# 31415Hacker/RayTracer-public

Measured on AMD Instinct MI355X. Metric: Msamples/sec @1920x1080 Stanford-Dragon-class, 4 spp, 8 bounces, higher is better.
Workload: dtype f32; 1 GPU; C2: dragon-class procedural closed mesh (871414 tris, seed 20260109; dragon.glb absent), native LBVH2->BVH4, 1920x1080, 4 spp, 8 bounces, camera (0,0,2.5) identity quat FOV 70, a new frame index (sample set) every step; triangles=871414, bvh4_nodes=1263056, width=1920, height=1080, spp=4, max_bounces=8, seed=1, frames_per_launch=32

## Files before the change

include/mi355pt.h:

```cpp
#ifndef MI355PT_H
#define MI355PT_H

#include <stdint.h>

#ifdef __cplusplus
extern "C" {
#endif

#if defined(__GNUC__)
#define PT_API __attribute__((visibility("default")))
#else
#define PT_API
#endif

typedef struct PtContext PtContext;

typedef enum PtStatus {
    PT_OK = 0,
    PT_ERR_INVALID_ARG = 1,
    PT_ERR_NO_DEVICE = 2,
    PT_ERR_HIP = 3,
    PT_ERR_NO_SCENE = 4,
    PT_ERR_BAD_BVH = 5,
    PT_ERR_IO = 6,
// ... 47 lines not shown
PT_API int  pt_set_stream(PtContext* ctx, void* hip_stream);
PT_API int  pt_synchronize(PtContext* ctx);
PT_API int  pt_get_stream(PtContext* ctx, void** hip_stream);


PT_API int pt_compute_bvh2_sizing(uint32_t num_tris, uint32_t* num_nodes2, uint64_t* bytes);
PT_API int pt_compute_bvh4_sizing(uint32_t num_nodes4, uint64_t* bytes);
PT_API int pt_morton_sort(const float* tris, uint32_t num_tris, uint32_t* morton_sorted, uint32_t* tri_index_sorted);
PT_API int pt_collapse_lbvh2_to_bvh4(const uint32_t* bvh2, uint32_t num_tris, uint32_t* out, uint64_t out_words, uint32_t* num_nodes4);
#define PT_ACCEL_REFERENCE     0
#define PT_ACCEL_AREA_COLLAPSE 1
#define PT_ACCEL_PLOC          2
PT_API int pt_collapse_bvh2_to_bvh4_accel(const uint32_t* bvh2, uint32_t num_tris, uint32_t accel, uint32_t* out, uint64_t out_words, uint32_t* num_nodes4);
PT_API int pt_build_bvh2_ploc(const float* tris, uint32_t num_tris, uint32_t* out, uint64_t out_words);
PT_API int pt_bvh2_to_bvh4_wide(const uint32_t* bvh2, uint64_t bvh2_words, uint32_t* out, uint64_t out_words);
PT_API int pt_file_write_u32(const char* path, const uint32_t* src, uint64_t words);
PT_API int pt_file_read_u32(const char* path, uint32_t* dst, uint64_t dst_words, uint64_t* words);

PT_API int pt_scene_procedural(uint32_t kind, uint32_t seed, uint32_t num_tris, float* tris_out);


PT_API int pt_set_triangles(PtContext* ctx, const float* tris, uint32_t num_tris);
PT_API int pt_build_bvh(PtContext* ctx);
PT_API int pt_build_bvh_accel(PtContext* ctx, uint32_t accel);
PT_API int pt_build_lbvh2(PtContext* ctx, const uint32_t* morton_sorted, const uint32_t* tri_index_sorted);
PT_API int pt_read_bvh2(PtContext* ctx, uint32_t* dst, uint64_t bytes);
PT_API int pt_set_bvh4(PtContext* ctx, const uint32_t* bvh4, uint64_t words);
PT_API int pt_set_bvh2(PtContext* ctx, const uint32_t* bvh2, uint64_t words);
PT_API int pt_read_bvh4(PtContext* ctx, uint32_t* dst, uint64_t bytes);
PT_API int pt_set_spheres(PtContext* ctx, const float* xyzr, uint32_t num_spheres);
PT_API int pt_scene_info(PtContext* ctx, uint32_t* num_tris, uint32_t* num_nodes2, uint32_t* num_nodes4);


PT_API int pt_render(PtContext* ctx, const PtRenderParams* params);
PT_API int pt_set_batch(PtContext* ctx, uint32_t frames_per_launch);
PT_API int pt_flush(PtContext* ctx);
PT_API int pt_last_render_ms(PtContext* ctx, float* ms);
PT_API int pt_timing_begin(PtContext* ctx, uint32_t capacity);
PT_API int pt_timing_collect(PtContext* ctx, float* ms, uint32_t capacity, uint32_t* count);
PT_API int pt_timing_collect_spans(PtContext* ctx, float* start_ms, float* dur_ms, uint32_t capacity, uint32_t* count);
PT_API int pt_get_stats(PtContext* ctx, PtStats* out);
PT_API int pt_read_radiance(PtContext* ctx, float* dst, uint64_t dst_floats);
PT_API int pt_read_rgba8(PtContext* ctx, uint8_t* dst, uint64_t dst_bytes);
PT_API int pt_read_tonemapped(PtContext* ctx, int from_rgba8, uint8_t* dst, uint64_t dst_bytes);

typedef struct PtAccumInfo {
    uint32_t width, height;
    uint32_t tile_rank, tile_count;
    uint32_t compact;
    uint32_t samples;
    uint64_t floats;
} PtAccumInfo;
PT_API int pt_accum_info(PtContext* ctx, PtAccumInfo* out);
PT_API int pt_read_accum(PtContext* ctx, float* dst, uint64_t dst_floats);
PT_API int pt_set_accum(PtContext* ctx, const PtAccumInfo* info, const float* src);

typedef struct PtRay { float org[3]; float t_max; float dir[3]; uint32_t reserved; } PtRay;
typedef struct PtHit { float t; uint32_t prim; float u, v; } PtHit;
enum {
    PT_TRACE_ANY_HIT = 1u,
    PT_TRACE_STATS = 2u,
    PT_TRACE_SIMPLE_KERNEL = 4u
};
PT_API int pt_trace_rays(PtContext* ctx, const void* rays_device, uint64_t n, uint32_t flags, void* hits_device);
PT_API int pt_trace_rays_host(PtContext* ctx, const PtRay* rays, uint64_t n, uint32_t flags, PtHit* hits);
PT_API int pt_camera_rays(PtContext* ctx, const PtRenderParams* params, void* rays_device);

typedef struct PtPoint   { float p[3]; float r_max; } PtPoint;
typedef struct PtClosest { float dist; uint32_t prim; float u, v; } PtClosest;
enum {
    PT_CLOSEST_STATS = 1u,
    PT_CLOSEST_SIMPLE_KERNEL = 2u,
    PT_CLOSEST_BRUTE_FORCE = 4u
};
PT_API int pt_closest_points(PtContext* ctx, const void* points_device, uint64_t n, uint32_t flags, void* out_device);
PT_API int pt_closest_points_host(PtContext* ctx, const PtPoint* points, uint64_t n, uint32_t flags, PtClosest* out);
PT_API int pt_closest_points_bvh4(const float* tris, uint32_t num_tris, const uint32_t* bvh4, uint64_t words,
                                  const PtPoint* points, uint64_t n, uint32_t flags, PtClosest* out, PtStats* stats);

typedef struct PtSurfel    { float p[3]; float r_max; float n[3]; uint32_t reserved; } PtSurfel;
typedef struct PtOcclusion { float visibility; uint32_t unoccluded; uint32_t samples; uint32_t reserved; } PtOcclusion;
typedef struct PtOcclusionParams { uint32_t samples; uint32_t seed; uint32_t index_base; float bias; uint32_t flags; } PtOcclusionParams;
enum {
    PT_OCCLUSION_STATS = 1u,
    PT_OCCLUSION_SIMPLE_KERNEL = 2u
};
PT_API int pt_occlusion(PtContext* ctx, const void* surfels_device, uint64_t n, const PtOcclusionParams* params, void* out_device);
PT_API int pt_occlusion_host(PtContext* ctx, const PtSurfel* surfels, uint64_t n, const PtOcclusionParams* params, PtOcclusion* out);
PT_API int pt_occlusion_rays(PtContext* ctx, const void* surfels_device, uint64_t n, const PtOcclusionParams* params, void* rays_device);
PT_API int pt_occlusion_rays_host(const PtSurfel* surfels, uint64_t n, const PtOcclusionParams* params, PtRay* rays);
PT_API int pt_hit_surfels(PtContext* ctx, const void* rays_device, const void* hits_device, uint64_t n, float r_max, void* surfels_device);
PT_API int pt_hit_surfels_host(PtContext* ctx, const PtRay* rays, const PtHit* hits, uint64_t n, float r_max, PtSurfel* out);

PT_API int pt_update_triangles(PtContext* ctx, const float* tris, uint32_t num_tris);
PT_API int pt_update_triangles_device(PtContext* ctx, const void* tris_device, uint32_t num_tris);
PT_API int pt_bvh_cost(PtContext* ctx, double* cost);
PT_API int pt_refit_bvh4(const float* tris, uint32_t num_tris, uint32_t* bvh4, uint64_t words);
PT_API int pt_refit_bvh2(const float* tris, uint32_t num_tris, uint32_t* bvh2, uint64_t words);
PT_API int pt_bvh4_cost(const uint32_t* bvh4, uint64_t words, double* cost);


PT_API int pt_tile_layout(uint32_t width, uint32_t height, uint32_t tile_rank, uint32_t tile_count,
                   uint32_t* num_tiles, uint64_t* compact_floats);
PT_API int pt_tile_ids(uint32_t width, uint32_t height, uint32_t tile_rank, uint32_t tile_count,
                uint32_t* ids, uint32_t capacity, uint32_t* num_tiles);
PT_API int pt_compact_radiance(PtContext* ctx, void** device_ptr, uint64_t* floats);
PT_API int pt_set_compact_buffer(PtContext* ctx, void* device_ptr, uint64_t floats);
PT_API int pt_set_output_buffer(PtContext* ctx, void* device_ptr, uint64_t floats);
PT_API int pt_buffer_busy(PtContext* ctx, const void* device_ptr, uint64_t bytes, int* busy);
PT_API int pt_deinterleave(PtContext* ctx, const void* gathered_device, uint64_t stride_floats,
                    uint32_t width, uint32_t height, uint32_t tile_count);
PT_API int pt_deinterleave_batch(PtContext* ctx, const void* gathered_device, uint64_t rank_stride_floats, uint64_t frame_stride_floats,
                          uint32_t num_frames, uint32_t width, uint32_t height, uint32_t tile_count,
                          void* frames_out_device, uint64_t out_stride_floats);

PT_API int pt_traced_tile_rect(PtContext* ctx, const PtRenderParams* params, uint32_t rect[4]);
PT_API int pt_packed_layout(uint32_t width, uint32_t height, uint32_t tile_count, const uint32_t rect[4], uint32_t* max_tiles, uint64_t* floats_per_frame);
PT_API int pt_packed_tile_ids(uint32_t width, uint32_t height, uint32_t tile_rank, uint32_t tile_count, const uint32_t rect[4],
                              uint32_t* ids, uint32_t capacity, uint32_t* num_tiles);
PT_API int pt_pack_shares(PtContext* ctx, const void* compact_device, uint64_t frame_stride_floats, uint32_t num_frames, uint32_t width, uint32_t height,
                          uint32_t tile_rank, uint32_t tile_count, const uint32_t rect[4], void* packed_device, uint64_t packed_frame_stride_floats);
PT_API int pt_unpack_batch(PtContext* ctx, const void* gathered_device, uint64_t rank_stride_floats, uint64_t frame_stride_floats, uint32_t num_frames,
                           uint32_t width, uint32_t height, uint32_t tile_count, const uint32_t rect[4], uint32_t spp,
                           void* frames_out_device, uint64_t out_stride_floats);

typedef struct PtGroup PtGroup;
enum {
    PT_GROUP_TRANSPORT_RCCL = 0,
    PT_GROUP_TRANSPORT_COPY = 1
};
PT_API int  pt_group_create(const int* device_ordinals, uint32_t num_devices, uint32_t transport, PtGroup** out);
PT_API void pt_group_destroy(PtGroup* group);
PT_API const char* pt_group_last_error(const PtGroup* group);
PT_API int  pt_group_size(const PtGroup* group, uint32_t* num_members);
PT_API int  pt_group_context(PtGroup* group, uint32_t rank, PtContext** ctx);
PT_API int  pt_group_set_triangles(PtGroup* group, const float* tris, uint32_t num_tris);
PT_API int  pt_group_update_triangles(PtGroup* group, const float* tris, uint32_t num_tris);
PT_API int  pt_group_build_bvh(PtGroup* group);
PT_API int  pt_group_build_bvh_accel(PtGroup* group, uint32_t accel);
PT_API int  pt_group_set_bvh2(PtGroup* group, const uint32_t* bvh2, uint64_t words);
PT_API int  pt_group_set_bvh4(PtGroup* group, const uint32_t* bvh4, uint64_t words);
PT_API int  pt_group_set_batch(PtGroup* group, uint32_t frames_per_launch);
PT_API int  pt_group_render(PtGroup* group, const PtRenderParams* params);
PT_API int  pt_group_flush(PtGroup* group);
PT_API int  pt_group_synchronize(PtGroup* group);
PT_API int  pt_group_read_radiance(PtGroup* group, float* dst, uint64_t dst_floats);
PT_API int  pt_group_read_rgba8(PtGroup* group, uint8_t* dst, uint64_t dst_bytes);
PT_API int  pt_group_read_tonemapped(PtGroup* group, int from_rgba8, uint8_t* dst, uint64_t dst_bytes);

PT_API int pt_debug_set_tune(PtContext* ctx, const char* name, uint32_t value);
PT_API int pt_debug_launch_plan(uint32_t num_cus, uint32_t frames, uint32_t tile_count, uint32_t launches_in_flight, uint32_t traced_batches, uint32_t batch_size, uint32_t out[12]);
PT_API int pt_debug_counters(PtContext* ctx, unsigned long long* dst24);
PT_API int pt_debug_wave_times(PtContext* ctx, unsigned long long* dst, uint32_t max_waves, uint32_t* n_waves);

#ifdef __cplusplus
}
#endif
#endif
```

raytracer-public_amd/__init__.py:

```python
import ctypes as C
import math
import os
import sys

import numpy as np

_HERE = os.path.dirname(os.path.abspath(__file__))
LIB_PATH = os.path.join(_HERE, "libmi355pt.so")

PT_MODE_REFERENCE_PACKET, PT_MODE_REFERENCE, PT_MODE_PATH = 0, 1, 2
PT_FLAG_STATS = 1
PT_FLAG_SIMPLE_KERNEL = 2
PT_FLAG_BRUTE_FORCE = 4
PT_FLAG_COMPACT = 8
SCENE_DRAGON_CLASS, SCENE_SPONZA_CLASS = 0, 1
PT_ACCEL_REFERENCE, PT_ACCEL_AREA_COLLAPSE, PT_ACCEL_PLOC = 0, 1, 2
PT_TRACE_ANY_HIT, PT_TRACE_STATS, PT_TRACE_SIMPLE_KERNEL = 1, 2, 4
PT_CLOSEST_STATS, PT_CLOSEST_SIMPLE_KERNEL, PT_CLOSEST_BRUTE_FORCE = 1, 2, 4
PT_OCCLUSION_STATS, PT_OCCLUSION_SIMPLE_KERNEL = 1, 2
PRIM_NONE = 0xFFFFFFFF


class PtError(RuntimeError):
    def __init__(self, code, message):
        super().__init__("libmi355pt error %d: %s" % (code, message))
        self.code = code


class PtRenderParams(C.Structure):
    _fields_ = [
        ("width", C.c_uint32), ("height", C.c_uint32),
        ("focal", C.c_float), ("aspect", C.c_float),
        ("cam_pos", C.c_float * 3), ("num_tris", C.c_uint32),
        ("cam_quat", C.c_float * 4),
        ("frame", C.c_uint32), ("mode", C.c_uint32),
        ("spp", C.c_uint32), ("max_bounces", C.c_uint32), ("seed", C.c_uint32),
        ("accumulate", C.c_uint32),
        ("tile_rank", C.c_uint32), ("tile_count", C.c_uint32),
        ("flags", C.c_uint32),
    ]


class PtStats(C.Structure):
    _fields_ = [(n, C.c_uint64) for n in (
        "rays_closest", "rays_shadow", "nodes_examined", "tris_tested", "stack_drops", "max_stack", "samples")]

    def as_dict(self):
        return {n: int(getattr(self, n)) for n, _ in self._fields_}


class PtRay(C.Structure):
    _fields_ = [("org", C.c_float * 3), ("t_max", C.c_float), ("dir", C.c_float * 3), ("reserved", C.c_uint32)]


class PtHit(C.Structure):
    _fields_ = [("t", C.c_float), ("prim", C.c_uint32), ("u", C.c_float), ("v", C.c_float)]


class PtPoint(C.Structure):
    _fields_ = [("p", C.c_float * 3), ("r_max", C.c_float)]


class PtClosest(C.Structure):
    _fields_ = [("dist", C.c_float), ("prim", C.c_uint32), ("u", C.c_float), ("v", C.c_float)]


class PtSurfel(C.Structure):
    _fields_ = [("p", C.c_float * 3), ("r_max", C.c_float), ("n", C.c_float * 3), ("reserved", C.c_uint32)]


class PtOcclusion(C.Structure):
    _fields_ = [("visibility", C.c_float), ("unoccluded", C.c_uint32), ("samples", C.c_uint32), ("reserved", C.c_uint32)]


class PtOcclusionParams(C.Structure):
    _fields_ = [("samples", C.c_uint32), ("seed", C.c_uint32), ("index_base", C.c_uint32), ("bias", C.c_float), ("flags", C.c_uint32)]


class PtAccumInfo(C.Structure):
    _fields_ = [("width", C.c_uint32), ("height", C.c_uint32), ("tile_rank", C.c_uint32), ("tile_count", C.c_uint32),
                ("compact", C.c_uint32), ("samples", C.c_uint32), ("floats", C.c_uint64)]


EXPORTS = [
    "pt_create", "pt_destroy", "pt_last_error", "pt_version", "pt_set_stream", "pt_get_stream", "pt_synchronize",
    "pt_compute_bvh2_sizing", "pt_compute_bvh4_sizing", "pt_morton_sort", "pt_collapse_lbvh2_to_bvh4",
    "pt_collapse_bvh2_to_bvh4_accel", "pt_build_bvh2_ploc", "pt_bvh2_to_bvh4_wide", "pt_file_write_u32", "pt_file_read_u32", "pt_scene_procedural",
    "pt_set_triangles", "pt_build_bvh", "pt_build_bvh_accel", "pt_build_lbvh2", "pt_read_bvh2", "pt_set_bvh4", "pt_set_bvh2",
    "pt_read_bvh4", "pt_set_spheres", "pt_scene_info", "pt_render", "pt_last_render_ms", "pt_set_batch", "pt_flush", "pt_timing_begin", "pt_timing_collect", "pt_timing_collect_spans", "pt_set_compact_buffer", "pt_set_output_buffer", "pt_get_stats", "pt_read_radiance",
    "pt_read_rgba8", "pt_read_tonemapped", "pt_tile_layout", "pt_tile_ids", "pt_compact_radiance", "pt_deinterleave", "pt_deinterleave_batch", "pt_buffer_busy",
    "pt_accum_info", "pt_read_accum", "pt_set_accum",
    "pt_trace_rays", "pt_trace_rays_host", "pt_camera_rays",
    "pt_closest_points", "pt_closest_points_host", "pt_closest_points_bvh4",
    "pt_occlusion", "pt_occlusion_host", "pt_occlusion_rays", "pt_occlusion_rays_host", "pt_hit_surfels", "pt_hit_surfels_host",
    "pt_update_triangles", "pt_update_triangles_device", "pt_bvh_cost", "pt_refit_bvh4", "pt_refit_bvh2", "pt_bvh4_cost", "pt_group_update_triangles",
    "pt_traced_tile_rect", "pt_packed_layout", "pt_packed_tile_ids", "pt_pack_shares", "pt_unpack_batch",
    "pt_group_create", "pt_group_destroy", "pt_group_last_error", "pt_group_size", "pt_group_context", "pt_group_set_triangles", "pt_group_build_bvh",
    "pt_group_build_bvh_accel",
    "pt_group_set_bvh2", "pt_group_set_bvh4", "pt_group_set_batch", "pt_group_render", "pt_group_flush", "pt_group_synchronize", "pt_group_read_radiance",
    "pt_group_read_rgba8", "pt_group_read_tonemapped",
    "pt_debug_set_tune", "pt_debug_counters", "pt_debug_wave_times", "pt_debug_launch_plan",
]


def _load():
    os.environ.setdefault("GPU_MAX_HW_QUEUES", "12")
    if not os.path.exists(LIB_PATH):
        raise ImportError(
            "libmi355pt.so is not built (%s). Run `python -c 'import __graft_entry__ as g; g.build()'` "
            "or `make -C raytracer-public_amd/csrc`. There is no CPU fallback." % LIB_PATH)
    lib = C.CDLL(LIB_PATH)
    lib.pt_last_error.restype = C.c_char_p
    lib.pt_last_error.argtypes = [C.c_void_p]
    lib.pt_version.restype = C.c_char_p
    lib.pt_destroy.restype = None
    lib.pt_destroy.argtypes = [C.c_void_p]
    return lib


_TORCH_FIRST = "torch" in sys.modules
lib = _load()


def _p(a, t):
    return a.ctypes.data_as(C.POINTER(t))


def _aligned_zeros(shape, dtype, align=16):
    dtype = np.dtype(dtype)
    n = int(np.prod(shape)) * dtype.itemsize
    raw = np.zeros(n + align, np.uint8)
    off = (-raw.ctypes.data) % align
    return raw[off: off + n].view(dtype).reshape(shape)


def _is_torch(x):
    return type(x).__module__.startswith("torch")


def _torch_route():
    if not _TORCH_FIRST:
        raise RuntimeError("the torch route of the ray queries needs `import torch` before this package is imported: both must use "
                           "the same HIP runtime (torch ships its own)")


def pack_rays(origins, directions, t_max=None):
    o = np.asarray(origins, np.float32).reshape(-1, 3)
    d = np.asarray(directions, np.float32).reshape(-1, 3)
    if o.shape != d.shape:
        raise ValueError("origins and directions differ in shape: %s vs %s" % (o.shape, d.shape))
    out = _aligned_zeros((o.shape[0], 8), np.float32)
    out[:, 0:3] = o
    out[:, 3] = np.inf if t_max is None else np.broadcast_to(np.asarray(t_max, np.float32), (o.shape[0],))
    out[:, 4:7] = d
    return out


def pack_points(points, r_max=None):
    p = np.asarray(points, np.float32).reshape(-1, 3)
    out = _aligned_zeros((p.shape[0], 4), np.float32)
    out[:, 0:3] = p
    out[:, 3] = np.inf if r_max is None else np.broadcast_to(np.asarray(r_max, np.float32), (p.shape[0],))
    return out


def _point_records(points, r_max):
    a = np.asarray(points, np.float32)
    if a.ndim == 2 and a.shape[1] == 4:
        if a.ctypes.data % 16 or not a.flags.c_contiguous or r_max is not None:
            r2 = _aligned_zeros(a.shape, np.float32); r2[...] = a; a = r2
            if r_max is not None:
                a[:, 3] = r_max
        return a
    return pack_points(a, r_max)


def pack_surfels(points, normals, r_max=None):
    return pack_rays(points, normals, r_max)


def _records8(a, what):
    a = np.asarray(a, np.float32)
    if a.ndim != 2 or a.shape[1] != 8:
        raise ValueError("%s: expected (n, 8) float32 records, got shape %s" % (what, a.shape))
    if a.ctypes.data % 16 or not a.flags.c_contiguous:
        r2 = _aligned_zeros(a.shape, np.float32); r2[...] = a; a = r2
    return a


def _occlusion_params(samples, seed, bias, index_base, stats=False, simple=False):
    p = PtOcclusionParams()
    p.samples, p.seed, p.index_base, p.bias = int(samples), int(seed) & 0xFFFFFFFF, int(index_base) & 0xFFFFFFFF, float(bias)
    p.flags = (PT_OCCLUSION_STATS if stats else 0) | (PT_OCCLUSION_SIMPLE_KERNEL if simple else 0)
    return p


def occlusion_rays_host(surfels, samples, seed=0, bias=1e-4, index_base=0):
    sf = _records8(surfels, "occlusion_rays_host")
    n = sf.shape[0]
    p = _occlusion_params(samples, seed, bias, index_base)
    rays = _aligned_zeros((n * max(int(samples), 0) if 0 < int(samples) <= 65536 else 0, 8), np.float32)
    _check(lib.pt_occlusion_rays_host(sf.ctypes.data_as(C.POINTER(PtSurfel)), C.c_uint64(n), C.byref(p), rays.ctypes.data_as(C.POINTER(PtRay))))
    return rays


def _closest_flags(stats, simple, brute_force):
    return (PT_CLOSEST_STATS if stats else 0) | (PT_CLOSEST_SIMPLE_KERNEL if simple else 0) | (PT_CLOSEST_BRUTE_FORCE if brute_force else 0)


def _check(rc, ctx=None):
    if rc != 0:
        msg = lib.pt_last_error(ctx)
        raise PtError(rc, msg.decode() if msg else "")


def focal_aspect(width, height):
    fov = (70.0 * math.pi) / 180
    return float(np.float32(1.0 / math.tan(0.5 * fov))), float(np.float32(width / height))



def compute_bvh2_sizing(num_tris):
    nn, by = C.c_uint32(), C.c_uint64()
    _check(lib.pt_compute_bvh2_sizing(C.c_uint32(num_tris), C.byref(nn), C.byref(by)))
    return {"numNodes2": nn.value, "bytes": by.value}


def compute_bvh4_sizing(num_nodes4):
    by = C.c_uint64()
    _check(lib.pt_compute_bvh4_sizing(C.c_uint32(num_nodes4), C.byref(by)))
    return {"bytes": by.value}


def morton_sort(tris):
    tris = np.ascontiguousarray(tris, np.float32).reshape(-1)
    n = tris.size // 9
    m = np.zeros(n, np.uint32); t = np.zeros(n, np.uint32)
    _check(lib.pt_morton_sort(_p(tris, C.c_float), C.c_uint32(n), _p(m, C.c_uint32), _p(t, C.c_uint32)))
    return m, t


def collapse_lbvh2_to_bvh4(bvh2, num_tris):
    bvh2 = np.ascontiguousarray(bvh2, np.uint32)
    cap = 1 + 8 * max(2 * num_tris - 1, 0)
    out = np.zeros(cap, np.uint32)
    n4 = C.c_uint32()
    _check(lib.pt_collapse_lbvh2_to_bvh4(_p(bvh2, C.c_uint32), C.c_uint32(num_tris), _p(out, C.c_uint32), C.c_uint64(cap), C.byref(n4)))
    return out[: 1 + 8 * n4.value].copy(), n4.value


def collapse_bvh2_to_bvh4_accel(bvh2, num_tris, accel):
    bvh2 = np.ascontiguousarray(bvh2, np.uint32)
    cap = 1 + 8 * max(2 * num_tris - 1, 0)
    out = np.zeros(cap, np.uint32)
# ... 93 lines not shown
    r = (C.c_uint32 * 4)(*rect); n = C.c_uint32()
    _check(lib.pt_packed_tile_ids(C.c_uint32(width), C.c_uint32(height), C.c_uint32(rank), C.c_uint32(count), r, None, C.c_uint32(0), C.byref(n)))
    ids = np.zeros(max(n.value, 1), np.uint32)
    _check(lib.pt_packed_tile_ids(C.c_uint32(width), C.c_uint32(height), C.c_uint32(rank), C.c_uint32(count), r, _p(ids, C.c_uint32), C.c_uint32(ids.size), C.byref(n)))
    return ids[: n.value]


def tile_ids(width, height, rank, count):
    n = C.c_uint32()
    _check(lib.pt_tile_ids(C.c_uint32(width), C.c_uint32(height), C.c_uint32(rank), C.c_uint32(count), None, C.c_uint32(0), C.byref(n)))
    ids = np.zeros(max(n.value, 1), np.uint32)
    _check(lib.pt_tile_ids(C.c_uint32(width), C.c_uint32(height), C.c_uint32(rank), C.c_uint32(count), ids.ctypes.data_as(C.POINTER(C.c_uint32)), C.c_uint32(ids.size), C.byref(n)))
    return ids[: n.value]



class Context:

    def __init__(self, device=-1):
        h = C.c_void_p()
        _check(lib.pt_create(C.c_int(device), C.byref(h)))
        self.h = h

    def close(self):
        if getattr(self, "h", None):
            lib.pt_destroy(self.h)
            self.h = None

    def __del__(self):
        try:
            self.close()
        except Exception:
            pass

    def _ck(self, rc):
        _check(rc, self.h)

    def set_stream(self, stream_handle):
        self._ck(lib.pt_set_stream(self.h, C.c_void_p(stream_handle)))

    def get_stream(self):
        p = C.c_void_p()
        self._ck(lib.pt_get_stream(self.h, C.byref(p)))
        return p.value

    def synchronize(self):
        self._ck(lib.pt_synchronize(self.h))

    def set_triangles(self, tris):
        tris = np.ascontiguousarray(tris, np.float32).reshape(-1)
        self._ck(lib.pt_set_triangles(self.h, _p(tris, C.c_float), C.c_uint32(tris.size // 9)))
        self.num_tris = tris.size // 9

    def update_triangles(self, tris):
        if _is_torch(tris):
            _torch_route()
            import torch
            if tris.device.type != "cuda":
                raise ValueError("update_triangles: torch tensors must be on the context's GPU (got %s)" % tris.device)
            t = tris.reshape(-1)
            if t.dtype != torch.float32 or not t.is_contiguous() or t.data_ptr() % 16:
                t = t.to(torch.float32).contiguous().clone()
            if t.numel() % 9:
                raise ValueError("update_triangles: 9 floats per triangle")
            self._on_context_stream(t.device, lambda: self.update_triangles_device(t.data_ptr(), t.numel() // 9))
            return
        tris = np.ascontiguousarray(tris, np.float32).reshape(-1)
        self._ck(lib.pt_update_triangles(self.h, _p(tris, C.c_float), C.c_uint32(tris.size // 9)))

    def update_triangles_device(self, tris_ptr, num_tris):
        self._ck(lib.pt_update_triangles_device(self.h, C.c_void_p(tris_ptr), C.c_uint32(num_tris)))

    def bvh_cost(self):
        cost = C.c_double()
        self._ck(lib.pt_bvh_cost(self.h, C.byref(cost)))
        return cost.value

    def set_spheres(self, xyzr):
        xyzr = np.ascontiguousarray(xyzr, np.float32).reshape(-1)
        self._ck(lib.pt_set_spheres(self.h, _p(xyzr, C.c_float), C.c_uint32(xyzr.size // 4)))

    def build_bvh(self, accel=PT_ACCEL_REFERENCE):
        if accel == PT_ACCEL_REFERENCE:
            self._ck(lib.pt_build_bvh(self.h))
        else:
            self._ck(lib.pt_build_bvh_accel(self.h, C.c_uint32(accel)))

    def build_lbvh2(self, morton, tri_idx):
        morton = np.ascontiguousarray(morton, np.uint32); tri_idx = np.ascontiguousarray(tri_idx, np.uint32)
        self._ck(lib.pt_build_lbvh2(self.h, _p(morton, C.c_uint32), _p(tri_idx, C.c_uint32)))

    def read_bvh2(self):
        out = np.zeros(compute_bvh2_sizing(self.num_tris)["bytes"] // 4, np.uint32)
        self._ck(lib.pt_read_bvh2(self.h, _p(out, C.c_uint32), C.c_uint64(out.size * 4)))
        return out

    def set_bvh4(self, bvh4):
        bvh4 = np.ascontiguousarray(bvh4, np.uint32)
        self._ck(lib.pt_set_bvh4(self.h, _p(bvh4, C.c_uint32), C.c_uint64(bvh4.size)))

    def set_bvh2(self, bvh2):
        bvh2 = np.ascontiguousarray(bvh2, np.uint32)
        self._ck(lib.pt_set_bvh2(self.h, _p(bvh2, C.c_uint32), C.c_uint64(bvh2.size)))

    def scene_info(self):
        a, b, c = C.c_uint32(), C.c_uint32(), C.c_uint32()
        self._ck(lib.pt_scene_info(self.h, C.byref(a), C.byref(b), C.byref(c)))
        return {"numTris": a.value, "numNodes2": b.value, "numNodes4": c.value}

    def read_bvh4(self):
        out = np.zeros(1 + 8 * self.scene_info()["numNodes4"], np.uint32)
        self._ck(lib.pt_read_bvh4(self.h, _p(out, C.c_uint32), C.c_uint64(out.size * 4)))
        return out

    def make_params(self, width, height, cam_pos=(0, 0, 2.5), cam_quat=(0, 0, 0, 1), mode=PT_MODE_REFERENCE, spp=1,
                    max_bounces=0, seed=1, frame=0, accumulate=False, tile_rank=0, tile_count=1, stats=False, num_tris=None, simple_kernel=False, brute_force=False):
        p = PtRenderParams()
        p.width, p.height = width, height
        p.focal, p.aspect = focal_aspect(width, height)
        p.cam_pos[:] = [float(np.float32(v)) for v in cam_pos]
        p.cam_quat[:] = [float(np.float32(v)) for v in cam_quat]
        p.num_tris = self.num_tris if num_tris is None else num_tris
        p.frame, p.mode, p.spp, p.max_bounces, p.seed = frame, mode, spp, max_bounces, seed
        p.accumulate = 1 if accumulate else 0
        p.tile_rank, p.tile_count = tile_rank, tile_count
        p.flags = (PT_FLAG_STATS if stats else 0) | (PT_FLAG_SIMPLE_KERNEL if simple_kernel else 0) | (PT_FLAG_BRUTE_FORCE if brute_force else 0)
        return p

    def render(self, params):
        self._ck(lib.pt_render(self.h, C.byref(params)))
        self._last = (params.width, params.height)

    def last_render_ms(self):
        ms = C.c_float()
        self._ck(lib.pt_last_render_ms(self.h, C.byref(ms)))
        return ms.value

    def set_batch(self, frames_per_launch):
        self._ck(lib.pt_set_batch(self.h, C.c_uint32(frames_per_launch)))

    def flush(self):
        self._ck(lib.pt_flush(self.h))

    def timing_begin(self, capacity):
        self._ck(lib.pt_timing_begin(self.h, C.c_uint32(capacity)))

    def timing_collect(self, capacity):
        ms = np.zeros(capacity, np.float32); n = C.c_uint32()
        self._ck(lib.pt_timing_collect(self.h, _p(ms, C.c_float), C.c_uint32(capacity), C.byref(n)))
        return ms[: n.value].copy()

    def debug_set_tune(self, name, value=None):
        self._ck(lib.pt_debug_set_tune(self.h, name.encode(), C.c_uint32(0xFFFFFFFF if value is None else value)))

    def timing_collect_spans(self, capacity):
        st = np.zeros(capacity, np.float32); ms = np.zeros(capacity, np.float32); n = C.c_uint32()
        self._ck(lib.pt_timing_collect_spans(self.h, _p(st, C.c_float), _p(ms, C.c_float), C.c_uint32(capacity), C.byref(n)))
        return st[: n.value].copy(), ms[: n.value].copy()

    def set_compact_buffer(self, device_ptr, floats):
        self._ck(lib.pt_set_compact_buffer(self.h, C.c_void_p(device_ptr), C.c_uint64(floats)))

    def set_output_buffer(self, device_ptr, floats):
        self._ck(lib.pt_set_output_buffer(self.h, C.c_void_p(device_ptr), C.c_uint64(floats)))

    def stats(self):
        st = PtStats()
        self._ck(lib.pt_get_stats(self.h, C.byref(st)))
        return st.as_dict()

    def read_radiance(self, width=None, height=None):
        w, h = (width, height) if width else self._last
        out = np.zeros((h, w, 4), np.float32)
        self._ck(lib.pt_read_radiance(self.h, _p(out, C.c_float), C.c_uint64(out.size)))
        return out

    def read_rgba8(self):
        w, h = self._last
        out = np.zeros((h, w, 4), np.uint8)
        self._ck(lib.pt_read_rgba8(self.h, _p(out, C.c_uint8), C.c_uint64(out.size)))
        return out

    def read_tonemapped(self, from_rgba8=True):
        w, h = self._last
        out = np.zeros((h, w, 4), np.uint8)
        self._ck(lib.pt_read_tonemapped(self.h, C.c_int(int(from_rgba8)), _p(out, C.c_uint8), C.c_uint64(out.size)))
        return out

    def compact_radiance(self):
        ptr, fl = C.c_void_p(), C.c_uint64()
        self._ck(lib.pt_compact_radiance(self.h, C.byref(ptr), C.byref(fl)))
        return ptr.value, fl.value

    def deinterleave(self, gathered_device_ptr, stride_floats, width, height, tile_count):
        self._ck(lib.pt_deinterleave(self.h, C.c_void_p(gathered_device_ptr), C.c_uint64(stride_floats),
                                     C.c_uint32(width), C.c_uint32(height), C.c_uint32(tile_count)))
        self._last = (width, height)

    def deinterleave_batch(self, gathered_device_ptr, rank_stride_floats, frame_stride_floats, num_frames, width, height, tile_count, frames_out_ptr=0, out_stride_floats=0):
        self._ck(lib.pt_deinterleave_batch(self.h, C.c_void_p(gathered_device_ptr), C.c_uint64(rank_stride_floats), C.c_uint64(frame_stride_floats), C.c_uint32(num_frames),
                                           C.c_uint32(width), C.c_uint32(height), C.c_uint32(tile_count), C.c_void_p(frames_out_ptr or None), C.c_uint64(out_stride_floats)))
        self._last = (width, height)

    def traced_tile_rect(self, params):
        r = (C.c_uint32 * 4)()
        self._ck(lib.pt_traced_tile_rect(self.h, C.byref(params), r))
        return tuple(int(v) for v in r)

    def pack_shares(self, compact_ptr, frame_stride_floats, num_frames, width, height, tile_rank, tile_count, rect, packed_ptr, packed_frame_stride_floats):
        self._ck(lib.pt_pack_shares(self.h, C.c_void_p(compact_ptr), C.c_uint64(frame_stride_floats), C.c_uint32(num_frames), C.c_uint32(width), C.c_uint32(height),
                                    C.c_uint32(tile_rank), C.c_uint32(tile_count), (C.c_uint32 * 4)(*rect), C.c_void_p(packed_ptr), C.c_uint64(packed_frame_stride_floats)))

    def unpack_batch(self, gathered_ptr, rank_stride_floats, frame_stride_floats, num_frames, width, height, tile_count, rect, spp, frames_out_ptr=0, out_stride_floats=0):
        self._ck(lib.pt_unpack_batch(self.h, C.c_void_p(gathered_ptr), C.c_uint64(rank_stride_floats), C.c_uint64(frame_stride_floats), C.c_uint32(num_frames),
                                     C.c_uint32(width), C.c_uint32(height), C.c_uint32(tile_count), (C.c_uint32 * 4)(*rect), C.c_uint32(spp),
                                     C.c_void_p(frames_out_ptr or None), C.c_uint64(out_stride_floats)))
        self._last = (width, height)

    def accum_info(self):
        info = PtAccumInfo()
        self._ck(lib.pt_accum_info(self.h, C.byref(info)))
        return info

    def read_accum(self):
        info = self.accum_info()
        out = np.zeros(int(info.floats), np.float32)
        self._ck(lib.pt_read_accum(self.h, _p(out, C.c_float), C.c_uint64(out.size)))
        return info, out

    def set_accum(self, info, data):
        data = np.ascontiguousarray(data, np.float32).reshape(-1)
        assert data.size == info.floats
        self._ck(lib.pt_set_accum(self.h, C.byref(info), _p(data, C.c_float)))

    def trace_rays(self, origins, directions=None, t_max=None, any_hit=False, stats=False, simple=False):
        flags = (PT_TRACE_ANY_HIT if any_hit else 0) | (PT_TRACE_STATS if stats else 0) | (PT_TRACE_SIMPLE_KERNEL if simple else 0)
        if _is_torch(origins):
            return self._trace_rays_torch(origins, directions, t_max, flags)
        if directions is None:
            rays = np.asarray(origins, np.float32).reshape(-1, 8)
            if rays.ctypes.data % 16 or not rays.flags.c_contiguous or t_max is not None:
                r2 = _aligned_zeros(rays.shape, np.float32); r2[...] = rays; rays = r2
                if t_max is not None:
                    rays[:, 3] = t_max
        else:
            rays = pack_rays(origins, directions, t_max)
        n = rays.shape[0]
        hits = _aligned_zeros((n, 4), np.uint32)
        self._ck(lib.pt_trace_rays_host(self.h, rays.ctypes.data_as(C.POINTER(PtRay)), C.c_uint64(n), C.c_uint32(flags),
                                        hits.ctypes.data_as(C.POINTER(PtHit))))
        f = hits.view(np.float32)
        return f[:, 0].copy(), hits[:, 1].copy(), f[:, 2].copy(), f[:, 3].copy()

    def trace_rays_device(self, rays_ptr, n, hits_ptr, flags=0):
        self._ck(lib.pt_trace_rays(self.h, C.c_void_p(rays_ptr), C.c_uint64(n), C.c_uint32(flags), C.c_void_p(hits_ptr)))

    def camera_rays_device(self, params, rays_ptr):
        self._ck(lib.pt_camera_rays(self.h, C.byref(params), C.c_void_p(rays_ptr)))

    def _on_context_stream(self, device, launch):
        import torch
        cur = torch.cuda.current_stream(device)
        mine = self.get_stream()
        if cur.cuda_stream == mine:
            launch()
            return
        ext = torch.cuda.ExternalStream(mine, device=device)
        before = torch.cuda.Event(); before.record(cur); ext.wait_event(before)
        launch()
        after = torch.cuda.Event(); after.record(ext); cur.wait_event(after)

    def _trace_rays_torch(self, origins, directions, t_max, flags):
        _torch_route()
        import torch
        dev = origins.device
        if dev.type != "cuda":
            raise ValueError("trace_rays: torch tensors must be on the context's GPU (got %s)" % dev)
        if directions is None:
            rays = origins.reshape(-1, 8)
            if rays.dtype != torch.float32 or not rays.is_contiguous() or rays.data_ptr() % 16:
                rays = rays.to(torch.float32).contiguous().clone()
            if t_max is not None:
                rays = rays.clone(); rays[:, 3] = t_max
        else:
            o = origins.reshape(-1, 3).to(torch.float32); d = directions.reshape(-1, 3).to(device=dev, dtype=torch.float32)
            n = o.shape[0]
            tm = torch.full((n, 1), float("inf"), dtype=torch.float32, device=dev) if t_max is None else \
                torch.as_tensor(t_max, dtype=torch.float32, device=dev).reshape(-1, 1).expand(n, 1)
            rays = torch.cat([o, tm, d, torch.zeros((n, 1), dtype=torch.float32, device=dev)], dim=1).contiguous()
        n = rays.shape[0]
        hits = torch.empty((n, 4), dtype=torch.int32, device=dev)
        self._on_context_stream(dev, lambda: self.trace_rays_device(rays.data_ptr(), n, hits.data_ptr(), flags))
        hf = hits.view(torch.float32)
        return hf[:, 0], hits.view(torch.uint32)[:, 1], hf[:, 2], hf[:, 3]

    def camera_rays(self, params, device=None):
        _torch_route()
        import torch
        dev = torch.device("cuda", torch.cuda.current_device() if device is None else device)
        rays = torch.empty((params.height * params.width, 8), dtype=torch.float32, device=dev)
        self._on_context_stream(dev, lambda: self.camera_rays_device(params, rays.data_ptr()))
        return rays

    def closest_points(self, points, r_max=None, stats=False, simple=False, brute_force=False):
        flags = _closest_flags(stats, simple, brute_force)
        if _is_torch(points):
# ... 295 lines not shown
```

raytracer-public_amd/csrc/pt_api.cpp:

```cpp
#include "mi355pt.h"
#include "pt_host.h"
#include "pt_kernels.h"

#include <hip/hip_runtime.h>

#include <algorithm>
#include <cstdio>
#include <cstdlib>
#include <cstring>
#include <string>
#include <vector>

namespace {

thread_local std::string g_global_error;

template <typename T>
struct DevBuf {
    T* ptr = nullptr; size_t cap = 0;
    hipError_t ensure(size_t n) {
        if (n <= cap && ptr) return hipSuccess;
        if (ptr) { (void)hipFree(ptr); ptr = nullptr; cap = 0; }
        if (n == 0) n = 1;
        hipError_t e = hipMalloc((void**)&ptr, n * sizeof(T));
        if (e == hipSuccess) cap = n;
        return e;
    }
    void release() { if (ptr) (void)hipFree(ptr); ptr = nullptr; cap = 0; }
};

}

struct PtTune {
    static constexpr uint32_t kAuto = 0xFFFFFFFFu;
    uint32_t grid_div = kAuto, rows = kAuto, chunk = kAuto, xcd = kAuto, shade = kAuto, fill = kAuto,
             slots = kAuto, cull = kAuto, stats_batch = kAuto, quad = kAuto, fork = kAuto, bounded = kAuto, timeline = kAuto;
    uint32_t* find(const char* name) {
        static const struct { const char* n; uint32_t PtTune::* m; } tab[] = {
            {"GRIDDIV", &PtTune::grid_div}, {"ROWS", &PtTune::rows}, {"CHUNK", &PtTune::chunk}, {"XCD", &PtTune::xcd}, {"SHADE", &PtTune::shade},
            {"FILL", &PtTune::fill}, {"SLOTS", &PtTune::slots}, {"CULL", &PtTune::cull}, {"STATSBATCH", &PtTune::stats_batch}, {"QUAD", &PtTune::quad}, {"FORK", &PtTune::fork}, {"BOUNDED", &PtTune::bounded}, {"TIMELINE", &PtTune::timeline}};
        for (const auto& t : tab) if (std::strcmp(name, t.n) == 0) return &(this->*(t.m));
        return nullptr;
    }
    void from_environment() {
        static const char* names[] = {"GRIDDIV", "ROWS", "CHUNK", "XCD", "SHADE", "FILL", "SLOTS", "CULL", "STATSBATCH", "QUAD", "FORK", "BOUNDED", "TIMELINE"};
        for (const char* n : names) {
            const std::string key = std::string("PT_TUNE_") + n;
            const char* v = std::getenv(key.c_str());
            if (v && *v) *find(n) = uint32_t(std::strtoul(v, nullptr, 10));
        }
    }
    static uint32_t pick(uint32_t knob, uint32_t dflt) { return knob == kAuto ? dflt : knob; }
};

struct PtContext {
    int device = 0;
    PtTune tune;
    hipStream_t own_stream = nullptr;
    hipStream_t stream = nullptr;
    hipEvent_t ev_start = nullptr, ev_stop = nullptr;
    bool timed = false;
    std::string err;

    uint32_t num_tris = 0, num_nodes2 = 0, num_nodes4 = 0;
    bool edges_small = false;
    DevBuf<uint32_t> d_edge_max;
    bool have_tris = false, have_bvh = false, have_bvh2 = false;
    bool bvh2_refit_pending = false;
    pt::WideBvh wide_meta;

    DevBuf<float> d_tris9;
    DevBuf<uint4> d_scene; uint64_t node_off = 0, node_cap = 0; uint32_t scene_tris = 0;
    float4* trirec() const { return (float4*)d_scene.ptr; }
    uint4* wide() const { return d_scene.ptr + node_off / 16; }
    DevBuf<uint32_t> d_bvh2, d_bvh4;
    DevBuf<uint32_t> d_morton, d_triidx, d_parent, d_flags;
    DevBuf<unsigned long long> d_bounds; DevBuf<uint32_t> d_counters, d_code_tmp, d_index_tmp, d_node2, d_subtree, d_ids, d_bnd;
    DevBuf<uint4> d_child_pos; DevBuf<unsigned char> d_build_temp; uint32_t* h_word = nullptr;
    DevBuf<uint32_t> d_ploc;
    DevBuf<float4> d_spheres; uint32_t num_spheres = 0;
    bool tree_built = false, refit_ready = false, refit2_ready = false;
    uint32_t num_wide = 0;
    DevBuf<uint2> d_refit_up, d_refit_self; DevBuf<uint4> d_refit_ref; DevBuf<uint32_t> d_refit_arrive, d_refit_parent2, d_refit_arrive2;
    DevBuf<double> d_cost;
    bool bvh2_stale = false;
    uint32_t* h_refit = nullptr; hipEvent_t ev_refit = nullptr; bool meta_pending = false, meta_has_root = false;
    DevBuf<unsigned long long> d_rq_queue, d_rq_spill; DevBuf<uint4> d_rq_rays, d_rq_hits;
    DevBuf<uint4> d_oc_surfels;

    DevBuf<float4> d_out, d_accum, d_compact, d_compact_accum;
    DevBuf<uint32_t> d_tiles, d_u32tmp;
    struct FrameSlot {
        hipStream_t side = nullptr; hipEvent_t resolved = nullptr, done = nullptr; bool used = false;
        uint64_t resolved_seq = 0;
        DevBuf<uint32_t> queue; DevBuf<float4> samples; DevBuf<uint2> spill; DevBuf<uint4> rays;
        DevBuf<uint32_t> trace_slots; uint32_t* h_trace = nullptr; size_t h_trace_cap = 0; hipEvent_t trace_copied = nullptr;
        uint32_t cull_key[8] = {0, 0, 0, 0, 0, 0, 0, 0}; uint32_t num_trace_tiles = 0; bool cull_valid = false;
        DevBuf<ptk::FrameParams> frame_params; DevBuf<float4*> frame_outs;
        const void* primed_ptr = nullptr; size_t primed_samples = 0;
    };
    static constexpr int kMaxSlots = 16;
    FrameSlot slots[kMaxSlots]; int num_slots = 0; uint32_t next_slot = 0;
    uint32_t batch_size = 1; uint32_t pending = 0; ptk::RenderArgs pendingA; bool pending_ring = false; uint32_t pending_rank = 0, pending_count = 1;
    std::vector<ptk::FrameParams> pending_frames; std::vector<float4*> pending_outs;
    DevBuf<unsigned long long> d_wave_times; uint32_t wave_times_n = 0;
    int num_cus = 0;
    DevBuf<unsigned long long> d_stats;
    std::vector<uint32_t> tiles_host; uint32_t tiles_w = 0, tiles_h = 0, tiles_rank = 0, tiles_count = 0;
    uint32_t out_w = 0, out_h = 0;
    uint32_t accum_w = 0, accum_h = 0, accum_count = 0, accum_rank = 0;
    uint64_t compact_floats = 0;
    uint32_t share_w = 0, share_h = 0, share_count = 0, share_max_tiles = 0;
    float4* ext_compact = nullptr; uint64_t ext_compact_floats = 0;
    float4* ext_out = nullptr; uint64_t ext_out_floats = 0;
    const float4* last_full = nullptr;
    bool last_stats = false;
    uint64_t stats_culled = 0;
    std::vector<hipEvent_t> ring;
    uint32_t ring_used = 0;
    struct InFlight { const char* lo; const char* hi; uint64_t seq; };
    std::vector<InFlight> inflight;
    uint64_t launch_seq = 0, delivered_seq = 0;
    hipEvent_t misc_fence = nullptr; uint64_t misc_fence_seq = 0;
};

namespace {

int fail(PtContext* ctx, int code, const std::string& msg) {
    if (ctx) ctx->err = msg; else g_global_error = msg;
    return code;
}
int fail_hip(PtContext* ctx, hipError_t e, const char* what) {
    return fail(ctx, PT_ERR_HIP, std::string(what) + ": " + hipGetErrorString(e));
}
#define PT_HIP(ctx, call) do { hipError_t e__ = (call); if (e__ != hipSuccess) return fail_hip((ctx), e__, #call); } while (0)

int bind(PtContext* ctx) {
    if (!ctx) return fail(nullptr, PT_ERR_INVALID_ARG, "null context");
    PT_HIP(ctx, hipSetDevice(ctx->device));
    return PT_OK;
}

int sync_refit_meta(PtContext* ctx) {
    if (!ctx->meta_pending) return PT_OK;
    PT_HIP(ctx, hipEventSynchronize(ctx->ev_refit));
    ctx->meta_pending = false;
    const uint32_t* h = ctx->h_refit;
    ctx->edges_small = h[3] < 0x49800000u;
    if (ctx->meta_has_root && ctx->have_bvh) {
        pt::WideBvh& w = ctx->wide_meta;
        w.root_box[0] = h[0]; w.root_box[1] = h[1]; w.root_box[2] = h[2];
        w.root_degenerate = pt::half_to_float(h[0] & 0xffffu) > pt::half_to_float(h[1] >> 16) || pt::half_to_float(h[0] >> 16) > pt::half_to_float(h[2] & 0xffffu) ||
                            pt::half_to_float(h[1] & 0xffffu) > pt::half_to_float(h[2] >> 16);
    }
    return PT_OK;
}

uint32_t accum_share_key(uint32_t rank, uint32_t count, bool compact) { return (rank & 0xfffu) | ((count & 0xfffu) << 12) | (compact ? 0x80000000u : 0u); }

void prune_inflight(PtContext* ctx) {
    if (ctx->inflight.empty()) return;
    uint64_t delivered = ctx->delivered_seq;
    auto done = [&](hipEvent_t ev) {
        const hipError_t q = hipEventQuery(ev);
        if (q == hipErrorNotReady) { (void)hipGetLastError(); return false; }
        return true;
    };
    for (auto& sl : ctx->slots) if (sl.side && sl.used && sl.resolved_seq > delivered && done(sl.resolved)) delivered = sl.resolved_seq;
    if (ctx->misc_fence && ctx->misc_fence_seq > delivered && done(ctx->misc_fence)) delivered = ctx->misc_fence_seq;
    if (delivered != ctx->delivered_seq) {
        ctx->delivered_seq = delivered;
        ctx->inflight.erase(std::remove_if(ctx->inflight.begin(), ctx->inflight.end(), [&](const PtContext::InFlight& f) { return f.seq <= delivered; }), ctx->inflight.end());
    }
}
void everything_delivered(PtContext* ctx) {
    ctx->delivered_seq = ctx->launch_seq; ctx->inflight.clear();
}
uint64_t track_targets(PtContext* ctx, float4* const* targets, uint32_t n, size_t bytes) {
    if (ctx->inflight.size() >= 64) prune_inflight(ctx);
    const uint64_t seq = ++ctx->launch_seq;
    for (uint32_t i = 0; i < n; ++i) {
        if (!targets[i]) continue;
        bool dup = false;
        for (uint32_t g = 0; g < i && !dup; ++g) dup = targets[g] == targets[i];
        if (!dup) ctx->inflight.push_back({(const char*)targets[i], (const char*)targets[i] + bytes, seq});
    }
    return seq;
}

uint64_t tri_region_bytes(uint32_t num_tris) { return (uint64_t(num_tris) + 1u) * 64u; }

int ensure_scene(PtContext* ctx, uint32_t num_tris, uint64_t nodes) {
    const uint64_t tri_bytes = tri_region_bytes(num_tris);
    const uint64_t need = tri_bytes + (nodes + 1u) * 64u;
    if (need >= 0xFFFFFFFFull) return fail(ctx, PT_ERR_INVALID_ARG, "scene too large: triangle records and BVH nodes are addressed by 32-bit byte offsets (4 GiB)");
    if (ctx->d_scene.ptr && ctx->node_off == tri_bytes && ctx->node_cap >= nodes) {
        if (ctx->scene_tris != num_tris)
            PT_HIP(ctx, hipMemset((char*)ctx->d_scene.ptr + uint64_t(num_tris) * 64u, 0, tri_bytes - uint64_t(num_tris) * 64u));
        ctx->scene_tris = num_tris; return PT_OK;
    }
    const uint64_t cap_nodes = nodes + nodes / 8u + 16u;
    uint4* fresh = nullptr;
    PT_HIP(ctx, hipMalloc((void**)&fresh, tri_bytes + (cap_nodes + 1u) * 64u));
    if (ctx->d_scene.ptr && ctx->scene_tris == num_tris && num_tris)
        PT_HIP(ctx, hipMemcpy(fresh, ctx->d_scene.ptr, uint64_t(num_tris) * 64u, hipMemcpyDeviceToDevice));
    if (ctx->d_scene.ptr) (void)hipFree(ctx->d_scene.ptr);
    PT_HIP(ctx, hipMemset((char*)fresh + uint64_t(num_tris) * 64u, 0, tri_bytes - uint64_t(num_tris) * 64u));
    ctx->d_scene.ptr = fresh; ctx->d_scene.cap = size_t((tri_bytes + (cap_nodes + 1u) * 64u) / 16u);
    ctx->node_off = tri_bytes; ctx->node_cap = cap_nodes; ctx->scene_tris = num_tris;
    return PT_OK;
}

int upload_wide(PtContext* ctx, const uint32_t* bvh4, uint64_t words) {
    pt::WideBvh w; std::string err;
    if (int rc = sync_refit_meta(ctx)) return rc;
    const uint32_t tris_now = ctx->have_tris ? ctx->num_tris : 0u;
    if (!pt::build_wide_bvh(bvh4, words, tris_now, uint32_t(tri_region_bytes(tris_now) / 16u), w, err)) return fail(ctx, PT_ERR_BAD_BVH, err);
    PT_HIP(ctx, ctx->d_bvh4.ensure(words));
    PT_HIP(ctx, hipMemcpyAsync(ctx->d_bvh4.ptr, bvh4, words * 4, hipMemcpyHostToDevice, ctx->stream));
    if (int rc = ensure_scene(ctx, tris_now, w.nodes.size())) return rc;
    if (!w.nodes.empty())
        PT_HIP(ctx, hipMemcpyAsync(ctx->wide(), w.nodes.data(), w.nodes.size() * sizeof(pt::WideNode), hipMemcpyHostToDevice, ctx->stream));
    PT_HIP(ctx, hipStreamSynchronize(ctx->stream));
    ctx->num_nodes4 = w.num_nodes4;
    ctx->num_wide = uint32_t(w.nodes.size()); ctx->tree_built = false; ctx->refit_ready = false;
    w.nodes.clear(); w.nodes.shrink_to_fit();
    ctx->wide_meta = w;
    ctx->have_bvh = true;
    return PT_OK;
}

struct TileRect { uint32_t tx0, ty0, tx1, ty1; };
bool root_box_rect(const pt::WideBvh& w, const ptk::FrameParams& f, uint32_t width, uint32_t height, TileRect& out) {
    const double qx = f.quat[0], qy = f.quat[1], qz = f.quat[2], qw = f.quat[3];
    const double qn = qx * qx + qy * qy + qz * qz + qw * qw;
    if (!(qn > 1.0 - 1e-5 && qn < 1.0 + 1e-5) || !(f.focal > 1e-3f) || !(f.aspect > 1e-3f)) return false;
    const double mn[3] = {pt::half_to_float(w.root_box[0] & 0xffffu), pt::half_to_float(w.root_box[0] >> 16), pt::half_to_float(w.root_box[1] & 0xffffu)};
    const double mx[3] = {pt::half_to_float(w.root_box[1] >> 16), pt::half_to_float(w.root_box[2] & 0xffffu), pt::half_to_float(w.root_box[2] >> 16)};
    double x0 = 1e300, x1 = -1e300, y0 = 1e300, y1 = -1e300;
    for (int c = 0; c < 8; ++c) {
        const double p[3] = {((c & 1) ? mx[0] : mn[0]) - f.cam[0], ((c & 2) ? mx[1] : mn[1]) - f.cam[1], ((c & 4) ? mx[2] : mn[2]) - f.cam[2]};
        if (!(p[0] == p[0] && p[1] == p[1] && p[2] == p[2])) return false;
        const double ux = -qx, uy = -qy, uz = -qz;
        const double cx = uy * p[2] - uz * p[1], cy = uz * p[0] - ux * p[2], cz = ux * p[1] - uy * p[0];
        const double dx = uy * cz - uz * cy, dy = uz * cx - ux * cz, dz = ux * cy - uy * cx;
        const double vx = p[0] + 2.0 * (qw * cx + dx), vy = p[1] + 2.0 * (qw * cy + dy), vz = p[2] + 2.0 * (qw * cz + dz);
        if (!(vz < -1e-4)) return false;
        const double sx = vx / -vz * f.focal / f.aspect, sy = vy / -vz * f.focal;
        const double fx = (sx + 1.0) * 0.5 * width, fy = (sy + 1.0) * 0.5 * height;
        x0 = fx < x0 ? fx : x0; x1 = fx > x1 ? fx : x1; y0 = fy < y0 ? fy : y0; y1 = fy > y1 ? fy : y1;
    }
    const double margin = 2.0;
    const uint32_t tiles_x = (width + pt::kTile - 1) / pt::kTile, tiles_y = (height + pt::kTile - 1) / pt::kTile;
    auto lo = [&](double v, uint32_t n) { v = (v - margin) / pt::kTile; return v <= 0.0 ? 0u : (v >= n ? n : uint32_t(v)); };
    auto hi = [&](double v, uint32_t n) { v = (v + margin) / pt::kTile + 1.0; return v <= 0.0 ? 0u : (v >= n ? n : uint32_t(v)); };
    out.tx0 = lo(x0, tiles_x); out.tx1 = hi(x1, tiles_x); out.ty0 = lo(y0, tiles_y); out.ty1 = hi(y1, tiles_y);
    return true;
}

bool arith_is_bounded(const PtContext* ctx, const std::vector<ptk::FrameParams>& frames, uint32_t nf) {
    if (!ctx->edges_small) return false;
    for (uint32_t i = 0; i < nf; ++i) {
        const float* q = frames[i].quat;
        const double n2 = double(q[0]) * q[0] + double(q[1]) * q[1] + double(q[2]) * q[2] + double(q[3]) * q[3];
        if (!(n2 < 262144.0)) return false;
        if (!(frames[i].focal > 1e-6f && frames[i].focal < 1e6f && frames[i].aspect < 1e6f && frames[i].aspect > -1e6f)) return false;
    }
    return true;
}


struct PlanInput {
    uint32_t num_cus;
    uint32_t frames;
    uint32_t tile_count;
    bool     sharded;
    bool     stats;
    uint32_t launches_in_flight;
    uint32_t traced_batches;
    uint32_t batch_size;
};
struct LaunchPlan {
    uint32_t grid;
    uint32_t perm_rows, perm_cols, total_items, chunk_items, xcd_span;
    uint32_t shade_threshold, fill_threshold, quad_live, fork_shadow;
    int      slots, setup_slots;
    const char* error;
};

int slots_for(const PtTune& tune, uint32_t frames, uint32_t tile_count, bool sharded) {
    const uint32_t w8 = frames * 8u / (tile_count ? tile_count : 1u);
    const int n = int(PtTune::pick(tune.slots, w8 >= 256u ? 3u : (w8 >= 64u ? 4u : (w8 >= 16u ? PT_FRAME_SLOTS : (w8 >= 8u ? (sharded ? 4u : 6u) : (sharded ? 8u : PT_FRAME_SLOTS))))));
    return n < 1 ? 1 : (n > PtContext::kMaxSlots ? PtContext::kMaxSlots : n);
}

LaunchPlan plan_launch(const PtTune& tune, const PlanInput& in) {
    LaunchPlan P; std::memset(&P, 0, sizeof(P));
    const uint32_t nf = in.frames, count = in.tile_count ? in.tile_count : 1u;
    const int cus = in.num_cus > 0 ? int(in.num_cus) : 256;
    P.grid = ptk::megakernel_grid(cus);
    {
        uint32_t div = PtTune::pick(tune.grid_div, count >= 8u ? 4u : (count >= 2u ? 2u : std::min(4u, 1u + in.launches_in_flight)));
        if (nf > 1u) div = div > nf ? div / nf : 1u;
        if (div > 1u) P.grid = (P.grid + div - 1u) / div;
    }
    const uint32_t grid_lanes = P.grid * ptk::megakernel_block();
    const uint32_t work8 = nf * 8u / count;
    P.perm_rows = PtTune::pick(tune.rows, work8 >= 24u ? nf : (work8 >= 8u ? 128u * nf : 64u * nf));
    if (P.perm_rows < 1u) P.perm_rows = 1u;
    if (P.perm_rows > 4096u) P.perm_rows = 4096u;
    P.perm_cols = (in.traced_batches + P.perm_rows - 1u) / P.perm_rows;
    if (uint64_t(P.perm_cols) * P.perm_rows * 64ull > 0xFFFFFFFFull) { P.error = "pt_render: batch too large (more than 2^32 items per launch)"; return P; }
    P.total_items = P.perm_cols * P.perm_rows * 64u;
    P.chunk_items = ((PtTune::pick(tune.chunk, 128u) + 63u) / 64u) * 64u;
    if (P.chunk_items < 64u) P.chunk_items = 64u;
    if (uint64_t(P.total_items) + uint64_t(grid_lanes / 64u + 1u) * P.chunk_items > 0xFFFFFFFFull) {
        P.error = "pt_render: launch too large for the 32-bit work-queue cursor (more than 2^32 - grid * chunk items; lower spp, the resolution or the batch)"; return P;
    }
    {
        const uint32_t per = (P.total_items + 7u) / 8u;
        P.xcd_span = PtTune::pick(tune.xcd, work8 >= 64u ? 1u : 0u) ? ((per + P.chunk_items - 1u) / P.chunk_items) * P.chunk_items : 0u;
    }
    P.shade_threshold = PtTune::pick(tune.shade, PT_SHADE_THRESHOLD); P.fill_threshold = PtTune::pick(tune.fill, PT_FILL_THRESHOLD);
    P.quad_live = std::min(16u, PtTune::pick(tune.quad, PT_QUAD_LIVE));
    P.fork_shadow = PtTune::pick(tune.fork, PT_FORK_SHADOW);
    P.slots = in.stats ? 1 : slots_for(tune, nf, count, in.sharded);
    P.setup_slots = in.stats ? 1 : std::max(P.slots, slots_for(tune, std::max(nf, in.batch_size), count, in.sharded));
    return P;
}

bool traced_tiles(const PtContext* ctx, const ptk::RenderArgs& A, uint32_t nf, bool sharded, TileRect& rect, std::vector<uint32_t>& traced) {
    traced.clear(); rect = {0, 0, 0, 0};
    if (!(ctx->have_bvh && ctx->wide_meta.root_ref != pt::kInvalid && !ctx->wide_meta.root_degenerate && A.num_tris != 0u && ctx->tune.cull != 0u)) return false;
    for (uint32_t i = 0; i < nf; ++i) {
        TileRect r;
        if (!root_box_rect(ctx->wide_meta, ctx->pending_frames[i], A.width, A.height, r)) return false;
        if (i == 0) rect = r;
        else { rect.tx0 = std::min(rect.tx0, r.tx0); rect.ty0 = std::min(rect.ty0, r.ty0); rect.tx1 = std::max(rect.tx1, r.tx1); rect.ty1 = std::max(rect.ty1, r.ty1); }
    }
    const uint32_t tiles_y = (A.height + pt::kTile - 1) / pt::kTile;
    if (rect.tx0 == 0u && rect.ty0 == 0u && rect.tx1 >= A.tiles_x && rect.ty1 >= tiles_y) return false;
    auto inside = [&](uint32_t tile) { const uint32_t tx = tile % A.tiles_x, ty = tile / A.tiles_x; return tx >= rect.tx0 && tx < rect.tx1 && ty >= rect.ty0 && ty < rect.ty1; };
    if (sharded) { for (uint32_t sl = 0; sl < A.num_tiles; ++sl) if (inside(ctx->tiles_host[sl])) traced.push_back(sl); }
    else { for (uint32_t ty = rect.ty0; ty < rect.ty1; ++ty) for (uint32_t tx = rect.tx0; tx < rect.tx1; ++tx) traced.push_back(ty * A.tiles_x + tx); }
    return true;
}

int prepare_slots(PtContext* ctx, const LaunchPlan& P, const ptk::RenderArgs& A, uint32_t nf, bool stats) {
    const size_t n_samples = size_t(A.num_sample_batches) * 64u;
    const size_t cap_samples = std::max(n_samples, size_t(A.batches_per_frame) * 64u * size_t(ctx->batch_size));
    if (cap_samples > 0xFFFFFFFFull) return fail(ctx, PT_ERR_INVALID_ARG, "pt_render: batch too large (more than 2^32 samples per launch)");
    const int cus = ctx->num_cus > 0 ? ctx->num_cus : 256;
    const uint32_t full_lanes = ptk::megakernel_grid(cus) * ptk::megakernel_block();
    for (int si = 0; si < (stats ? 1 : P.setup_slots); ++si) {
        PtContext::FrameSlot& s = ctx->slots[si];
        if (!s.side) {
            PT_HIP(ctx, hipStreamCreateWithFlags(&s.side, hipStreamNonBlocking));
            PT_HIP(ctx, hipEventCreateWithFlags(&s.resolved, hipEventDisableTiming));
            PT_HIP(ctx, hipEventCreateWithFlags(&s.done, hipEventDisableTiming));
        }
        PT_HIP(ctx, s.queue.ensure(16));
        PT_HIP(ctx, s.samples.ensure(cap_samples));
        PT_HIP(ctx, s.spill.ensure(size_t(full_lanes) * size_t(64 - PT_SHORT_STACK)));
        PT_HIP(ctx, s.rays.ensure(size_t(full_lanes) * 3u));
        PT_HIP(ctx, s.frame_params.ensure(std::max<size_t>(ctx->batch_size, nf))); PT_HIP(ctx, s.frame_outs.ensure(std::max<size_t>(ctx->batch_size, nf)));
        if (s.primed_ptr != (const void*)s.samples.ptr || s.primed_samples < cap_samples) {
            if (s.used) PT_HIP(ctx, hipStreamWaitEvent(s.side, s.resolved, 0));
            PT_HIP(ctx, ptk::launch_prime(s.queue.ptr, s.side));
            s.primed_ptr = s.samples.ptr; s.primed_samples = cap_samples;
        }
    }
    return PT_OK;
}

int stage_traced_tiles(PtContext* ctx, PtContext::FrameSlot& sl, const uint32_t key[8], const std::vector<uint32_t>& traced) {
    if (sl.cull_valid && std::memcmp(key, sl.cull_key, 8 * sizeof(uint32_t)) == 0) return PT_OK;
    if (!sl.trace_copied) PT_HIP(ctx, hipEventCreateWithFlags(&sl.trace_copied, hipEventDisableTiming));
    else PT_HIP(ctx, hipEventSynchronize(sl.trace_copied));
    if (sl.h_trace_cap < traced.size()) {
        if (sl.h_trace) (void)hipHostFree(sl.h_trace);
        sl.h_trace = nullptr; sl.h_trace_cap = 0;
        PT_HIP(ctx, hipHostMalloc((void**)&sl.h_trace, std::max<size_t>(traced.size(), 1024) * sizeof(uint32_t), hipHostMallocDefault));
        sl.h_trace_cap = std::max<size_t>(traced.size(), 1024);
    }
    PT_HIP(ctx, sl.trace_slots.ensure(std::max<size_t>(traced.size(), 1)));
    if (!traced.empty()) std::memcpy(sl.h_trace, traced.data(), traced.size() * sizeof(uint32_t));
    sl.cull_valid = false;
    return PT_OK;
}

int flush_pending_stats(PtContext* ctx, bool stats, bool sharded, uint32_t count) {
    if (!ctx->pending) return PT_OK;
    ptk::RenderArgs A = ctx->pendingA;
    const uint32_t nf = ctx->pending;
    ctx->pending = 0;
    const bool ring = ctx->ring_used + 2 <= ctx->ring.size();
    hipEvent_t e0 = ring ? ctx->ring[ctx->ring_used] : ctx->ev_start, e1 = ring ? ctx->ring[ctx->ring_used + 1] : ctx->ev_stop;
    A.num_frames = nf;
    if (uint64_t(A.num_tiles) * A.spp * nf * 64ull > 0xFFFFFFFFull)
        return fail(ctx, PT_ERR_INVALID_ARG, "pt_render: more than 2^32 pixel-samples in one launch (lower spp, the resolution or the batch)");
    A.batches_per_frame = A.num_tiles * A.spp;
    A.num_sample_batches = A.batches_per_frame * nf;

    std::vector<uint32_t> traced;
    TileRect rect;
    const bool cull = traced_tiles(ctx, A, nf, sharded, rect, traced);
    A.num_trace_tiles = cull ? uint32_t(traced.size()) : A.num_tiles;
    ctx->stats_culled = 0;
    if (stats && cull) {
        uint64_t px_all = 0, px_traced = 0;
        auto tile_px = [&](uint32_t tile) { const uint32_t tx = tile % A.tiles_x, ty = tile / A.tiles_x; return uint64_t(std::min(8u, A.width - tx * 8u)) * std::min(8u, A.height - ty * 8u); };
        for (uint32_t sl = 0; sl < A.num_tiles; ++sl) px_all += tile_px(sharded ? ctx->tiles_host[sl] : sl);
        for (uint32_t sl : traced) px_traced += tile_px(sharded ? ctx->tiles_host[sl] : sl);
        ctx->stats_culled = (px_all - px_traced) * A.spp * nf;
    }
    A.trace_bpf = A.num_trace_tiles * A.spp;
    A.num_batches = A.trace_bpf * nf;
    auto magic = [](uint32_t d) { return d > 1u ? uint32_t(0x100000000ull / d) : 0xFFFFFFFFu; };
    A.trace_bpf_magic = magic(A.trace_bpf ? A.trace_bpf : 1u); A.spp_magic = magic(A.spp); A.tiles_x_magic = magic(A.tiles_x);
    if (A.num_batches == 0u) { A.trace_bpf = 1u; A.trace_bpf_magic = magic(1u); }
    PlanInput in; std::memset(&in, 0, sizeof(in));
    in.num_cus = uint32_t(ctx->num_cus > 0 ? ctx->num_cus : 256); in.frames = nf; in.tile_count = count; in.sharded = sharded; in.stats = stats;
    in.traced_batches = A.num_batches; in.batch_size = ctx->batch_size;
    if (count < 2u && nf == 1u && !stats) {
        for (const auto& o : ctx->slots) if (o.side && o.used && hipEventQuery(o.done) == hipErrorNotReady) ++in.launches_in_flight;
        (void)hipGetLastError();
    }
    const LaunchPlan P = plan_launch(ctx->tune, in);
    if (P.error) return fail(ctx, PT_ERR_INVALID_ARG, P.error);
    A.perm_rows = P.perm_rows; A.perm_rows_magic = magic(P.perm_rows); A.perm_cols = P.perm_cols; A.total_items = P.total_items;
    A.chunk_items = P.chunk_items; A.xcd_span = P.xcd_span;
    A.shade_threshold = P.shade_threshold; A.fill_threshold = P.fill_threshold; A.quad_live = P.quad_live; A.fork_shadow = P.fork_shadow;
    A.rcp_short = (PtTune::pick(ctx->tune.bounded, 1u) != 0u && arith_is_bounded(ctx, ctx->pending_frames, nf)) ? 1u : 0u;

    ctx->num_slots = P.slots;
    if (int rc = prepare_slots(ctx, P, A, nf, stats)) return rc;
    PtContext::FrameSlot& sl = ctx->slots[stats ? 0 : (ctx->next_slot++ % uint32_t(P.slots))];
    A.prime = stats ? 1u : 0u;
    A.samples = sl.samples.ptr; A.queue = sl.queue.ptr; A.spill = sl.spill.ptr; A.raybuf = sl.rays.ptr;
    A.trace_slots = nullptr;
    const uint32_t cull_key[8] = {rect.tx0, rect.ty0, rect.tx1, rect.ty1, A.width, A.height, ctx->pending_rank | (ctx->pending_count << 16), A.num_trace_tiles};
    if (cull) { if (int rc = stage_traced_tiles(ctx, sl, cull_key, traced)) return rc; }
    const bool timeline = !stats && PtTune::pick(ctx->tune.timeline, 0u) != 0u;
    if (stats || timeline) {
        const uint32_t stat_waves = P.grid * ptk::megakernel_block() / 64u;
        PT_HIP(ctx, ctx->d_wave_times.ensure(size_t(stat_waves) * ptk::kWaveTimeWords));
        A.wave_times = ctx->d_wave_times.ptr; ctx->wave_times_n = stat_waves;
    }

    if (!ring) PT_HIP(ctx, hipEventRecord(e0, ctx->stream));
    if (sl.used) PT_HIP(ctx, hipStreamWaitEvent(sl.side, sl.resolved, 0));
    if (cull) {
        if (!sl.cull_valid) {
            if (!traced.empty()) PT_HIP(ctx, hipMemcpyAsync(sl.trace_slots.ptr, sl.h_trace, traced.size() * sizeof(uint32_t), hipMemcpyHostToDevice, sl.side));
            PT_HIP(ctx, hipEventRecord(sl.trace_copied, sl.side));
            std::memcpy(sl.cull_key, cull_key, sizeof cull_key); sl.cull_valid = true; sl.num_trace_tiles = A.num_trace_tiles;
        }
        A.trace_slots = sl.trace_slots.ptr;
        A.trace_rect[0] = rect.tx0; A.trace_rect[1] = rect.tx1; A.trace_rect[2] = rect.ty0; A.trace_rect[3] = rect.ty1;
    }
    if (stats) {
        PT_HIP(ctx, hipMemsetAsync(ctx->d_stats.ptr, 0, 24 * sizeof(unsigned long long), sl.side));
        PT_HIP(ctx, hipMemsetAsync(ctx->d_wave_times.ptr, 0, size_t(ctx->wave_times_n) * ptk::kWaveTimeWords * 8u, sl.side));
    }
    if (timeline) PT_HIP(ctx, hipMemsetAsync(ctx->d_wave_times.ptr, 0, size_t(ctx->wave_times_n) * ptk::kWaveTimeWords * 8u, sl.side));
    {
        std::vector<ptk::FrameParams>& F = ctx->pending_frames;
        for (uint32_t i = 0; i < nf; ++i) {
            bool superseded = false;
            if ((F[i].accum_mode & 0xffu) == 0u)
                for (uint32_t g = i + 1u; g < nf && !superseded; ++g) superseded = ctx->pending_outs[g] == ctx->pending_outs[i];
            F[i].accum_mode = (F[i].accum_mode & 0xffu) | (superseded ? 0x100u : 0u);
        }
        PT_HIP(ctx, ptk::launch_frame_params(F.data(), ctx->pending_outs.data(), nf, sl.frame_params.ptr, sl.frame_outs.ptr, sl.side));
        A.frames = sl.frame_params.ptr; A.outs = sl.frame_outs.ptr;
    }
    PT_HIP(ctx, ptk::launch_trace(A, stats, P.grid, sl.side, ring ? e0 : nullptr, ring ? e1 : nullptr));
    PT_HIP(ctx, hipEventRecord(sl.done, sl.side));
    PT_HIP(ctx, hipStreamWaitEvent(ctx->stream, sl.done, 0));
    PT_HIP(ctx, ptk::launch_resolve(A, ctx->stream));
    PT_HIP(ctx, hipEventRecord(sl.resolved, ctx->stream)); sl.used = true;
    sl.resolved_seq = track_targets(ctx, ctx->pending_outs.data(), nf, (A.compact ? size_t(A.num_tiles) * 64u : size_t(A.width) * A.height) * sizeof(float4));
    if (!ring) PT_HIP(ctx, hipEventRecord(e1, ctx->stream));
    if (ring) ctx->ring_used += 2;
    ctx->timed = !ring;
    return PT_OK;
}

int flush_pending(PtContext* ctx) {
    if (!ctx->pending) return PT_OK;
    const uint32_t count = ctx->tiles_count ? ctx->tiles_count : 1u;
    const bool sharded = ctx->pendingA.compact != 0u;
    return flush_pending_stats(ctx, ctx->pendingA.stats != nullptr, sharded, sharded ? count : 1u);
}

}

extern "C" {

#define PT_STR2(x) #x
#define PT_STR(x) PT_STR2(x)
const char* pt_version(void) { return "mi355pt 0.1 (gfx950; workgroup " PT_STR(PT_MEGA_BLOCK) ", quad " PT_STR(PT_QUAD) ")"; }

const char* pt_last_error(const PtContext* ctx) { return ctx ? ctx->err.c_str() : g_global_error.c_str(); }

int pt_create(int device_ordinal, PtContext** out) {
    if (!out) return fail(nullptr, PT_ERR_INVALID_ARG, "pt_create: null out pointer");
    *out = nullptr;
    int count = 0;
    hipError_t e = hipGetDeviceCount(&count);
    if (e != hipSuccess || count <= 0)
        return fail(nullptr, PT_ERR_NO_DEVICE, std::string("pt_create: no HIP device available (") + (e != hipSuccess ? hipGetErrorString(e) : "device count 0") + "); libmi355pt has no CPU path");
    int dev = device_ordinal;
    if (dev < 0) { if (hipGetDevice(&dev) != hipSuccess) dev = 0; }
    if (dev >= count) return fail(nullptr, PT_ERR_INVALID_ARG, "pt_create: device ordinal out of range");
    e = hipSetDevice(dev);
    if (e != hipSuccess) return fail_hip(nullptr, e, "hipSetDevice");
    PtContext* ctx = new PtContext();
    ctx->device = dev;
    ctx->tune.from_environment();
    {
        int lo = 0, hi = 0;
        (void)hipDeviceGetStreamPriorityRange(&lo, &hi);
        e = hipStreamCreateWithPriority(&ctx->own_stream, hipStreamNonBlocking, hi);
    }
    if (e == hipSuccess) e = hipEventCreate(&ctx->ev_start);
    if (e == hipSuccess) e = hipEventCreate(&ctx->ev_stop);
    if (e == hipSuccess) e = ctx->d_stats.ensure(24);
    if (e == hipSuccess) { hipDeviceProp_t prop; e = hipGetDeviceProperties(&prop, dev); if (e == hipSuccess) ctx->num_cus = prop.multiProcessorCount; }
    if (e != hipSuccess) { int rc = fail_hip(nullptr, e, "pt_create"); pt_destroy(ctx); return rc; }
    ctx->stream = ctx->own_stream;
    *out = ctx;
    return PT_OK;
}

void pt_destroy(PtContext* ctx) {
    if (!ctx) return;
    (void)hipSetDevice(ctx->device);
    (void)flush_pending(ctx);
    if (ctx->stream) (void)hipStreamSynchronize(ctx->stream);
    ctx->d_tris9.release(); ctx->d_scene.release(); ctx->d_bvh2.release(); ctx->d_bvh4.release();
    ctx->d_spheres.release(); ctx->d_rq_queue.release(); ctx->d_rq_spill.release(); ctx->d_rq_rays.release(); ctx->d_rq_hits.release(); ctx->d_oc_surfels.release();
    ctx->d_morton.release(); ctx->d_triidx.release(); ctx->d_parent.release(); ctx->d_flags.release();
    ctx->d_out.release(); ctx->d_accum.release(); ctx->d_compact.release(); ctx->d_compact_accum.release();
    ctx->d_tiles.release(); ctx->d_u32tmp.release(); ctx->d_stats.release();
    ctx->d_wave_times.release();
    ctx->d_bounds.release(); ctx->d_counters.release(); ctx->d_code_tmp.release(); ctx->d_index_tmp.release(); ctx->d_node2.release();
    ctx->d_subtree.release(); ctx->d_ids.release(); ctx->d_bnd.release(); ctx->d_child_pos.release(); ctx->d_build_temp.release();
    if (ctx->h_word) (void)hipHostFree(ctx->h_word);
    ctx->d_refit_up.release(); ctx->d_refit_self.release(); ctx->d_refit_ref.release(); ctx->d_refit_arrive.release();
    ctx->d_refit_parent2.release(); ctx->d_refit_arrive2.release(); ctx->d_cost.release();
    if (ctx->h_refit) (void)hipHostFree(ctx->h_refit);
    if (ctx->ev_refit) (void)hipEventDestroy(ctx->ev_refit);
    for (auto& sl : ctx->slots) {
        sl.queue.release(); sl.samples.release(); sl.spill.release(); sl.rays.release(); sl.trace_slots.release();
        if (sl.h_trace) (void)hipHostFree(sl.h_trace);
        if (sl.trace_copied) (void)hipEventDestroy(sl.trace_copied); sl.frame_params.release(); sl.frame_outs.release();
        if (sl.resolved) (void)hipEventDestroy(sl.resolved);
        if (sl.done) (void)hipEventDestroy(sl.done);
        if (sl.side) { (void)hipStreamSynchronize(sl.side); (void)hipStreamDestroy(sl.side); }
    }
    for (hipEvent_t e : ctx->ring) (void)hipEventDestroy(e);
    if (ctx->misc_fence) (void)hipEventDestroy(ctx->misc_fence);
    if (ctx->ev_start) (void)hipEventDestroy(ctx->ev_start);
    if (ctx->ev_stop) (void)hipEventDestroy(ctx->ev_stop);
    if (ctx->own_stream) (void)hipStreamDestroy(ctx->own_stream);
    delete ctx;
}

int pt_set_stream(PtContext* ctx, void* hip_stream) {
    if (int rc = bind(ctx)) return rc;
    if (int rc = flush_pending(ctx)) return rc;
    PT_HIP(ctx, hipStreamSynchronize(ctx->stream));
    everything_delivered(ctx);
    ctx->stream = hip_stream ? (hipStream_t)hip_stream : ctx->own_stream;
    ctx->timed = false;
    return PT_OK;
}

int pt_get_stream(PtContext* ctx, void** hip_stream) {
    if (!ctx || !hip_stream) return fail(ctx, PT_ERR_INVALID_ARG, "pt_get_stream: null argument");
    *hip_stream = (void*)ctx->stream;
    return PT_OK;
}

int pt_synchronize(PtContext* ctx) {
    if (int rc = bind(ctx)) return rc;
    if (int rc = flush_pending(ctx)) return rc;
    PT_HIP(ctx, hipStreamSynchronize(ctx->stream));
    everything_delivered(ctx);
    return PT_OK;
}


int pt_compute_bvh2_sizing(uint32_t num_tris, uint32_t* num_nodes2, uint64_t* bytes) {
    const uint32_t nn = num_tris ? 2 * num_tris - 1 : 0;
    if (num_nodes2) *num_nodes2 = nn;
    if (bytes) *bytes = num_tris ? 4ull * (1ull + 6ull * nn) : 4ull;
    return PT_OK;
}
int pt_compute_bvh4_sizing(uint32_t num_nodes4, uint64_t* bytes) {
    if (bytes) *bytes = num_nodes4 ? 4ull * (1ull + 8ull * num_nodes4) : 4ull;
    return PT_OK;
}
int pt_morton_sort(const float* tris, uint32_t num_tris, uint32_t* morton_sorted, uint32_t* tri_index_sorted) {
    if (num_tris && (!tris || !morton_sorted || !tri_index_sorted)) return fail(nullptr, PT_ERR_INVALID_ARG, "pt_morton_sort: null pointer");
    pt::morton_codes_sorted(tris, num_tris, morton_sorted, tri_index_sorted);
    return PT_OK;
}
int pt_collapse_lbvh2_to_bvh4(const uint32_t* bvh2, uint32_t num_tris, uint32_t* out, uint64_t out_words, uint32_t* num_nodes4) {
    if (!out || (num_tris && !bvh2)) return fail(nullptr, PT_ERR_INVALID_ARG, "pt_collapse_lbvh2_to_bvh4: null pointer");
    std::vector<uint32_t> v; std::string err;
    if (!pt::collapse_to_bvh4(bvh2, num_tris, v, err)) return fail(nullptr, PT_ERR_BAD_BVH, err);
    if (v.size() > out_words) return fail(nullptr, PT_ERR_INVALID_ARG, "pt_collapse_lbvh2_to_bvh4: output buffer too small");
    std::memcpy(out, v.data(), v.size() * 4);
    if (num_nodes4) *num_nodes4 = v[0];
    return PT_OK;
}
int pt_collapse_bvh2_to_bvh4_accel(const uint32_t* bvh2, uint32_t num_tris, uint32_t accel, uint32_t* out, uint64_t out_words, uint32_t* num_nodes4) {
    if (accel > PT_ACCEL_PLOC) return fail(nullptr, PT_ERR_INVALID_ARG, "pt_collapse_bvh2_to_bvh4_accel: accel must be 0, 1 or 2");
    if (!out || (num_tris && !bvh2)) return fail(nullptr, PT_ERR_INVALID_ARG, "pt_collapse_bvh2_to_bvh4_accel: null pointer");
    std::vector<uint32_t> v; std::string err;
    if (!pt::collapse_to_bvh4(bvh2, num_tris, accel != PT_ACCEL_REFERENCE, v, err)) return fail(nullptr, PT_ERR_BAD_BVH, err);
    if (v.size() > out_words) return fail(nullptr, PT_ERR_INVALID_ARG, "pt_collapse_bvh2_to_bvh4_accel: output buffer too small");
    std::memcpy(out, v.data(), v.size() * 4);
    if (num_nodes4) *num_nodes4 = v[0];
    return PT_OK;
}
int pt_build_bvh2_ploc(const float* tris, uint32_t num_tris, uint32_t* out, uint64_t out_words) {
    if (!out || (num_tris && !tris)) return fail(nullptr, PT_ERR_INVALID_ARG, "pt_build_bvh2_ploc: null pointer");
    if (num_tris >= 0x7fffffffu) return fail(nullptr, PT_ERR_INVALID_ARG, "pt_build_bvh2_ploc: too many triangles for the 31-bit leaf index");
    std::vector<uint32_t> v; std::string err;
    if (!pt::build_bvh2_ploc(tris, num_tris, v, err)) return fail(nullptr, PT_ERR_BAD_BVH, err);
    if (v.size() > out_words) return fail(nullptr, PT_ERR_INVALID_ARG, "pt_build_bvh2_ploc: output buffer too small");
    std::memcpy(out, v.data(), v.size() * 4);
    return PT_OK;
}
int pt_bvh2_to_bvh4_wide(const uint32_t* bvh2, uint64_t bvh2_words, uint32_t* out, uint64_t out_words) {
    if (!bvh2 || !out) return fail(nullptr, PT_ERR_INVALID_ARG, "pt_bvh2_to_bvh4_wide: null pointer");
    std::vector<uint32_t> v; std::string err;
    if (!pt::promote_to_bvh4_wide(bvh2, bvh2_words, v, err)) return fail(nullptr, PT_ERR_BAD_BVH, err);
    if (v.size() > out_words) return fail(nullptr, PT_ERR_INVALID_ARG, "pt_bvh2_to_bvh4_wide: output buffer too small");
    std::memcpy(out, v.data(), v.size() * 4);
    return PT_OK;
}
int pt_file_write_u32(const char* path, const uint32_t* src, uint64_t words) {
    if (!path || (!src && words)) return fail(nullptr, PT_ERR_INVALID_ARG, "pt_file_write_u32: null pointer");
    FILE* f = std::fopen(path, "wb");
    if (!f) return fail(nullptr, PT_ERR_IO, std::string("cannot open for writing: ") + path);
    const size_t n = std::fwrite(src, 4, words, f);
    const int rc = std::fclose(f);
    if (n != words || rc != 0) return fail(nullptr, PT_ERR_IO, std::string("short write: ") + path);
    return PT_OK;
}
int pt_file_read_u32(const char* path, uint32_t* dst, uint64_t dst_words, uint64_t* words) {
    if (!path) return fail(nullptr, PT_ERR_INVALID_ARG, "pt_file_read_u32: null path");
    FILE* f = std::fopen(path, "rb");
    if (!f) return fail(nullptr, PT_ERR_IO, std::string("cannot open: ") + path);
    std::fseek(f, 0, SEEK_END);
    const long size = std::ftell(f);
    std::fseek(f, 0, SEEK_SET);
    if (size <= 0 || (size & 3)) { std::fclose(f); return fail(nullptr, PT_ERR_IO, std::string("not a u32 dump (size): ") + path); }
    const uint64_t n = uint64_t(size) / 4;
    if (words) *words = n;
    if (!dst) { std::fclose(f); return PT_OK; }
    if (dst_words < n) { std::fclose(f); return fail(nullptr, PT_ERR_INVALID_ARG, "pt_file_read_u32: destination too small"); }
    const size_t got = std::fread(dst, 4, n, f);
    std::fclose(f);
    if (got != n) return fail(nullptr, PT_ERR_IO, std::string("short read: ") + path);
    return PT_OK;
}
int pt_scene_procedural(uint32_t kind, uint32_t seed, uint32_t num_tris, float* tris_out) {
    std::string err;
    if (!pt::procedural_scene(kind, seed, num_tris, tris_out, err)) return fail(nullptr, PT_ERR_INVALID_ARG, err);
    return PT_OK;
}


int pt_set_triangles(PtContext* ctx, const float* tris, uint32_t num_tris) {
    if (int rc = bind(ctx)) return rc;
    if (int rc = flush_pending(ctx)) return rc;
    if (num_tris && !tris) return fail(ctx, PT_ERR_INVALID_ARG, "pt_set_triangles: null triangles");
    if (num_tris >= 0x7fffffffu) return fail(ctx, PT_ERR_INVALID_ARG, "pt_set_triangles: too many triangles for the 31-bit leaf index");
    if (int rc = sync_refit_meta(ctx)) return rc;
    PT_HIP(ctx, ctx->d_tris9.ensure(size_t(num_tris) * 9));
    ctx->scene_tris = ~0u;
    if (int rc = ensure_scene(ctx, num_tris, uint64_t(num_tris) + 16u)) return rc;
    uint32_t edge_bits = 0u;
    if (num_tris) {
        PT_HIP(ctx, ctx->d_edge_max.ensure(1));
        PT_HIP(ctx, hipMemsetAsync(ctx->d_edge_max.ptr, 0, sizeof(uint32_t), ctx->stream));
        PT_HIP(ctx, hipMemcpyAsync(ctx->d_tris9.ptr, tris, size_t(num_tris) * 36, hipMemcpyHostToDevice, ctx->stream));
        PT_HIP(ctx, ptk::launch_tri_records(ctx->d_tris9.ptr, num_tris, ctx->trirec(), ctx->d_edge_max.ptr, ctx->stream));
        PT_HIP(ctx, hipMemcpyAsync(&edge_bits, ctx->d_edge_max.ptr, sizeof(uint32_t), hipMemcpyDeviceToHost, ctx->stream));
    }
    PT_HIP(ctx, hipStreamSynchronize(ctx->stream));
    ctx->edges_small = edge_bits < 0x49800000u;
    ctx->num_tris = num_tris;
    ctx->have_tris = true;
    ctx->have_bvh = false; ctx->have_bvh2 = false; ctx->bvh2_refit_pending = false;
    ctx->refit_ready = false; ctx->refit2_ready = false; ctx->bvh2_stale = false;
    ctx->accum_count = 0;
    return PT_OK;
}

int pt_build_lbvh2(PtContext* ctx, const uint32_t* morton_sorted, const uint32_t* tri_index_sorted) {
    if (int rc = bind(ctx)) return rc;
    if (int rc = flush_pending(ctx)) return rc;
    if (!ctx->have_tris) return fail(ctx, PT_ERR_NO_SCENE, "pt_build_lbvh2: no triangles uploaded");
    const uint32_t n = ctx->num_tris;
    uint32_t nn2 = 0; uint64_t bytes = 0;
    pt_compute_bvh2_sizing(n, &nn2, &bytes);
    PT_HIP(ctx, ctx->d_bvh2.ensure(bytes / 4));
    ctx->num_nodes2 = nn2; ctx->refit2_ready = false; ctx->bvh2_stale = false;
    PT_HIP(ctx, hipMemcpyAsync(ctx->d_bvh2.ptr, &nn2, 4, hipMemcpyHostToDevice, ctx->stream));
    if (n == 0) { PT_HIP(ctx, hipStreamSynchronize(ctx->stream)); ctx->have_bvh2 = true; return PT_OK; }
    if (!morton_sorted || !tri_index_sorted) return fail(ctx, PT_ERR_INVALID_ARG, "pt_build_lbvh2: null sorted arrays");
    for (uint32_t i = 0; i < n; ++i)
        if (tri_index_sorted[i] >= n) return fail(ctx, PT_ERR_INVALID_ARG, "pt_build_lbvh2: triangle index out of range");
    for (uint32_t i = 1; i < n; ++i)
        if (morton_sorted[i] < morton_sorted[i - 1]) return fail(ctx, PT_ERR_INVALID_ARG, "pt_build_lbvh2: Morton codes are not sorted");
    PT_HIP(ctx, ctx->d_morton.ensure(n)); PT_HIP(ctx, ctx->d_triidx.ensure(n));
    PT_HIP(ctx, ctx->d_parent.ensure(nn2)); PT_HIP(ctx, ctx->d_flags.ensure(n > 1 ? n - 1 : 1));
    PT_HIP(ctx, hipMemcpyAsync(ctx->d_morton.ptr, morton_sorted, size_t(n) * 4, hipMemcpyHostToDevice, ctx->stream));
    PT_HIP(ctx, hipMemcpyAsync(ctx->d_triidx.ptr, tri_index_sorted, size_t(n) * 4, hipMemcpyHostToDevice, ctx->stream));
    PT_HIP(ctx, ptk::launch_lbvh2(ctx->d_bvh2.ptr, ctx->d_tris9.ptr, ctx->d_morton.ptr, ctx->d_triidx.ptr, ctx->d_parent.ptr, ctx->d_flags.ptr, n, true, ctx->stream));
    ctx->bvh2_refit_pending = false;
    PT_HIP(ctx, hipStreamSynchronize(ctx->stream));
    ctx->have_bvh2 = true;
    return PT_OK;
}

namespace {
ptk::RefitBuffers refit_buffers(PtContext* ctx) {
    ptk::RefitBuffers R;
    R.up = ctx->d_refit_up.ptr; R.self = ctx->d_refit_self.ptr; R.child_ref = ctx->d_refit_ref.ptr; R.arrive = ctx->d_refit_arrive.ptr;
    return R;
}

int ensure_refit_plan(PtContext* ctx) {
    if (ctx->refit_ready) return PT_OK;
    const uint32_t m = ctx->num_nodes4;
    PT_HIP(ctx, ctx->d_refit_up.ensure(m)); PT_HIP(ctx, ctx->d_refit_self.ensure(m));
    PT_HIP(ctx, ctx->d_refit_ref.ensure(ctx->num_wide)); PT_HIP(ctx, ctx->d_refit_arrive.ensure(m));
    if (m) PT_HIP(ctx, hipMemsetAsync(ctx->d_refit_arrive.ptr, 0, size_t(m) * 4, ctx->stream));
    const uint32_t node_base16 = uint32_t(ctx->node_off / 16u);
    if (ctx->tree_built) {
        PT_HIP(ctx, ptk::launch_refit_prepare4(ctx->d_bvh4.ptr, m, ctx->d_ids.ptr, ctx->num_tris, node_base16, refit_buffers(ctx), ctx->stream));
    } else if (m) {
        std::vector<uint32_t> words(1 + size_t(m) * 8), up, self, ref; std::string err;
        PT_HIP(ctx, hipMemcpyAsync(words.data(), ctx->d_bvh4.ptr, words.size() * 4, hipMemcpyDeviceToHost, ctx->stream));
        PT_HIP(ctx, hipStreamSynchronize(ctx->stream));
        if (!pt::refit_plan4(words.data(), words.size(), ctx->num_tris, node_base16, up, self, ref, err)) return fail(ctx, PT_ERR_BAD_BVH, err);
        if (ref.size() / 4 != ctx->num_wide) return fail(ctx, PT_ERR_BAD_BVH, "refit plan: wide node count differs from the arena's");
        PT_HIP(ctx, hipMemcpyAsync(ctx->d_refit_up.ptr, up.data(), up.size() * 4, hipMemcpyHostToDevice, ctx->stream));
        PT_HIP(ctx, hipMemcpyAsync(ctx->d_refit_self.ptr, self.data(), self.size() * 4, hipMemcpyHostToDevice, ctx->stream));
        if (!ref.empty()) PT_HIP(ctx, hipMemcpyAsync(ctx->d_refit_ref.ptr, ref.data(), ref.size() * 4, hipMemcpyHostToDevice, ctx->stream));
        PT_HIP(ctx, hipStreamSynchronize(ctx->stream));
    }
    ctx->refit_ready = true;
    return PT_OK;
}

int refit_bvh2_on_stream(PtContext* ctx) {
    const uint32_t nn2 = ctx->num_nodes2;
    if (!ctx->refit2_ready) {
        PT_HIP(ctx, ctx->d_refit_parent2.ensure(nn2)); PT_HIP(ctx, ctx->d_refit_arrive2.ensure(nn2));
        if (nn2) PT_HIP(ctx, hipMemsetAsync(ctx->d_refit_arrive2.ptr, 0, size_t(nn2) * 4, ctx->stream));
        PT_HIP(ctx, ptk::launch_refit_prepare2(ctx->d_bvh2.ptr, nn2, ctx->d_refit_parent2.ptr, ctx->stream));
        ctx->refit2_ready = true;
    }
    PT_HIP(ctx, ptk::launch_refit2(ctx->d_tris9.ptr, ctx->num_tris, ctx->d_bvh2.ptr, nn2, ctx->d_refit_parent2.ptr, ctx->d_refit_arrive2.ptr, ctx->stream));
    ctx->bvh2_stale = false; ctx->bvh2_refit_pending = false;
    return PT_OK;
}

int update_triangles(PtContext* ctx, const char* fn, const void* tris, uint32_t num_tris, bool from_device) {
    if (int rc = bind(ctx)) return rc;
    if (!tris) return fail(ctx, PT_ERR_INVALID_ARG, std::string(fn) + ": null triangles");
    if (from_device && (reinterpret_cast<uintptr_t>(tris) & 15u)) return fail(ctx, PT_ERR_INVALID_ARG, std::string(fn) + ": the device array must be 16-byte aligned");
    if (!ctx->have_tris) return fail(ctx, PT_ERR_NO_SCENE, std::string(fn) + ": no triangles uploaded (pt_set_triangles first)");
    if (num_tris != ctx->num_tris) return fail(ctx, PT_ERR_INVALID_ARG, std::string(fn) + ": an update keeps the triangle count (pt_set_triangles changes it)");
    if (int rc = flush_pending(ctx)) return rc;
    if (num_tris == 0u) return PT_OK;
    const bool tree = ctx->have_bvh && ctx->num_nodes4 != 0u;
    if (tree) { if (int rc = ensure_refit_plan(ctx)) return rc; }
    if (!ctx->h_refit) PT_HIP(ctx, hipHostMalloc((void**)&ctx->h_refit, 16, hipHostMallocDefault));
    if (!ctx->ev_refit) PT_HIP(ctx, hipEventCreateWithFlags(&ctx->ev_refit, hipEventDisableTiming));
    PT_HIP(ctx, ctx->d_edge_max.ensure(1));
    PT_HIP(ctx, hipMemsetAsync(ctx->d_edge_max.ptr, 0, sizeof(uint32_t), ctx->stream));
    PT_HIP(ctx, hipMemcpyAsync(ctx->d_tris9.ptr, tris, size_t(num_tris) * 36, from_device ? hipMemcpyDeviceToDevice : hipMemcpyHostToDevice, ctx->stream));
    PT_HIP(ctx, ptk::launch_tri_records(ctx->d_tris9.ptr, num_tris, ctx->trirec(), ctx->d_edge_max.ptr, ctx->stream));
    if (tree) {
        PT_HIP(ctx, ptk::launch_refit4(ctx->d_tris9.ptr, num_tris, ctx->d_bvh4.ptr, ctx->num_nodes4, refit_buffers(ctx), ctx->wide(), ctx->stream));
        PT_HIP(ctx, hipMemcpyAsync(ctx->h_refit, ctx->d_bvh4.ptr + 1, 12, hipMemcpyDeviceToHost, ctx->stream));
    }
    PT_HIP(ctx, hipMemcpyAsync(ctx->h_refit + 3, ctx->d_edge_max.ptr, 4, hipMemcpyDeviceToHost, ctx->stream));
    PT_HIP(ctx, hipEventRecord(ctx->ev_refit, ctx->stream));
    ctx->meta_pending = true; ctx->meta_has_root = tree;
    if (ctx->have_bvh2) ctx->bvh2_stale = true;
    ctx->accum_count = 0;
    if (!from_device) {
        PT_HIP(ctx, hipStreamSynchronize(ctx->stream));
        return sync_refit_meta(ctx);
    }
    return PT_OK;
}
}

int pt_update_triangles(PtContext* ctx, const float* tris, uint32_t num_tris) { return update_triangles(ctx, "pt_update_triangles", tris, num_tris, false); }
int pt_update_triangles_device(PtContext* ctx, const void* tris_device, uint32_t num_tris) { return update_triangles(ctx, "pt_update_triangles_device", tris_device, num_tris, true); }

int pt_bvh_cost(PtContext* ctx, double* cost) {
    if (int rc = bind(ctx)) return rc;
    if (!cost) return fail(ctx, PT_ERR_INVALID_ARG, "pt_bvh_cost: null destination");
    if (!ctx->have_bvh) return fail(ctx, PT_ERR_NO_SCENE, "pt_bvh_cost: no BVH on the device");
    *cost = 0.0;
    if (ctx->num_nodes4 == 0u) return PT_OK;
    if (int rc = ensure_refit_plan(ctx)) return rc;
    PT_HIP(ctx, ctx->d_cost.ensure(1));
    PT_HIP(ctx, ptk::launch_bvh_cost(ctx->d_bvh4.ptr, ctx->num_nodes4, ctx->d_refit_self.ptr, ctx->d_cost.ptr, ctx->stream));
    PT_HIP(ctx, hipMemcpyAsync(cost, ctx->d_cost.ptr, sizeof(double), hipMemcpyDeviceToHost, ctx->stream));
    PT_HIP(ctx, hipStreamSynchronize(ctx->stream));
    return PT_OK;
}

int pt_refit_bvh4(const float* tris, uint32_t num_tris, uint32_t* bvh4, uint64_t words) {
    if (!bvh4 || (!tris && num_tris)) return fail(nullptr, PT_ERR_INVALID_ARG, "pt_refit_bvh4: null pointer");
    std::string err;
    if (!pt::refit_bvh4(tris, num_tris, bvh4, words, err)) return fail(nullptr, PT_ERR_BAD_BVH, err);
    return PT_OK;
}
int pt_refit_bvh2(const float* tris, uint32_t num_tris, uint32_t* bvh2, uint64_t words) {
    if (!bvh2 || (!tris && num_tris)) return fail(nullptr, PT_ERR_INVALID_ARG, "pt_refit_bvh2: null pointer");
    std::string err;
    if (!pt::refit_bvh2(tris, num_tris, bvh2, words, err)) return fail(nullptr, PT_ERR_BAD_BVH, err);
    return PT_OK;
}
int pt_bvh4_cost(const uint32_t* bvh4, uint64_t words, double* cost) {
    if (!bvh4 || !cost) return fail(nullptr, PT_ERR_INVALID_ARG, "pt_bvh4_cost: null pointer");
    std::string err;
    if (!pt::bvh4_cost(bvh4, words, *cost, err)) return fail(nullptr, PT_ERR_BAD_BVH, err);
    return PT_OK;
}

int pt_read_bvh2(PtContext* ctx, uint32_t* dst, uint64_t bytes) {
    if (int rc = bind(ctx)) return rc;
    if (!ctx->have_bvh2) return fail(ctx, PT_ERR_NO_SCENE, "pt_read_bvh2: no BVH2 on the device");
    if (!dst) return fail(ctx, PT_ERR_INVALID_ARG, "pt_read_bvh2: null destination");
    uint64_t have = 0; pt_compute_bvh2_sizing(ctx->num_tris, nullptr, &have);
    const uint64_t n = bytes < have ? bytes : have;
    if (ctx->bvh2_stale) {
        if (int rc = refit_bvh2_on_stream(ctx)) return rc;
    } else if (ctx->bvh2_refit_pending) {
        PT_HIP(ctx, ptk::launch_lbvh2_refit(ctx->d_bvh2.ptr, ctx->d_parent.ptr, ctx->d_flags.ptr, ctx->num_tris, ctx->stream));
        ctx->bvh2_refit_pending = false;
    }
    PT_HIP(ctx, hipMemcpyAsync(dst, ctx->d_bvh2.ptr, n, hipMemcpyDeviceToHost, ctx->stream));
    PT_HIP(ctx, hipStreamSynchronize(ctx->stream));
    return PT_OK;
}

int pt_set_bvh4(PtContext* ctx, const uint32_t* bvh4, uint64_t words) {
    if (int rc = bind(ctx)) return rc;
    if (int rc = flush_pending(ctx)) return rc;
    if (!bvh4 || words < 1) return fail(ctx, PT_ERR_INVALID_ARG, "pt_set_bvh4: empty buffer");
    ctx->accum_count = 0;
    return upload_wide(ctx, bvh4, words);
}

int pt_set_bvh2(PtContext* ctx, const uint32_t* bvh2, uint64_t words) {
    if (int rc = bind(ctx)) return rc;
    if (int rc = flush_pending(ctx)) return rc;
    if (!ctx->have_tris) return fail(ctx, PT_ERR_NO_SCENE, "pt_set_bvh2: upload triangles first");
    uint32_t nn2 = 0; uint64_t bytes = 0; pt_compute_bvh2_sizing(ctx->num_tris, &nn2, &bytes);
    if (!bvh2 || words * 4 < bytes || bvh2[0] != nn2) return fail(ctx, PT_ERR_BAD_BVH, "pt_set_bvh2: buffer does not match 2N-1 nodes of the uploaded triangles");
    PT_HIP(ctx, ctx->d_bvh2.ensure(bytes / 4));
    PT_HIP(ctx, hipMemcpyAsync(ctx->d_bvh2.ptr, bvh2, bytes, hipMemcpyHostToDevice, ctx->stream));
    PT_HIP(ctx, hipStreamSynchronize(ctx->stream));
    ctx->num_nodes2 = nn2; ctx->have_bvh2 = true; ctx->bvh2_refit_pending = false;
    ctx->refit2_ready = false; ctx->bvh2_stale = false;
    std::vector<uint32_t> b4; std::string err;
    if (!pt::collapse_to_bvh4(bvh2, ctx->num_tris, b4, err)) return fail(ctx, PT_ERR_BAD_BVH, err);
    ctx->accum_count = 0;
    return upload_wide(ctx, b4.data(), b4.size());
}

int pt_build_bvh(PtContext* ctx) { return pt_build_bvh_accel(ctx, PT_ACCEL_REFERENCE); }

int pt_build_bvh_accel(PtContext* ctx, uint32_t accel) {
    if (int rc = bind(ctx)) return rc;
    if (accel > PT_ACCEL_PLOC) return fail(ctx, PT_ERR_INVALID_ARG, "pt_build_bvh_accel: accel must be 0 (reference), 1 (area collapse) or 2 (PLOC)");
    if (int rc = flush_pending(ctx)) return rc;
    if (!ctx->have_tris) return fail(ctx, PT_ERR_NO_SCENE, "pt_build_bvh: no triangles uploaded");
    if (int rc = sync_refit_meta(ctx)) return rc;
    const uint32_t n = ctx->num_tris;
    if (n == 0) {
        const uint32_t zero = 0;
        if (int rc = pt_build_lbvh2(ctx, nullptr, nullptr)) return rc;
        return upload_wide(ctx, &zero, 1);
    }
    uint32_t nn2 = 0; uint64_t bytes2 = 0;
    pt_compute_bvh2_sizing(n, &nn2, &bytes2);
    PT_HIP(ctx, ctx->d_bvh2.ensure(bytes2 / 4));
    PT_HIP(ctx, ctx->d_morton.ensure(n)); PT_HIP(ctx, ctx->d_triidx.ensure(n));
    PT_HIP(ctx, ctx->d_parent.ensure(nn2)); PT_HIP(ctx, ctx->d_flags.ensure(n > 1 ? n - 1 : 1));
    PT_HIP(ctx, ctx->d_bounds.ensure(6)); PT_HIP(ctx, ctx->d_counters.ensure(ptk::kBuildCounters));
    PT_HIP(ctx, ctx->d_code_tmp.ensure(n)); PT_HIP(ctx, ctx->d_index_tmp.ensure(n));
    PT_HIP(ctx, ctx->d_node2.ensure(nn2)); PT_HIP(ctx, ctx->d_child_pos.ensure(nn2)); PT_HIP(ctx, ctx->d_subtree.ensure(nn2));
    PT_HIP(ctx, ctx->d_ids.ensure(nn2)); PT_HIP(ctx, ctx->d_bnd.ensure(size_t(nn2) * 3));
    size_t temp_bytes = ptk::build_temp_bytes(n);
    if (accel == PT_ACCEL_PLOC) {
        temp_bytes = std::max(temp_bytes, ptk::ploc_temp_bytes(n));
        PT_HIP(ctx, ctx->d_ploc.ensure(ptk::ploc_words(n)));
    }
    PT_HIP(ctx, ctx->d_build_temp.ensure(temp_bytes));
    if (!ctx->h_word) PT_HIP(ctx, hipHostMalloc((void**)&ctx->h_word, 64, hipHostMallocDefault));
    PT_HIP(ctx, ctx->d_bvh4.ensure(1 + size_t(nn2) * 8));
    ptk::BuildBuffers B;
    B.bounds = ctx->d_bounds.ptr; B.counters = ctx->d_counters.ptr; B.code_tmp = ctx->d_code_tmp.ptr; B.index_tmp = ctx->d_index_tmp.ptr;
    B.morton = ctx->d_morton.ptr; B.tri_index = ctx->d_triidx.ptr; B.temp = ctx->d_build_temp.ptr; B.temp_bytes = temp_bytes;
    B.node2 = ctx->d_node2.ptr; B.child_pos = ctx->d_child_pos.ptr; B.subtree = ctx->d_subtree.ptr; B.ids = ctx->d_ids.ptr; B.bnd = ctx->d_bnd.ptr;
    B.host_word = ctx->h_word;
    ctx->have_bvh = false; ctx->have_bvh2 = false;
    ctx->refit_ready = false; ctx->refit2_ready = false; ctx->bvh2_stale = false;
    PT_HIP(ctx, hipMemcpyAsync(ctx->d_bvh2.ptr, &nn2, 4, hipMemcpyHostToDevice, ctx->stream));
    PT_HIP(ctx, ptk::launch_morton_sort(B, ctx->d_tris9.ptr, n, ctx->stream));
    if (accel == PT_ACCEL_PLOC) {
        uint32_t iterations = 0;
        hipError_t e = ptk::build_ploc_on_device(B, ctx->d_ploc.ptr, ctx->d_tris9.ptr, n, ctx->d_bvh2.ptr, ctx->d_parent.ptr, ctx->d_flags.ptr, &iterations, ctx->stream);
        if (e == hipErrorInvalidValue) return fail(ctx, PT_ERR_BAD_BVH, "pt_build_bvh_accel: a PLOC iteration merged no pair");
        PT_HIP(ctx, e);
        ctx->bvh2_refit_pending = false;
    } else {
        PT_HIP(ctx, ptk::launch_lbvh2(ctx->d_bvh2.ptr, ctx->d_tris9.ptr, ctx->d_morton.ptr, ctx->d_triidx.ptr, ctx->d_parent.ptr, ctx->d_flags.ptr, n,
                                      accel == PT_ACCEL_AREA_COLLAPSE, ctx->stream));
        ctx->bvh2_refit_pending = accel == PT_ACCEL_REFERENCE;
    }
    ctx->num_nodes2 = nn2;
    uint32_t m = 0;
    {
        hipError_t e = ptk::collapse_on_device(B, ctx->d_bvh2.ptr, n, ctx->d_bvh4.ptr, &m, accel != PT_ACCEL_REFERENCE, ctx->stream);
        if (e == hipErrorInvalidValue) return fail(ctx, PT_ERR_BAD_BVH, "pt_build_bvh: the LBVH2 is not a tree of 2N-1 nodes");
        PT_HIP(ctx, e);
    }
    ctx->have_bvh2 = true;
    PT_HIP(ctx, ptk::launch_internal_scan(B, ctx->d_bvh4.ptr, m, ctx->stream));
    uint32_t tail[2] = {0, 0}, root[8];
    PT_HIP(ctx, hipMemcpyAsync(&tail[0], ctx->d_ids.ptr + (m - 1), 4, hipMemcpyDeviceToHost, ctx->stream));
    PT_HIP(ctx, hipMemcpyAsync(&tail[1], ctx->d_subtree.ptr + (m - 1), 4, hipMemcpyDeviceToHost, ctx->stream));
    PT_HIP(ctx, hipMemcpyAsync(root, ctx->d_bvh4.ptr + 1, 32, hipMemcpyDeviceToHost, ctx->stream));
    PT_HIP(ctx, hipStreamSynchronize(ctx->stream));
    const uint32_t internal = tail[0] + tail[1];
    if (int rc = ensure_scene(ctx, n, internal)) return rc;
    PT_HIP(ctx, ptk::launch_wide_nodes(B, ctx->d_bvh4.ptr, m, ctx->wide(), n, uint32_t(ctx->node_off / 16u), ctx->stream));
    PT_HIP(ctx, hipStreamSynchronize(ctx->stream));
    pt::WideBvh meta;
    meta.num_nodes4 = m;
    meta.root_box[0] = root[0]; meta.root_box[1] = root[1]; meta.root_box[2] = root[2];
    meta.root_degenerate = pt::half_to_float(root[0] & 0xffffu) > pt::half_to_float(root[1] >> 16) || pt::half_to_float(root[0] >> 16) > pt::half_to_float(root[2] & 0xffffu) ||
                           pt::half_to_float(root[1] & 0xffffu) > pt::half_to_float(root[2] >> 16);
    meta.root_ref = (root[7] & pt::kLeafFlag) ? pt::packed_leaf_ref(root[7] & 0x7fffffffu, n) : uint32_t(ctx->node_off / 16u);
    ctx->wide_meta = meta;
    ctx->num_nodes4 = m;
    ctx->num_wide = internal; ctx->tree_built = true;
    ctx->have_bvh = true;
    ctx->accum_count = 0;
    return PT_OK;
}

int pt_read_bvh4(PtContext* ctx, uint32_t* dst, uint64_t bytes) {
    if (int rc = bind(ctx)) return rc;
    if (!ctx->have_bvh) return fail(ctx, PT_ERR_NO_SCENE, "pt_read_bvh4: no BVH on the device");
    if (!dst) return fail(ctx, PT_ERR_INVALID_ARG, "pt_read_bvh4: null destination");
    const uint64_t have = 4ull * (1ull + 8ull * ctx->num_nodes4);
    const uint64_t n = bytes < have ? bytes : have;
    PT_HIP(ctx, hipMemcpyAsync(dst, ctx->d_bvh4.ptr, n, hipMemcpyDeviceToHost, ctx->stream));
    PT_HIP(ctx, hipStreamSynchronize(ctx->stream));
    return PT_OK;
}

int pt_set_spheres(PtContext* ctx, const float* xyzr, uint32_t num_spheres) {
    if (int rc = bind(ctx)) return rc;
    if (int rc = flush_pending(ctx)) return rc;
    if (num_spheres && !xyzr) return fail(ctx, PT_ERR_INVALID_ARG, "pt_set_spheres: null spheres");
    PT_HIP(ctx, ctx->d_spheres.ensure(num_spheres));
    if (num_spheres) PT_HIP(ctx, hipMemcpy(ctx->d_spheres.ptr, xyzr, size_t(num_spheres) * 16, hipMemcpyHostToDevice));
    ctx->num_spheres = num_spheres; ctx->accum_count = 0;
    return PT_OK;
}

int pt_scene_info(PtContext* ctx, uint32_t* num_tris, uint32_t* num_nodes2, uint32_t* num_nodes4) {
    if (!ctx) return fail(nullptr, PT_ERR_INVALID_ARG, "null context");
    if (num_tris) *num_tris = ctx->num_tris;
    if (num_nodes2) *num_nodes2 = ctx->have_bvh2 ? ctx->num_nodes2 : 0;
    if (num_nodes4) *num_nodes4 = ctx->have_bvh ? ctx->num_nodes4 : 0;
    return PT_OK;
}


int pt_tile_layout(uint32_t width, uint32_t height, uint32_t tile_rank, uint32_t tile_count, uint32_t* num_tiles, uint64_t* compact_floats) {
    if (tile_count == 0) tile_count = 1;
    if (tile_rank >= tile_count) return fail(nullptr, PT_ERR_INVALID_ARG, "pt_tile_layout: rank >= count");
    const uint32_t n = pt::tile_count_of(width, height, tile_rank, tile_count);
    if (num_tiles) *num_tiles = n;
    if (compact_floats) *compact_floats = uint64_t(n) * 64ull * 4ull;
    return PT_OK;
}

int pt_tile_ids(uint32_t width, uint32_t height, uint32_t tile_rank, uint32_t tile_count, uint32_t* ids, uint32_t capacity, uint32_t* num_tiles) {
    if (tile_count == 0) tile_count = 1;
    if (tile_rank >= tile_count) return fail(nullptr, PT_ERR_INVALID_ARG, "pt_tile_ids: rank >= count");
    std::vector<uint32_t> t; pt::tile_list(width, height, tile_rank, tile_count, t);
    if (num_tiles) *num_tiles = uint32_t(t.size());
    if (ids) {
        if (capacity < t.size()) return fail(nullptr, PT_ERR_INVALID_ARG, "pt_tile_ids: destination too small");
        if (!t.empty()) std::memcpy(ids, t.data(), t.size() * sizeof(uint32_t));
    }
    return PT_OK;
}

int pt_render(PtContext* ctx, const PtRenderParams* p) {
    if (int rc = bind(ctx)) return rc;
    if (!p) return fail(ctx, PT_ERR_INVALID_ARG, "pt_render: null params");
    if (int rc = sync_refit_meta(ctx)) return rc;
    const bool brute = (p->flags & PT_FLAG_BRUTE_FORCE) != 0;
    if (!ctx->have_tris || (!ctx->have_bvh && !brute)) return fail(ctx, PT_ERR_NO_SCENE, "pt_render: scene not set (triangles + BVH)");
    if (brute && p->mode == PT_MODE_REFERENCE_PACKET) return fail(ctx, PT_ERR_INVALID_ARG, "pt_render: brute-force scenes render in modes 1 and 2");
    if (p->width == 0 || p->height == 0 || p->width > 32768 || p->height > 32768) return fail(ctx, PT_ERR_INVALID_ARG, "pt_render: bad resolution");
    if (p->num_tris > ctx->num_tris) return fail(ctx, PT_ERR_INVALID_ARG, "pt_render: num_tris exceeds the uploaded triangle count");
    if (p->mode > PT_MODE_PATH) return fail(ctx, PT_ERR_INVALID_ARG, "pt_render: unknown mode");
    if (p->mode == PT_MODE_PATH && p->spp == 0) return fail(ctx, PT_ERR_INVALID_ARG, "pt_render: spp must be >= 1");
    const uint32_t count = p->tile_count ? p->tile_count : 1;
    if (p->tile_rank >= count) return fail(ctx, PT_ERR_INVALID_ARG, "pt_render: tile_rank >= tile_count");
    if (count > 0xfffu) return fail(ctx, PT_ERR_INVALID_ARG, "pt_render: tile_count > 4095 (the share a running accumulation covers is remembered as 12 + 12 bits; pt_set_accum has the same limit)");
    const bool sharded = count > 1 || (p->flags & PT_FLAG_COMPACT) != 0;
    const bool stats = (p->flags & PT_FLAG_STATS) != 0;

    if (ctx->pending) {
        const ptk::RenderArgs& Q = ctx->pendingA;
        const bool ref = p->mode == PT_MODE_REFERENCE;
        const bool stats_joins = stats && PtTune::pick(ctx->tune.stats_batch, 0u) != 0u && Q.stats != nullptr;
        const bool mega = (p->mode == PT_MODE_PATH || ref) && !(p->flags & PT_FLAG_SIMPLE_KERNEL) && !brute && (!stats || stats_joins);
        const bool same = mega && Q.width == p->width && Q.height == p->height && Q.ref_mode == (ref ? 1u : 0u) && (ref || (Q.spp == p->spp && Q.max_bounces == p->max_bounces)) &&
                          Q.num_tris == p->num_tris && ctx->pending_rank == p->tile_rank && ctx->pending_count == count && (Q.accum != nullptr) == (!ref && p->accumulate != 0);
        if (!same) { if (int rc = flush_pending(ctx)) return rc; }
    }

    ptk::RenderArgs A; std::memset(&A, 0, sizeof(A));
    A.nodes = ctx->wide(); A.tris = ctx->trirec(); A.scene = ctx->d_scene.ptr; A.node_off = uint32_t(ctx->node_off); A.bvh4_ref = ctx->d_bvh4.ptr; A.tris9 = ctx->d_tris9.ptr;
    A.width = p->width; A.height = p->height; A.focal = p->focal; A.aspect = p->aspect;
    std::memcpy(A.cam, p->cam_pos, 12); std::memcpy(A.quat, p->cam_quat, 16);
    A.num_tris = p->num_tris; A.frame = p->frame;
    A.tri_gate = p->num_tris < ctx->num_tris ? (0x80000000u | (4u * p->num_tris)) : 0xFFFFFFFFu;
    A.root_ref = ctx->wide_meta.root_ref; std::memcpy(A.root_box, ctx->wide_meta.root_box, 12);
    A.root_degenerate = ctx->wide_meta.root_degenerate ? 1u : 0u;
    A.spheres = ctx->d_spheres.ptr; A.num_spheres = brute ? ctx->num_spheres : 0u; A.brute = brute ? 1u : 0u;
    A.spp = p->spp; A.max_bounces = p->max_bounces; A.seed = p->seed; A.accumulate = 0; A.compact = sharded ? 1u : 0u;
    A.tiles_x = (p->width + pt::kTile - 1) / pt::kTile;
    const uint32_t tiles_y = (p->height + pt::kTile - 1) / pt::kTile;

    const size_t npx = size_t(p->width) * p->height;
    if (sharded) {
        if (ctx->tiles_w != p->width || ctx->tiles_h != p->height || ctx->tiles_rank != p->tile_rank || ctx->tiles_count != count) {
            pt::tile_list(p->width, p->height, p->tile_rank, count, ctx->tiles_host);
            PT_HIP(ctx, ctx->d_tiles.ensure(ctx->tiles_host.size()));
            if (!ctx->tiles_host.empty())
                PT_HIP(ctx, hipMemcpyAsync(ctx->d_tiles.ptr, ctx->tiles_host.data(), ctx->tiles_host.size() * 4, hipMemcpyHostToDevice, ctx->stream));
            PT_HIP(ctx, hipStreamSynchronize(ctx->stream));
            ctx->tiles_w = p->width; ctx->tiles_h = p->height; ctx->tiles_rank = p->tile_rank; ctx->tiles_count = count;
        }
        A.tiles = ctx->d_tiles.ptr; A.num_tiles = uint32_t(ctx->tiles_host.size());
        ctx->compact_floats = uint64_t(A.num_tiles) * 64ull * 4ull;
        if (ctx->ext_compact) {
            if (ctx->ext_compact_floats < ctx->compact_floats) return fail(ctx, PT_ERR_INVALID_ARG, "pt_render: caller-owned compact buffer too small");
            A.out = ctx->ext_compact;
        } else {
            PT_HIP(ctx, ctx->d_compact.ensure(size_t(A.num_tiles) * 64));
            A.out = ctx->d_compact.ptr;
        }
    } else {
        A.tiles = nullptr; A.num_tiles = A.tiles_x * tiles_y;
        if (ctx->ext_out) {
            if (ctx->ext_out_floats < uint64_t(npx) * 4ull) return fail(ctx, PT_ERR_INVALID_ARG, "pt_render: caller-owned output buffer too small");
            A.out = ctx->ext_out;
        } else {
            PT_HIP(ctx, ctx->d_out.ensure(npx));
            A.out = ctx->d_out.ptr;
        }
        ctx->last_full = A.out;
        ctx->out_w = p->width; ctx->out_h = p->height;
    }
    if (p->mode == PT_MODE_PATH && p->accumulate) {
        DevBuf<float4>& acc = sharded ? ctx->d_compact_accum : ctx->d_accum;
        const size_t need = sharded ? size_t(A.num_tiles) * 64 : npx;
        const uint32_t share_key = accum_share_key(p->tile_rank, count, sharded);
        const bool cont = ctx->accum_count > 0 && ctx->accum_w == p->width && ctx->accum_h == p->height && ctx->accum_rank == share_key && acc.cap >= need;
        PT_HIP(ctx, acc.ensure(need));
        A.accum = acc.ptr; A.accumulate = cont ? 1u : 0u;
        ctx->accum_w = p->width; ctx->accum_h = p->height; ctx->accum_rank = share_key;
        ctx->accum_count = cont ? ctx->accum_count + p->spp : p->spp;
    } else {
        ctx->accum_count = 0;
    }
    const bool mega_ref = p->mode == PT_MODE_REFERENCE && !(p->flags & PT_FLAG_SIMPLE_KERNEL) && !brute;
    const bool mega_path = (p->mode == PT_MODE_PATH && !(p->flags & PT_FLAG_SIMPLE_KERNEL) && !brute) || mega_ref;
    if (mega_ref) { A.ref_mode = 1u; A.spp = 1u; A.max_bounces = 0u; }
    if (stats) {
        if (!mega_path) {
            if (int rc = flush_pending(ctx)) return rc;
            ctx->stats_culled = 0;
            PT_HIP(ctx, hipMemsetAsync(ctx->d_stats.ptr, 0, 24 * sizeof(unsigned long long), ctx->stream));
        }
        A.stats = ctx->d_stats.ptr;
    }
    ctx->last_stats = stats;
    const bool ring = ctx->ring_used + 2 <= ctx->ring.size();
    hipEvent_t e0 = ring ? ctx->ring[ctx->ring_used] : ctx->ev_start, e1 = ring ? ctx->ring[ctx->ring_used + 1] : ctx->ev_stop;
    const int kmode = p->mode == PT_MODE_REFERENCE_PACKET ? PT_KMODE_PACKET : (p->mode == PT_MODE_REFERENCE ? PT_KMODE_REFERENCE : PT_KMODE_PATH);
    if (mega_path) {
        if (uint64_t(A.num_tiles) * A.spp * 64ull * ctx->batch_size > 0xFFFFFFFFull)
// ... 257 lines not shown
    if (int rc = flush_pending(ctx)) return rc;
    PT_HIP(ctx, ptk::launch_occlusion_rays(surfels_device, rays_device, uint32_t(n), params->samples, params->seed, params->index_base, params->bias, ctx->stream));
    return PT_OK;
}

int pt_occlusion_rays_host(const PtSurfel* surfels, uint64_t n, const PtOcclusionParams* params, PtRay* rays) {
    if (int rc = check_occlusion_params(nullptr, "pt_occlusion_rays_host", n, params)) return rc;
    if (n && (!surfels || !rays)) return fail(nullptr, PT_ERR_INVALID_ARG, "pt_occlusion_rays_host: null pointer");
    pt::occlusion_rays(reinterpret_cast<const float*>(surfels), n, params->samples, params->seed, params->index_base, params->bias, reinterpret_cast<float*>(rays));
    return PT_OK;
}

int pt_hit_surfels(PtContext* ctx, const void* rays_device, const void* hits_device, uint64_t n, float r_max, void* surfels_device) {
    if (int rc = bind(ctx)) return rc;
    if (n > 0xFFFFFFFFull) return fail(ctx, PT_ERR_INVALID_ARG, "pt_hit_surfels: more than 2^32 - 1 rays");
    if (!aligned16(rays_device) || !aligned16(hits_device) || !aligned16(surfels_device))
        return fail(ctx, PT_ERR_INVALID_ARG, "pt_hit_surfels: rays, hits and surfels must be non-null and 16-byte aligned");
    if (!ctx->have_tris) return fail(ctx, PT_ERR_NO_SCENE, "pt_hit_surfels: no triangles set");
    if (int rc = flush_pending(ctx)) return rc;
    if (n == 0) return PT_OK;
    ptk::RenderArgs A; std::memset(&A, 0, sizeof(A));
    A.tris = ctx->trirec(); A.num_tris = ctx->num_tris;
    PT_HIP(ctx, ptk::launch_hit_surfels(A, rays_device, hits_device, uint32_t(n), r_max, surfels_device, ctx->stream));
    return PT_OK;
}

int pt_hit_surfels_host(PtContext* ctx, const PtRay* rays, const PtHit* hits, uint64_t n, float r_max, PtSurfel* out) {
    if (int rc = bind(ctx)) return rc;
    if (n > 0xFFFFFFFFull) return fail(ctx, PT_ERR_INVALID_ARG, "pt_hit_surfels_host: more than 2^32 - 1 rays");
    if (!aligned16(rays) || !aligned16(hits) || !aligned16(out))
        return fail(ctx, PT_ERR_INVALID_ARG, "pt_hit_surfels_host: rays, hits and surfels must be non-null and 16-byte aligned");
    if (!ctx->have_tris) return fail(ctx, PT_ERR_NO_SCENE, "pt_hit_surfels_host: no triangles set");
    if (int rc = flush_pending(ctx)) return rc;
    if (n == 0) return PT_OK;
    PT_HIP(ctx, ctx->d_rq_rays.ensure(size_t(n) * 2)); PT_HIP(ctx, ctx->d_rq_hits.ensure(size_t(n))); PT_HIP(ctx, ctx->d_oc_surfels.ensure(size_t(n) * 2));
    PT_HIP(ctx, hipMemcpyAsync(ctx->d_rq_rays.ptr, rays, size_t(n) * sizeof(PtRay), hipMemcpyHostToDevice, ctx->stream));
    PT_HIP(ctx, hipMemcpyAsync(ctx->d_rq_hits.ptr, hits, size_t(n) * sizeof(PtHit), hipMemcpyHostToDevice, ctx->stream));
    ptk::RenderArgs A; std::memset(&A, 0, sizeof(A));
    A.tris = ctx->trirec(); A.num_tris = ctx->num_tris;
    PT_HIP(ctx, ptk::launch_hit_surfels(A, ctx->d_rq_rays.ptr, ctx->d_rq_hits.ptr, uint32_t(n), r_max, ctx->d_oc_surfels.ptr, ctx->stream));
    PT_HIP(ctx, hipMemcpyAsync(out, ctx->d_oc_surfels.ptr, size_t(n) * sizeof(PtSurfel), hipMemcpyDeviceToHost, ctx->stream));
    PT_HIP(ctx, hipStreamSynchronize(ctx->stream));
    return PT_OK;
}

int pt_set_batch(PtContext* ctx, uint32_t frames_per_launch) {
    if (int rc = bind(ctx)) return rc;
    if (int rc = flush_pending(ctx)) return rc;
    if (frames_per_launch < 1u || frames_per_launch > PT_MAX_BATCH) return fail(ctx, PT_ERR_INVALID_ARG, "pt_set_batch: 1..256 frames per launch");
    ctx->batch_size = frames_per_launch;
    return PT_OK;
}

int pt_flush(PtContext* ctx) {
    if (int rc = bind(ctx)) return rc;
    return flush_pending(ctx);
}

int pt_timing_begin(PtContext* ctx, uint32_t capacity) {
    if (int rc = bind(ctx)) return rc;
    while (ctx->ring.size() < size_t(capacity) * 2) {
        hipEvent_t e = nullptr;
        PT_HIP(ctx, hipEventCreate(&e));
        ctx->ring.push_back(e);
    }
    while (ctx->ring.size() > size_t(capacity) * 2) { (void)hipEventDestroy(ctx->ring.back()); ctx->ring.pop_back(); }
    ctx->ring_used = 0;
    return PT_OK;
}

int pt_timing_collect_spans(PtContext* ctx, float* start_ms, float* dur_ms, uint32_t capacity, uint32_t* count) {
    if (int rc = bind(ctx)) return rc;
    if (int rc = flush_pending(ctx)) return rc;
    PT_HIP(ctx, hipStreamSynchronize(ctx->stream));
    const uint32_t n = ctx->ring_used / 2;
    uint32_t got = 0;
    for (uint32_t i = 0; i < n && i < capacity; ++i, ++got) {
        if (dur_ms) PT_HIP(ctx, hipEventElapsedTime(&dur_ms[i], ctx->ring[2 * i], ctx->ring[2 * i + 1]));
        if (start_ms) { start_ms[i] = 0.0f; if (i) PT_HIP(ctx, hipEventElapsedTime(&start_ms[i], ctx->ring[0], ctx->ring[2 * i])); }
    }
    if (count) *count = got;
    for (hipEvent_t e : ctx->ring) (void)hipEventDestroy(e);
    ctx->ring.clear(); ctx->ring_used = 0;
    return PT_OK;
}

int pt_timing_collect(PtContext* ctx, float* ms, uint32_t capacity, uint32_t* count) {
    return pt_timing_collect_spans(ctx, nullptr, ms, capacity, count);
}

int pt_last_render_ms(PtContext* ctx, float* ms) {
    if (int rc = bind(ctx)) return rc;
    if (int rc = flush_pending(ctx)) return rc;
    if (!ms) return fail(ctx, PT_ERR_INVALID_ARG, "pt_last_render_ms: null output");
    if (!ctx->timed) return fail(ctx, PT_ERR_NO_SCENE, "pt_last_render_ms: nothing rendered yet");
    PT_HIP(ctx, hipEventSynchronize(ctx->ev_stop));
    PT_HIP(ctx, hipEventElapsedTime(ms, ctx->ev_start, ctx->ev_stop));
    return PT_OK;
}

int pt_get_stats(PtContext* ctx, PtStats* out) {
    if (int rc = bind(ctx)) return rc;
    if (int rc = flush_pending(ctx)) return rc;
    if (!out) return fail(ctx, PT_ERR_INVALID_ARG, "pt_get_stats: null output");
    if (!ctx->last_stats) return fail(ctx, PT_ERR_NO_SCENE, "pt_get_stats: last render did not run with PT_FLAG_STATS");
    unsigned long long h[8];
    PT_HIP(ctx, hipMemcpyAsync(h, ctx->d_stats.ptr, sizeof(h), hipMemcpyDeviceToHost, ctx->stream));
    PT_HIP(ctx, hipStreamSynchronize(ctx->stream));
    out->rays_closest = h[0]; out->rays_shadow = h[1]; out->nodes_examined = h[2]; out->tris_tested = h[3];
    out->stack_drops = h[4]; out->max_stack = h[5]; out->samples = h[6];
    if (ctx->stats_culled) {
        out->rays_closest += ctx->stats_culled; out->nodes_examined += ctx->stats_culled; out->samples += ctx->stats_culled;
        if (out->max_stack < 1u) out->max_stack = 1u;
    }
    return PT_OK;
}

int pt_debug_set_tune(PtContext* ctx, const char* name, uint32_t value) {
    if (int rc = bind(ctx)) return rc;
    if (int rc = flush_pending(ctx)) return rc;
    uint32_t* knob = name ? ctx->tune.find(name) : nullptr;
    if (!knob) return fail(ctx, PT_ERR_INVALID_ARG, "pt_debug_set_tune: unknown knob");
    *knob = value;
    return PT_OK;
}

int pt_debug_launch_plan(uint32_t num_cus, uint32_t frames, uint32_t tile_count, uint32_t launches_in_flight, uint32_t traced_batches, uint32_t batch_size, uint32_t out[12]) {
    if (!out || frames == 0u) return fail(nullptr, PT_ERR_INVALID_ARG, "pt_debug_launch_plan: bad arguments");
    PlanInput in; std::memset(&in, 0, sizeof(in));
    in.num_cus = num_cus; in.frames = frames; in.tile_count = tile_count ? tile_count : 1u; in.sharded = in.tile_count > 1u; in.stats = false;
    in.launches_in_flight = launches_in_flight; in.traced_batches = traced_batches; in.batch_size = batch_size ? batch_size : 1u;
    const LaunchPlan P = plan_launch(PtTune(), in);
    if (P.error) return fail(nullptr, PT_ERR_INVALID_ARG, P.error);
    const uint32_t v[12] = {P.grid, P.perm_rows, P.perm_cols, P.total_items, P.chunk_items, P.xcd_span, P.shade_threshold, P.fill_threshold, P.quad_live, P.fork_shadow,
                            uint32_t(P.slots), uint32_t(P.setup_slots)};
    std::memcpy(out, v, sizeof v);
    return PT_OK;
}

int pt_debug_counters(PtContext* ctx, unsigned long long* dst24) {
    if (int rc = bind(ctx)) return rc;
    PT_HIP(ctx, hipMemcpy(dst24, ctx->d_stats.ptr, 24 * sizeof(unsigned long long), hipMemcpyDeviceToHost));
    return PT_OK;
}

int pt_debug_wave_times(PtContext* ctx, unsigned long long* dst, uint32_t max_waves, uint32_t* n_waves) {
    if (int rc = bind(ctx)) return rc;
    const uint32_t n = ctx->wave_times_n < max_waves ? ctx->wave_times_n : max_waves;
    if (n) PT_HIP(ctx, hipMemcpy(dst, ctx->d_wave_times.ptr, size_t(n) * ptk::kWaveTimeWords * 8u, hipMemcpyDeviceToHost));
    if (n_waves) *n_waves = n;
    return PT_OK;
}

int pt_read_radiance(PtContext* ctx, float* dst, uint64_t dst_floats) {
    if (int rc = bind(ctx)) return rc;
    if (int rc = flush_pending(ctx)) return rc;
    if (!dst) return fail(ctx, PT_ERR_INVALID_ARG, "pt_read_radiance: null destination");
    const uint64_t need = uint64_t(ctx->out_w) * ctx->out_h * 4;
    if (need == 0) return fail(ctx, PT_ERR_NO_SCENE, "pt_read_radiance: no full-frame result (render with tile_count <= 1 or call pt_deinterleave)");
    if (dst_floats < need) return fail(ctx, PT_ERR_INVALID_ARG, "pt_read_radiance: destination too small");
    PT_HIP(ctx, hipMemcpyAsync(dst, ctx->last_full, need * 4, hipMemcpyDeviceToHost, ctx->stream));
    PT_HIP(ctx, hipStreamSynchronize(ctx->stream));
    return PT_OK;
}

int pt_read_rgba8(PtContext* ctx, uint8_t* dst, uint64_t dst_bytes) {
    if (int rc = bind(ctx)) return rc;
    if (int rc = flush_pending(ctx)) return rc;
    const uint64_t npx = uint64_t(ctx->out_w) * ctx->out_h;
    if (npx == 0) return fail(ctx, PT_ERR_NO_SCENE, "pt_read_rgba8: no full-frame result");
    if (!dst || dst_bytes < npx * 4) return fail(ctx, PT_ERR_INVALID_ARG, "pt_read_rgba8: destination too small");
    PT_HIP(ctx, ctx->d_u32tmp.ensure(npx));
    PT_HIP(ctx, ptk::launch_rgba8(ctx->last_full, ctx->d_u32tmp.ptr, uint32_t(npx), ctx->stream));
    PT_HIP(ctx, hipMemcpyAsync(dst, ctx->d_u32tmp.ptr, npx * 4, hipMemcpyDeviceToHost, ctx->stream));
    PT_HIP(ctx, hipStreamSynchronize(ctx->stream));
    return PT_OK;
}

int pt_read_tonemapped(PtContext* ctx, int from_rgba8, uint8_t* dst, uint64_t dst_bytes) {
    if (int rc = bind(ctx)) return rc;
    if (int rc = flush_pending(ctx)) return rc;
    const uint64_t npx = uint64_t(ctx->out_w) * ctx->out_h;
    if (npx == 0) return fail(ctx, PT_ERR_NO_SCENE, "pt_read_tonemapped: no full-frame result");
    if (!dst || dst_bytes < npx * 4) return fail(ctx, PT_ERR_INVALID_ARG, "pt_read_tonemapped: destination too small");
    PT_HIP(ctx, ctx->d_u32tmp.ensure(npx));
    PT_HIP(ctx, ptk::launch_tonemap(ctx->last_full, ctx->d_u32tmp.ptr, ctx->out_w, ctx->out_h, from_rgba8, ctx->stream));
    PT_HIP(ctx, hipMemcpyAsync(dst, ctx->d_u32tmp.ptr, npx * 4, hipMemcpyDeviceToHost, ctx->stream));
    PT_HIP(ctx, hipStreamSynchronize(ctx->stream));
    return PT_OK;
}

int pt_accum_info(PtContext* ctx, PtAccumInfo* out) {
    if (int rc = bind(ctx)) return rc;
    if (int rc = flush_pending(ctx)) return rc;
    if (!out) return fail(ctx, PT_ERR_INVALID_ARG, "pt_accum_info: null output");
    std::memset(out, 0, sizeof(*out));
    if (ctx->accum_count == 0) return PT_OK;
    out->width = ctx->accum_w; out->height = ctx->accum_h;
    out->tile_rank = ctx->accum_rank & 0xfffu; out->tile_count = (ctx->accum_rank >> 12) & 0xfffu; out->compact = ctx->accum_rank >> 31;
    out->samples = ctx->accum_count;
    out->floats = out->compact ? uint64_t(pt::tile_count_of(out->width, out->height, out->tile_rank, out->tile_count)) * 256ull : uint64_t(out->width) * out->height * 4ull;
    return PT_OK;
}

int pt_read_accum(PtContext* ctx, float* dst, uint64_t dst_floats) {
    PtAccumInfo info;
    if (int rc = pt_accum_info(ctx, &info)) return rc;
    if (info.samples == 0) return fail(ctx, PT_ERR_NO_SCENE, "pt_read_accum: no running accumulation (render with accumulate = 1 first)");
    if (info.floats == 0) return PT_OK;
    if (!dst || dst_floats < info.floats) return fail(ctx, PT_ERR_INVALID_ARG, "pt_read_accum: destination too small (pt_accum_info gives the size)");
    const DevBuf<float4>& acc = info.compact ? ctx->d_compact_accum : ctx->d_accum;
    PT_HIP(ctx, hipMemcpyAsync(dst, acc.ptr, info.floats * sizeof(float), hipMemcpyDeviceToHost, ctx->stream));
    PT_HIP(ctx, hipStreamSynchronize(ctx->stream));
    if (info.compact && ((info.width | info.height) & 7u)) {
        std::vector<uint32_t> tiles; pt::tile_list(info.width, info.height, info.tile_rank, info.tile_count ? info.tile_count : 1u, tiles);
        const uint32_t tiles_x = (info.width + 7u) / 8u;
        for (size_t slot = 0; slot < tiles.size(); ++slot) {
            const uint32_t x0 = (tiles[slot] % tiles_x) * 8u, y0 = (tiles[slot] / tiles_x) * 8u;
            if (x0 + 8u <= info.width && y0 + 8u <= info.height) continue;
            for (uint32_t p = 0; p < 64u; ++p)
                if (x0 + (p & 7u) >= info.width || y0 + (p >> 3) >= info.height) std::memset(dst + (slot * 64u + p) * 4u, 0, 4 * sizeof(float));
        }
    }
    return PT_OK;
}

int pt_set_accum(PtContext* ctx, const PtAccumInfo* info, const float* src) {
    if (int rc = bind(ctx)) return rc;
    if (int rc = flush_pending(ctx)) return rc;
    if (!info || !src) return fail(ctx, PT_ERR_INVALID_ARG, "pt_set_accum: null argument");
    const uint32_t count = info->tile_count ? info->tile_count : 1u;
    if (info->width == 0 || info->height == 0 || info->width > 32768 || info->height > 32768 || info->tile_rank >= count || count > 0xfffu || info->samples == 0)
        return fail(ctx, PT_ERR_INVALID_ARG, "pt_set_accum: bad shape (resolution, tile share or a sample count of 0)");
    const bool compact = info->compact != 0 || count > 1u;
    const uint64_t need = compact ? uint64_t(pt::tile_count_of(info->width, info->height, info->tile_rank, count)) * 256ull : uint64_t(info->width) * info->height * 4ull;
    if (info->floats != need) return fail(ctx, PT_ERR_INVALID_ARG, "pt_set_accum: `floats` does not match the shape (whole frame: W*H*4; tile share: tiles*64*4)");
    DevBuf<float4>& acc = compact ? ctx->d_compact_accum : ctx->d_accum;
    if (need == 0) {
        ctx->accum_w = info->width; ctx->accum_h = info->height; ctx->accum_rank = accum_share_key(info->tile_rank, count, compact); ctx->accum_count = info->samples;
        return PT_OK;
    }
    const uint64_t last_w = compact ? need - 256u + 3u : need - 1u;
    if (src[3] != float(info->samples) || src[last_w] != float(info->samples))
        return fail(ctx, PT_ERR_INVALID_ARG, "pt_set_accum: `samples` does not match the sample count stored in the data (w of the first / last pixel)");
    PT_HIP(ctx, hipStreamSynchronize(ctx->stream));
    everything_delivered(ctx);
    PT_HIP(ctx, acc.ensure(size_t(need / 4u)));
    PT_HIP(ctx, hipMemcpyAsync(acc.ptr, src, need * sizeof(float), hipMemcpyHostToDevice, ctx->stream));
    PT_HIP(ctx, hipStreamSynchronize(ctx->stream));
    ctx->accum_w = info->width; ctx->accum_h = info->height; ctx->accum_rank = accum_share_key(info->tile_rank, count, compact); ctx->accum_count = info->samples;
    return PT_OK;
}

int pt_set_compact_buffer(PtContext* ctx, void* device_ptr, uint64_t floats) {
    if (int rc = bind(ctx)) return rc;
    if (!device_ptr) {
        if (int rc = flush_pending(ctx)) return rc;
        PT_HIP(ctx, hipStreamSynchronize(ctx->stream));
    }
    ctx->ext_compact = (float4*)device_ptr;
    ctx->ext_compact_floats = device_ptr ? floats : 0;
    return PT_OK;
}

int pt_set_output_buffer(PtContext* ctx, void* device_ptr, uint64_t floats) {
    if (int rc = bind(ctx)) return rc;
    if (!device_ptr) {
        if (int rc = flush_pending(ctx)) return rc;
        PT_HIP(ctx, hipStreamSynchronize(ctx->stream));
    }
    ctx->ext_out = (float4*)device_ptr;
    ctx->ext_out_floats = device_ptr ? floats : 0;
    return PT_OK;
}

int pt_compact_radiance(PtContext* ctx, void** device_ptr, uint64_t* floats) {
    if (int rc = bind(ctx)) return rc;
    if (int rc = flush_pending(ctx)) return rc;
    if (ctx->compact_floats == 0 || !(ctx->ext_compact || ctx->d_compact.ptr)) return fail(ctx, PT_ERR_NO_SCENE, "pt_compact_radiance: no tile-sharded render yet");
    if (device_ptr) *device_ptr = ctx->ext_compact ? (void*)ctx->ext_compact : (void*)ctx->d_compact.ptr;
    if (floats) *floats = ctx->compact_floats;
    return PT_OK;
}

static uint32_t max_share_tiles(PtContext* ctx, uint32_t width, uint32_t height, uint32_t count) {
    if (ctx->share_w != width || ctx->share_h != height || ctx->share_count != count) {
        uint32_t m = 0;
        for (uint32_t r = 0; r < count; ++r) m = std::max(m, pt::tile_count_of(width, height, r, count));
        ctx->share_w = width; ctx->share_h = height; ctx->share_count = count; ctx->share_max_tiles = m;
    }
    return ctx->share_max_tiles;
}

int pt_deinterleave_batch(PtContext* ctx, const void* gathered_device, uint64_t rank_stride_floats, uint64_t frame_stride_floats, uint32_t num_frames,
                          uint32_t width, uint32_t height, uint32_t tile_count, void* frames_out_device, uint64_t out_stride_floats) {
    if (int rc = bind(ctx)) return rc;
    if (int rc = flush_pending(ctx)) return rc;
    if (!gathered_device || tile_count == 0 || num_frames == 0 || (rank_stride_floats & 3) || (frame_stride_floats & 3) || (out_stride_floats & 3) || width == 0 || height == 0)
        return fail(ctx, PT_ERR_INVALID_ARG, "pt_deinterleave_batch: bad arguments");
    const uint64_t share = uint64_t(max_share_tiles(ctx, width, height, tile_count)) * 256ull;
    if (share > frame_stride_floats && num_frames > 1u) return fail(ctx, PT_ERR_INVALID_ARG, "pt_deinterleave_batch: frame stride smaller than a rank's compact buffer");
    if (share + uint64_t(num_frames - 1u) * frame_stride_floats > rank_stride_floats) return fail(ctx, PT_ERR_INVALID_ARG, "pt_deinterleave_batch: rank stride smaller than the frames of one rank");
    const size_t npx = size_t(width) * height;
    float4* out = (float4*)frames_out_device; uint64_t out_stride_px = out_stride_floats / 4u;
    if (out) {
        if (num_frames > 1u && out_stride_px < npx) return fail(ctx, PT_ERR_INVALID_ARG, "pt_deinterleave_batch: output stride smaller than a frame");
// ... 117 lines not shown
```

raytracer-public_amd/csrc/pt_kernels.h:

```cpp
#pragma once
#include <hip/hip_runtime.h>
#include <stdint.h>

#define PT_KMODE_PACKET    0
#define PT_KMODE_REFERENCE 1
#define PT_KMODE_PATH      2

#ifndef PT_SHORT_STACK
#define PT_SHORT_STACK 12
#endif
#ifndef PT_MEGA_WAVES_PER_SIMD
#define PT_MEGA_WAVES_PER_SIMD 6
#endif
#ifndef PT_FRAME_SLOTS
#define PT_FRAME_SLOTS 3
#endif
#ifndef PT_MEGA_BLOCK
#define PT_MEGA_BLOCK 64
#endif
#ifndef PT_SHADE_THRESHOLD
#define PT_SHADE_THRESHOLD 16
#endif
#ifndef PT_QUAD
#define PT_QUAD 1
// ... 12 lines not shown
#endif
#ifndef PT_RQ_WAVES_PER_SIMD
#define PT_RQ_WAVES_PER_SIMD 6
#endif
#ifndef PT_RQ_FILL
#define PT_RQ_FILL 8
#endif
#ifndef PT_PQ_SHORT_STACK
#define PT_PQ_SHORT_STACK 12
#endif
#ifndef PT_PQ_WAVES_PER_SIMD
#define PT_PQ_WAVES_PER_SIMD 6
#endif
#ifndef PT_PQ_FILL
#define PT_PQ_FILL 8
#endif
#ifndef PT_OC_SHORT_STACK
#define PT_OC_SHORT_STACK 12
#endif
#ifndef PT_OC_WAVES_PER_SIMD
#define PT_OC_WAVES_PER_SIMD 6
#endif
#ifndef PT_OC_FILL
#define PT_OC_FILL 8
#endif
#ifndef PT_FILL_THRESHOLD
#define PT_FILL_THRESHOLD 4
#endif

namespace ptk {

constexpr uint32_t kWaveTimeWords = 24;
#define PT_MAX_BATCH 256
struct FrameParams {
    float cam[3]; float focal;
    float quat[4];
    float aspect; uint32_t frame; uint32_t seed;
    uint32_t accum_mode;
};
constexpr int kFrameChunk = 32;
struct FrameChunk { FrameParams f[kFrameChunk]; float4* o[kFrameChunk]; };

struct RenderArgs {
    const uint4*  nodes;
    const float4* tris;
    const uint4*  scene;
    uint32_t      node_off;
    uint32_t      rcp_short;
    uint32_t      tri_gate;
    const uint32_t* bvh4_ref;
    const float*    tris9;
    float4*   out;
    float4*   accum;
    uint32_t* tri_ids;
    const float4* spheres;
    uint32_t num_spheres, brute;
    const uint32_t* tiles;
    unsigned long long* stats;
    uint32_t num_tiles, tiles_x;
    uint32_t width, height; float focal, aspect;
    float cam[3]; uint32_t num_tris;
    float quat[4];
    uint32_t frame;
    uint32_t root_ref; uint32_t root_box[3]; uint32_t root_degenerate;
    uint32_t spp, max_bounces, seed, accumulate, compact;
    float4*   samples;
    uint32_t* queue;
    uint2*    spill;
    uint4*    raybuf;
    unsigned long long* wave_times;
    const uint32_t* trace_slots; uint32_t num_trace_tiles;
    uint32_t  trace_rect[4];
    uint32_t  trace_bpf, trace_bpf_magic;
    uint32_t  spp_magic, tiles_x_magic;
    uint32_t  num_sample_batches;
    uint32_t  total_items, chunk_items;
    uint32_t  xcd_span;
    uint32_t  num_batches, perm_cols;
    uint32_t  perm_rows, perm_rows_magic;
    uint32_t  shade_threshold, fill_threshold;
    uint32_t  fork_shadow;
    uint32_t  quad_live;
    const FrameParams* frames; float4* const* outs;
    uint32_t  num_frames, batches_per_frame;
    uint32_t  prime;
    uint32_t  ref_mode;
};

hipError_t launch_render(const RenderArgs& args, int kmode, bool stats, hipStream_t stream);
hipError_t launch_trace(const RenderArgs& args, bool stats, uint32_t grid_blocks, hipStream_t stream, hipEvent_t k0, hipEvent_t k1);
hipError_t launch_prime(uint32_t* queue, hipStream_t stream);
hipError_t launch_frame_params(const FrameParams* frames, float4* const* outs, uint32_t n, FrameParams* d_frames, float4** d_outs, hipStream_t stream);
hipError_t launch_resolve(const RenderArgs& args, hipStream_t stream);
uint32_t megakernel_grid(int num_cus);
uint32_t megakernel_block();
hipError_t launch_lbvh2(uint32_t* bvh2, const float* tris9, const uint32_t* morton, const uint32_t* tri_index,
                        uint32_t* parent, uint32_t* flags, uint32_t num_tris, bool refit, hipStream_t stream);
hipError_t launch_lbvh2_refit(uint32_t* bvh2, const uint32_t* parent, uint32_t* flags, uint32_t num_tris, hipStream_t stream);
hipError_t launch_lbvh2_leaves(uint32_t* bvh2, const float* tris9, const uint32_t* tri_index, const uint32_t* parent, uint32_t* flags, uint32_t num_tris, hipStream_t stream);
constexpr int kBuildCounters = 256;
struct BuildBuffers {
    unsigned long long* bounds;
    uint32_t* counters;
    uint32_t *code_tmp, *index_tmp;
    uint32_t *morton, *tri_index;
    void* temp; size_t temp_bytes;
    uint32_t* node2; uint4* child_pos; uint32_t *subtree, *ids, *bnd;
    uint32_t* host_word;
};
size_t build_temp_bytes(uint32_t num_tris);
hipError_t launch_tri_records(const float* tris9, uint32_t num_tris, float4* records, uint32_t* edge_max, hipStream_t stream);
hipError_t launch_morton_sort(const BuildBuffers& B, const float* tris9, uint32_t num_tris, hipStream_t stream);
hipError_t collapse_on_device(const BuildBuffers& B, const uint32_t* bvh2, uint32_t num_tris, uint32_t* bvh4, uint32_t* num_nodes4, bool by_area, hipStream_t stream);
size_t ploc_words(uint32_t num_tris);
size_t ploc_temp_bytes(uint32_t num_tris);
hipError_t build_ploc_on_device(const BuildBuffers& B, uint32_t* ploc, const float* tris9, uint32_t num_tris, uint32_t* bvh2, uint32_t* parent, uint32_t* flags,
                                uint32_t* iterations, hipStream_t stream);
hipError_t launch_internal_scan(const BuildBuffers& B, const uint32_t* bvh4, uint32_t num_nodes4, hipStream_t stream);
hipError_t launch_wide_nodes(const BuildBuffers& B, const uint32_t* bvh4, uint32_t num_nodes4, uint4* wide, uint32_t num_tris, uint32_t node_base16, hipStream_t stream);
hipError_t launch_deinterleave(const float4* gathered, uint64_t rank_stride_px, uint64_t frame_stride_px, uint32_t frames, float4* full, uint64_t full_stride_px,
                               uint32_t width, uint32_t height, uint32_t count, hipStream_t stream);
hipError_t launch_pack_shares(const float4* compact, uint64_t frame_stride_px, uint32_t frames, float* packed, uint64_t packed_stride_floats, uint32_t width,
                              uint32_t rank, uint32_t count, const uint32_t rect[4], hipStream_t stream);
hipError_t launch_unpack_frames(const float* gathered, uint64_t rank_stride_floats, uint64_t frame_stride_floats, uint32_t frames, float4* full, uint64_t full_stride_px,
                                uint32_t width, uint32_t height, uint32_t count, const uint32_t rect[4], uint32_t spp, hipStream_t stream);
constexpr uint32_t kRqQueueWords = 256;
uint32_t rayquery_grid(int num_cus);
size_t rayquery_spill_entries(uint32_t grid);
hipError_t launch_trace_rays(const RenderArgs& A, const void* rays, void* hits, uint32_t n, bool anyhit, bool simple, bool stats,
                             unsigned long long* queue, unsigned long long* spill, uint32_t grid, hipStream_t stream);
hipError_t launch_camera_rays(const RenderArgs& A, void* rays, hipStream_t stream);
uint32_t pointquery_grid(int num_cus);
size_t pointquery_spill_entries(uint32_t grid);
hipError_t launch_closest_points(const RenderArgs& A, const void* points, void* out, uint32_t n, bool simple, bool stats, bool brute,
                                 unsigned long long* queue, unsigned long long* spill, uint32_t grid, hipStream_t stream);
uint32_t occlusion_grid(int num_cus);
size_t occlusion_spill_entries(uint32_t grid);
hipError_t launch_occlusion(const RenderArgs& A, const void* surfels, void* out, uint32_t n, uint32_t samples, uint32_t seed, uint32_t index_base, float bias,
                            bool simple, bool stats, unsigned long long* queue, unsigned long long* spill, uint32_t grid, hipStream_t stream);
hipError_t launch_occlusion_rays(const void* surfels, void* rays, uint32_t n, uint32_t samples, uint32_t seed, uint32_t index_base, float bias, hipStream_t stream);
hipError_t launch_hit_surfels(const RenderArgs& A, const void* rays, const void* hits, uint32_t n, float r_max, void* surfels, hipStream_t stream);
constexpr uint32_t kRefitLeaf = 0x80000000u, kRefitDead = 0xFFFFFFFFu;
struct RefitBuffers {
    uint2* up;
    uint2* self;
    uint4* child_ref;
    uint32_t* arrive;
};
hipError_t launch_refit_prepare4(const uint32_t* bvh4, uint32_t num_nodes4, const uint32_t* wide_index, uint32_t num_tris, uint32_t node_base16, const RefitBuffers& R, hipStream_t stream);
hipError_t launch_refit4(const float* tris9, uint32_t num_tris, uint32_t* bvh4, uint32_t num_nodes4, const RefitBuffers& R, uint4* wide, hipStream_t stream);
hipError_t launch_refit_prepare2(const uint32_t* bvh2, uint32_t nn2, uint32_t* parent2, hipStream_t stream);
hipError_t launch_refit2(const float* tris9, uint32_t num_tris, uint32_t* bvh2, uint32_t nn2, const uint32_t* parent2, uint32_t* arrive, hipStream_t stream);
hipError_t launch_bvh_cost(const uint32_t* bvh4, uint32_t num_nodes4, const uint2* self, double* out, hipStream_t stream);
hipError_t launch_rgba8(const float4* src, uint32_t* dst, uint32_t n, hipStream_t stream);
hipError_t launch_tonemap(const float4* src, uint32_t* dst, uint32_t width, uint32_t height, int from_rgba8, hipStream_t stream);

}
```

raytracer-public_amd/csrc/pt_megakernel.hip:

```cpp
#include <hip/hip_runtime.h>
#include <stdint.h>

#include "pt_kernels.h"
#include "pt_device.h"

namespace ptk {

#ifndef PT_TAIL_PRIORITY
#define PT_TAIL_PRIORITY 3
#endif
#define PT_TAIL_PRIO do { if (PT_TAIL_PRIORITY) __builtin_amdgcn_s_setprio(PT_TAIL_PRIORITY); } while (0)
constexpr int kShort = PT_SHORT_STACK;
constexpr uint32_t kPhaseIdle = 0, kPhaseTrav = 1, kPhaseDone = 2, kPhaseWait = 3;
struct Lane {
    F3 o, d, inv;
    RaySel sel;
    float best_t; uint32_t best_tri;
    uint32_t cur; int sp;
    F3 T, rad;
    F3 d_next, contrib;
    uint32_t key, item;
    uint32_t bounce;
};

// ... 98 lines not shown
        if (!slab(r, A.root_box[0], A.root_box[1], A.root_box[2], kInfT, troot)) return false;
        if (STATS && count_lane()) ++c_enter;
        S.cur = A.root_ref;
        S.sel = ray_selectors(S.inv);
        return true;
    };

    uint4* const rb = A.raybuf + ((size_t)blockIdx.x * (PT_MEGA_BLOCK / 64) + wave) * (64 * 3);
    uint32_t rb_next = 0, rb_count = 0;
    auto source_dry = [&]() __attribute__((always_inline)) -> bool { return queue_empty && rb_next == rb_count; };
    auto claim_chunk = [&]() __attribute__((always_inline)) {
        if (A.xcd_span != 0u) {
            for (;;) {
                const uint32_t qi = (xcc + xcd_hop) & 7u;
                const uint32_t q_begin = qi * A.xcd_span;
                const uint32_t q_end = min(q_begin + A.xcd_span, total_items);
                uint32_t start = 0;
                if (lane == 0) start = atomicAdd(A.queue + 8 + qi, chunk_items);
                start = __builtin_amdgcn_readfirstlane(start);
                if (q_begin < q_end && start < q_end - q_begin) { chunk_next = q_begin + start; chunk_end = min(chunk_next + chunk_items, q_end); break; }
                if (++xcd_hop == 8u) { queue_empty = true; PT_TAIL_PRIO; if (TIMELINE) tl_event(1, 6, 8, 15); break; }
            }
        } else {
            uint32_t start = 0;
            if (lane == 0) start = atomicAdd(A.queue, chunk_items);
            start = __builtin_amdgcn_readfirstlane(start);
            if (start >= total_items) { queue_empty = true; PT_TAIL_PRIO; if (TIMELINE) tl_event(1, 6, 8, 15); }
            else { chunk_next = start; chunk_end = min(start + chunk_items, total_items); }
        }
    };
    auto shade_due = [&](unsigned long long m_live) __attribute__((always_inline)) -> uint32_t {
        if (!source_dry()) return A.shade_threshold;
        const uint32_t q = (uint32_t)__popcll(m_live) >> 2;
        return q < 1u ? 1u : (q < A.shade_threshold ? q : A.shade_threshold);
    };
    bool want_reseat = false;
    auto reseat = [&]() __attribute__((always_inline)) {
        const unsigned long long m_live = __ballot(phase != kPhaseIdle);
        const uint32_t n_live = (uint32_t)__popcll(m_live);
        uint32_t srcl = lane;
        {
            unsigned long long m = m_live; uint32_t r = 0u;
            while (m != 0ull) {
                const uint32_t l = (uint32_t)__builtin_ctzll(m); m &= m - 1ull;
                srcl = ((lane >> 2) == r) ? l : srcl;
                ++r;
            }
        }
        const bool seated = (lane >> 2) < n_live;
        const int sa = (int)(srcl << 2);
        auto gu = [&](uint32_t v) __attribute__((always_inline)) -> uint32_t { return (uint32_t)__builtin_amdgcn_ds_bpermute(sa, (int)v); };
        auto gf = [&](float v) __attribute__((always_inline)) -> float { return __uint_as_float(gu(__float_as_uint(v))); };
        auto g3 = [&](F3 v) __attribute__((always_inline)) -> F3 { return f3(gf(v.x), gf(v.y), gf(v.z)); };
        S.o = g3(S.o); S.d = g3(S.d); S.inv = g3(S.inv); S.sel = ray_selectors(S.inv);
        S.best_t = gf(S.best_t); S.best_tri = gu(S.best_tri); S.cur = gu(S.cur); S.sp = (int)gu((uint32_t)S.sp);
        S.T = g3(S.T); S.rad = g3(S.rad); S.d_next = g3(S.d_next); S.contrib = g3(S.contrib);
        S.key = gu(S.key); S.item = gu(S.item); S.bounce = gu(S.bounce);
        if (PT_FORK_LANES) {
            if (S.bounce & kPendBit) {
                const uint32_t old_lane = S.bounce >> kChildShift;
                const uint32_t new_quad = (uint32_t)__popcll(m_live & ((1ull << old_lane) - 1ull));
                S.bounce = (S.bounce & ((1u << kChildShift) - 1u)) | ((new_quad << 2) << kChildShift);
            }
        }
        phase = gu(phase);
        if (STATS) { path_steps = gu(path_steps); ray_steps = gu(ray_steps); path_shadow_steps = gu(path_shadow_steps); }
        col = (wave << 6) | srcl;
        if (!seated) {
            phase = kPhaseIdle;
            const uint32_t used = (uint32_t)(m_live >> (lane & 60u)) & 15u;
            col = used == 15u ? kNoCol : ((wave << 6) | ((lane & 60u) + (uint32_t)__builtin_ctz(~used & 15u)));
        }
        if (STATS) { ++n_reseated; cy_step_reseat = cy_step; }
        if (TIMELINE) tl_event(16, 17, 18, -1);
    };
    bool want_stage_b = false;
    if (PT_QUAD != 2) {
#define PT_LOOP_QUAD 0
#define PT_LOOP_STAGE 0
#define PT_LOOP_FORK false
#include "pt_megakernel_loop.inc"
#undef PT_LOOP_FORK
#undef PT_LOOP_STAGE
        if (want_stage_b) {
#define PT_LOOP_STAGE 1
#define PT_LOOP_FORK true
#include "pt_megakernel_loop.inc"
#undef PT_LOOP_FORK
#undef PT_LOOP_STAGE
        }
#undef PT_LOOP_QUAD
    }
    if (PT_QUAD == 2 || want_reseat) {
        if (want_reseat) reseat();
        quad_now = true;
#define PT_LOOP_QUAD 1
#define PT_LOOP_STAGE 1
#define PT_LOOP_FORK (A.fork_shadow != 0u)
#include "pt_megakernel_loop.inc"
#undef PT_LOOP_FORK
#undef PT_LOOP_STAGE
#undef PT_LOOP_QUAD
    }
    if (TIMELINE) {
        if (lane == 0) {
            unsigned long long* w = A.wave_times + ((size_t)blockIdx.x * (PT_MEGA_BLOCK / 64) + wave) * kWaveTimeWords;
            w[2] = wall_clock64(); w[3] = n_iter; w[4] = n_shade; w[5] = n_fill; w[7] = lanes_sum; w[9] = leaf_lanes;
            w[20] = (unsigned long long)INSTR;
            if (STATS) { w[10] = cy_shade; w[11] = cy_fill; w[12] = cy_step; w[13] = cy_step_q; w[19] = cy_step_reseat; }
        }
    }
    if (STATS) {
        if (A.wave_times) {
            unsigned long long* w = A.wave_times + ((size_t)blockIdx.x * (PT_MEGA_BLOCK / 64) + wave) * kWaveTimeWords;
            atomicMax(&w[14], (unsigned long long)max_path_steps_post);
        }
        atomicMax(&A.stats[12], (unsigned long long)max_path_steps); atomicMax(&A.stats[13], (unsigned long long)max_ray_steps);
        atomicAdd(&A.stats[14], (unsigned long long)long_paths); atomicAdd(&A.stats[15], (unsigned long long)longer_paths);
        if (lane == 0) { atomicAdd(&A.stats[22], wait_seat_iters); atomicAdd(&A.stats[23], live_seat_iters); }
        atomicAdd(&A.stats[17], long_shadow_steps); atomicAdd(&A.stats[18], long_total_steps);
        atomicAdd(&A.stats[19], (unsigned long long)n_fork); atomicAdd(&A.stats[20], (unsigned long long)n_fork_none); atomicAdd(&A.stats[21], (unsigned long long)n_fork_wait);
        if (lane == 0) atomicAdd(&A.stats[16], (unsigned long long)n_reseated);
        atomicAdd(&A.stats[7], ((unsigned long long)c_enter << 1) + ((lane == 0 && blockIdx.x == 0 && wave == 0 && BOUNDED) ? 1ull : 0ull));
        atomicAdd(&A.stats[8], (unsigned long long)push_ops); atomicAdd(&A.stats[9], (unsigned long long)push8_ops);
        atomicAdd(&A.stats[10], (unsigned long long)push12_ops); atomicAdd(&A.stats[11], (unsigned long long)spill_ops);
        atomicAdd(&A.stats[0], (unsigned long long)c_closest);
        atomicAdd(&A.stats[1], (unsigned long long)c_shadow);
        atomicAdd(&A.stats[2], (unsigned long long)c_nodes);
        atomicAdd(&A.stats[3], (unsigned long long)c_tris);
        atomicAdd(&A.stats[4], (unsigned long long)c_drops);
        atomicMax(&A.stats[5], (unsigned long long)c_maxstack);
        atomicAdd(&A.stats[6], (unsigned long long)c_samples);
    }
}

template <bool ACCUM>
#ifndef PT_RESOLVE_BLOCK
#define PT_RESOLVE_BLOCK 64
#endif
__global__ __launch_bounds__(PT_RESOLVE_BLOCK) void resolve_kernel(const RenderArgs A) {
    const uint32_t idx = blockIdx.x * blockDim.x + threadIdx.x;
    const uint32_t slot = idx >> 6, p = idx & 63u;
    if (idx == 0u && blockIdx.y == 0u) { for (int k = 0; k < 16; ++k) A.queue[k] = 0u; }
    if (slot >= A.num_tiles) return;
    const uint32_t tile = A.tiles ? A.tiles[slot] : slot;
    const uint32_t tx = tile % A.tiles_x, ty = tile / A.tiles_x;
    const uint32_t px = tx * 8u + (p & 7u), py = ty * 8u + (p >> 3);
    if (px >= A.width || py >= A.height) return;
    const size_t out_index = A.compact ? (size_t)idx : ((size_t)py * A.width + px);
    const float bg = 0.0f + 1.0f * kBgPrimary;
    const FrameParams* const frames = A.frames;
    float4* const* const outs = A.outs;
    const uint32_t f_begin = ACCUM ? 0u : blockIdx.y, f_end = ACCUM ? A.num_frames : blockIdx.y + 1u;
    const bool untraced = A.trace_slots != nullptr && !(tx >= A.trace_rect[0] && tx < A.trace_rect[1] && ty >= A.trace_rect[2] && ty < A.trace_rect[3]);
    for (uint32_t fid = f_begin; fid < f_end; ++fid) {
        F3 sum = f3(0.0f, 0.0f, 0.0f);
        float4* const sp = A.samples + (((size_t)fid * A.batches_per_frame + (size_t)slot * A.spp) * 64u + p);
        if (untraced) {
            if (!ACCUM && (frames[fid].accum_mode & 0x100u)) continue;
            for (uint32_t s = 0; s < A.spp; ++s) sum = sum + f3(bg, bg, bg);
        } else {
        if (!ACCUM) {
            if (frames[fid].accum_mode & 0x100u) continue;
        }
        for (uint32_t s0 = 0; s0 < A.spp; s0 += 4u) {
            const uint32_t n = min(4u, A.spp - s0);
            float4 v[4];
#pragma unroll
            for (uint32_t j = 0; j < 4u; ++j) v[j] = (j < n) ? sp[(size_t)(s0 + j) * 64u] : make_float4(0.0f, 0.0f, 0.0f, 0.0f);
#pragma unroll
            for (uint32_t j = 0; j < 4u; ++j) if (j < n) sum = sum + f3(v[j].x, v[j].y, v[j].z);
        }
        }
        float count = (float)A.spp;
        if (ACCUM) {
            const uint32_t am = frames[fid].accum_mode & 0xffu;
            const float4 acc = (am == 2u) ? A.accum[out_index] : make_float4(0.0f, 0.0f, 0.0f, 0.0f);
            sum = f3(acc.x + sum.x, acc.y + sum.y, acc.z + sum.z);
            count = acc.w + count;
            A.accum[out_index] = make_float4(sum.x, sum.y, sum.z, count);
        }
        const float inv = 1.0f / count;
        outs[fid][out_index] = make_float4(sum.x * inv, sum.y * inv, sum.z * inv, 1.0f);
    }
}

hipError_t launch_trace(const RenderArgs& A, bool stats, uint32_t grid_blocks, hipStream_t stream, hipEvent_t k0, hipEvent_t k1) {
    hipError_t e = hipSuccess;
    if (A.total_items == 0u) {
        if (k0) { e = hipEventRecord(k0, stream); if (e != hipSuccess) return e; }
        if (k1) { e = hipEventRecord(k1, stream); if (e != hipSuccess) return e; }
        return hipSuccess;
    }
    if (A.prime) {
        e = hipMemsetAsync(A.queue, 0, 16 * sizeof(uint32_t), stream);
        if (e != hipSuccess) return e;
    }
    if (k0) { e = hipEventRecord(k0, stream); if (e != hipSuccess) return e; }
    if (stats)               { if (A.rcp_short) hipLaunchKernelGGL((trace_paths_kernel<1, true>), dim3(grid_blocks), dim3(PT_MEGA_BLOCK), 0, stream, A);
                               else             hipLaunchKernelGGL((trace_paths_kernel<1, false>), dim3(grid_blocks), dim3(PT_MEGA_BLOCK), 0, stream, A); }
    else if (A.wave_times)   { if (A.rcp_short) hipLaunchKernelGGL((trace_paths_kernel<2, true>), dim3(grid_blocks), dim3(PT_MEGA_BLOCK), 0, stream, A);
                               else             hipLaunchKernelGGL((trace_paths_kernel<2, false>), dim3(grid_blocks), dim3(PT_MEGA_BLOCK), 0, stream, A); }
    else                     { if (A.rcp_short) hipLaunchKernelGGL((trace_paths_kernel<0, true>), dim3(grid_blocks), dim3(PT_MEGA_BLOCK), 0, stream, A);
                               else             hipLaunchKernelGGL((trace_paths_kernel<0, false>), dim3(grid_blocks), dim3(PT_MEGA_BLOCK), 0, stream, A); }
    e = hipGetLastError(); if (e != hipSuccess) return e;
    if (k1) { e = hipEventRecord(k1, stream); if (e != hipSuccess) return e; }
    return hipSuccess;
}

hipError_t launch_resolve(const RenderArgs& A, hipStream_t stream) {
    if (A.num_tiles == 0u || A.num_frames == 0u) return hipSuccess;
    const uint32_t n = A.num_tiles * 64u;
    const uint32_t rb = PT_RESOLVE_BLOCK;
    if (A.accum) hipLaunchKernelGGL(resolve_kernel<true>, dim3((n + rb - 1u) / rb, 1), dim3(rb), 0, stream, A);
    else         hipLaunchKernelGGL(resolve_kernel<false>, dim3((n + rb - 1u) / rb, A.num_frames), dim3(rb), 0, stream, A);
    return hipGetLastError();
}

__global__ void write_frame_params_kernel(const FrameChunk c, FrameParams* d_frames, float4** d_outs, uint32_t offset, uint32_t n) {
    const uint32_t i = threadIdx.x;
    if (i < n) { d_frames[offset + i] = c.f[i]; d_outs[offset + i] = c.o[i]; }
}

hipError_t launch_frame_params(const FrameParams* frames, float4* const* outs, uint32_t n, FrameParams* d_frames, float4** d_outs, hipStream_t stream) {
    for (uint32_t off = 0; off < n; off += (uint32_t)kFrameChunk) {
        FrameChunk c;
        const uint32_t m = n - off < (uint32_t)kFrameChunk ? n - off : (uint32_t)kFrameChunk;
        for (uint32_t i = 0; i < m; ++i) { c.f[i] = frames[off + i]; c.o[i] = outs[off + i]; }
        for (uint32_t i = m; i < (uint32_t)kFrameChunk; ++i) { c.f[i] = frames[off]; c.o[i] = nullptr; }
        hipLaunchKernelGGL(write_frame_params_kernel, dim3(1), dim3(kFrameChunk), 0, stream, c, d_frames, d_outs, off, m);
        const hipError_t e = hipGetLastError(); if (e != hipSuccess) return e;
    }
    return hipSuccess;
}

hipError_t launch_prime(uint32_t* queue, hipStream_t stream) {
    return hipMemsetAsync(queue, 0, 16 * sizeof(uint32_t), stream);
}

uint32_t megakernel_grid(int num_cus) { return (uint32_t)num_cus * PT_MEGA_WAVES_PER_SIMD * (256 / PT_MEGA_BLOCK); }
uint32_t megakernel_block() { return PT_MEGA_BLOCK; }


}
```

Before: 12110 Msamples/s.

## Cull untraced tiles using projected BVH cut coverage mask

Builds a cut of up to a few thousand BVH4 child boxes once per tree. Each launch projects those boxes through the frame cameras on a high-priority side stream to build a per-tile coverage bitmask, which is cached per camera set. Tiles whose 8x8 region no projected box can touch are dropped from the traced list, and resolve writes background for them instead of tracing rays. The cost is a host-synchronous cover computation whenever a new camera set appears, plus a slightly larger trace-slot upload and an extra mask lookup in resolve.

```diff
diff --git a/include/mi355pt.h b/include/mi355pt.h
--- a/include/mi355pt.h
+++ b/include/mi355pt.h
@@ -223,6 +223,7 @@
 PT_API int pt_debug_launch_plan(uint32_t num_cus, uint32_t frames, uint32_t tile_count, uint32_t launches_in_flight, uint32_t traced_batches, uint32_t batch_size, uint32_t out[12]);
 PT_API int pt_debug_counters(PtContext* ctx, unsigned long long* dst24);
 PT_API int pt_debug_wave_times(PtContext* ctx, unsigned long long* dst, uint32_t max_waves, uint32_t* n_waves);
+PT_API int pt_debug_traced_tiles(PtContext* ctx, const PtRenderParams* params, uint32_t* bitmask_out, uint32_t words, uint32_t* rect_tiles, uint32_t* traced_tiles);
 
 #ifdef __cplusplus
 }
diff --git a/raytracer-public_amd/__init__.py b/raytracer-public_amd/__init__.py
--- a/raytracer-public_amd/__init__.py
+++ b/raytracer-public_amd/__init__.py
@@ -99,7 +99,7 @@
     "pt_group_build_bvh_accel",
     "pt_group_set_bvh2", "pt_group_set_bvh4", "pt_group_set_batch", "pt_group_render", "pt_group_flush", "pt_group_synchronize", "pt_group_read_radiance",
     "pt_group_read_rgba8", "pt_group_read_tonemapped",
-    "pt_debug_set_tune", "pt_debug_counters", "pt_debug_wave_times", "pt_debug_launch_plan",
+    "pt_debug_set_tune", "pt_debug_counters", "pt_debug_wave_times", "pt_debug_launch_plan", "pt_debug_traced_tiles",
 ]
 
 
@@ -499,6 +499,14 @@
 
     def debug_set_tune(self, name, value=None):
         self._ck(lib.pt_debug_set_tune(self.h, name.encode(), C.c_uint32(0xFFFFFFFF if value is None else value)))
+
+    def debug_traced_tiles(self, params):
+        tx, ty = (params.width + 7) // 8, (params.height + 7) // 8
+        words = (tx * ty + 31) // 32
+        bits = np.zeros(words, np.uint32); nr = C.c_uint32(); nt = C.c_uint32()
+        self._ck(lib.pt_debug_traced_tiles(self.h, C.byref(params), _p(bits, C.c_uint32), C.c_uint32(words), C.byref(nr), C.byref(nt)))
+        mask = np.unpackbits(bits.view(np.uint8), bitorder="little")[: tx * ty].astype(bool).reshape(ty, tx)
+        return mask, nr.value, nt.value
 
     def timing_collect_spans(self, capacity):
         st = np.zeros(capacity, np.float32); ms = np.zeros(capacity, np.float32); n = C.c_uint32()
diff --git a/raytracer-public_amd/csrc/pt_api.cpp b/raytracer-public_amd/csrc/pt_api.cpp
--- a/raytracer-public_amd/csrc/pt_api.cpp
+++ b/raytracer-public_amd/csrc/pt_api.cpp
@@ -85,6 +85,17 @@
     DevBuf<double> d_cost;
     bool bvh2_stale = false;
     uint32_t* h_refit = nullptr; hipEvent_t ev_refit = nullptr; bool meta_pending = false, meta_has_root = false;
+    DevBuf<uint32_t> d_cut; uint32_t cut_count = 0, tree_version = 0;
+    hipStream_t cover_stream = nullptr; DevBuf<uint32_t> d_cover; uint32_t* h_cover = nullptr; size_t h_cover_cap = 0;
+    struct Cover {
+        bool valid = false, computed = false, usable = false;
+        uint32_t tree_version = 0, width = 0, height = 0, id = 0; uint64_t used = 0;
+        std::vector<ptk::CoverCam> cams; std::vector<uint32_t> mask;
+    };
+    static constexpr int kCovers = 4;
+    Cover covers[kCovers]; uint64_t cover_clock = 0;
+    std::vector<ptk::CoverCam> cover_cams;
+    uint32_t cover_ids = 0;
     DevBuf<unsigned long long> d_rq_queue, d_rq_spill; DevBuf<uint4> d_rq_rays, d_rq_hits;
     DevBuf<uint4> d_oc_surfels;
 
@@ -95,7 +106,7 @@
         uint64_t resolved_seq = 0;
         DevBuf<uint32_t> queue; DevBuf<float4> samples; DevBuf<uint2> spill; DevBuf<uint4> rays;
         DevBuf<uint32_t> trace_slots; uint32_t* h_trace = nullptr; size_t h_trace_cap = 0; hipEvent_t trace_copied = nullptr;
-        uint32_t cull_key[8] = {0, 0, 0, 0, 0, 0, 0, 0}; uint32_t num_trace_tiles = 0; bool cull_valid = false;
+        uint32_t cull_key[9] = {0, 0, 0, 0, 0, 0, 0, 0, 0}; uint32_t num_trace_tiles = 0; bool cull_valid = false;
         DevBuf<ptk::FrameParams> frame_params; DevBuf<float4*> frame_outs;
         const void* primed_ptr = nullptr; size_t primed_samples = 0;
     };
@@ -211,6 +222,19 @@
     return PT_OK;
 }
 
+int install_cut(PtContext* ctx) {
+    ++ctx->tree_version; ctx->cut_count = 0;
+    const uint32_t base16 = uint32_t(ctx->node_off / 16u), root = ctx->wide_meta.root_ref;
+    if (root == pt::kInvalid || (root & pt::kLeafFlag) || ctx->num_wide == 0u || root < base16) return PT_OK;
+    PT_HIP(ctx, ctx->d_cut.ensure(ptk::kCutMax + 1u));
+    if (!ctx->h_word) PT_HIP(ctx, hipHostMalloc((void**)&ctx->h_word, 64, hipHostMallocDefault));
+    PT_HIP(ctx, ptk::launch_tile_cut(ctx->wide(), ctx->num_wide, base16, (root - base16) / 4u, ctx->d_cut.ptr, ctx->stream));
+    PT_HIP(ctx, hipMemcpyAsync(ctx->h_word, ctx->d_cut.ptr + ptk::kCutMax, 4, hipMemcpyDeviceToHost, ctx->stream));
+    PT_HIP(ctx, hipStreamSynchronize(ctx->stream));
+    ctx->cut_count = std::min(ctx->h_word[0], ptk::kCutMax);
+    return PT_OK;
+}
+
 int upload_wide(PtContext* ctx, const uint32_t* bvh4, uint64_t words) {
     pt::WideBvh w; std::string err;
     if (int rc = sync_refit_meta(ctx)) return rc;
@@ -227,7 +251,7 @@
     w.nodes.clear(); w.nodes.shrink_to_fit();
     ctx->wide_meta = w;
     ctx->have_bvh = true;
-    return PT_OK;
+    return install_cut(ctx);
 }
 
 struct TileRect { uint32_t tx0, ty0, tx1, ty1; };
@@ -329,21 +353,95 @@
     return P;
 }
 
-bool traced_tiles(const PtContext* ctx, const ptk::RenderArgs& A, uint32_t nf, bool sharded, TileRect& rect, std::vector<uint32_t>& traced) {
-    traced.clear(); rect = {0, 0, 0, 0};
-    if (!(ctx->have_bvh && ctx->wide_meta.root_ref != pt::kInvalid && !ctx->wide_meta.root_degenerate && A.num_tris != 0u && ctx->tune.cull != 0u)) return false;
+bool launch_rect(const PtContext* ctx, const ptk::FrameParams* frames, uint32_t nf, uint32_t width, uint32_t height, uint32_t num_tris, TileRect& rect) {
+    rect = {0, 0, 0, 0};
+    if (!(ctx->have_bvh && ctx->wide_meta.root_ref != pt::kInvalid && !ctx->wide_meta.root_degenerate && num_tris != 0u && ctx->tune.cull != 0u)) return false;
     for (uint32_t i = 0; i < nf; ++i) {
         TileRect r;
-        if (!root_box_rect(ctx->wide_meta, ctx->pending_frames[i], A.width, A.height, r)) return false;
+        if (!root_box_rect(ctx->wide_meta, frames[i], width, height, r)) return false;
         if (i == 0) rect = r;
         else { rect.tx0 = std::min(rect.tx0, r.tx0); rect.ty0 = std::min(rect.ty0, r.ty0); rect.tx1 = std::max(rect.tx1, r.tx1); rect.ty1 = std::max(rect.ty1, r.ty1); }
     }
+    return true;
+}
+bool traced_tiles(const PtContext* ctx, const ptk::RenderArgs& A, uint32_t nf, bool sharded, const uint32_t* cover, TileRect& rect, std::vector<uint32_t>& traced) {
+    traced.clear();
+    if (!launch_rect(ctx, ctx->pending_frames.data(), nf, A.width, A.height, A.num_tris, rect)) return false;
     const uint32_t tiles_y = (A.height + pt::kTile - 1) / pt::kTile;
-    if (rect.tx0 == 0u && rect.ty0 == 0u && rect.tx1 >= A.tiles_x && rect.ty1 >= tiles_y) return false;
-    auto inside = [&](uint32_t tile) { const uint32_t tx = tile % A.tiles_x, ty = tile / A.tiles_x; return tx >= rect.tx0 && tx < rect.tx1 && ty >= rect.ty0 && ty < rect.ty1; };
+    if (!cover && rect.tx0 == 0u && rect.ty0 == 0u && rect.tx1 >= A.tiles_x && rect.ty1 >= tiles_y) return false;
+    auto inside = [&](uint32_t tile) {
+        const uint32_t tx = tile % A.tiles_x, ty = tile / A.tiles_x;
+        return tx >= rect.tx0 && tx < rect.tx1 && ty >= rect.ty0 && ty < rect.ty1 && (!cover || ((cover[tile >> 5] >> (tile & 31u)) & 1u));
+    };
     if (sharded) { for (uint32_t sl = 0; sl < A.num_tiles; ++sl) if (inside(ctx->tiles_host[sl])) traced.push_back(sl); }
-    else { for (uint32_t ty = rect.ty0; ty < rect.ty1; ++ty) for (uint32_t tx = rect.tx0; tx < rect.tx1; ++tx) traced.push_back(ty * A.tiles_x + tx); }
+    else {
+        for (uint32_t ty = rect.ty0; ty < rect.ty1; ++ty) for (uint32_t tx = rect.tx0; tx < rect.tx1; ++tx) {
+            const uint32_t tile = ty * A.tiles_x + tx;
+            if (!cover || ((cover[tile >> 5] >> (tile & 31u)) & 1u)) traced.push_back(tile);
+        }
+    }
     return true;
+}
+
+int tile_cover(PtContext* ctx, const ptk::FrameParams* frames, uint32_t nf, uint32_t width, uint32_t height, uint32_t num_tris, bool now, const uint32_t** mask, uint32_t* id) {
+    *mask = nullptr; *id = 0u;
+    if (ctx->cut_count == 0u || nf == 0u) return PT_OK;
+    TileRect rect;
+    if (!launch_rect(ctx, frames, nf, width, height, num_tris, rect)) return PT_OK;
+    std::vector<ptk::CoverCam>& cams = ctx->cover_cams;
+    cams.clear();
+    for (uint32_t i = 0; i < nf; ++i) {
+        ptk::CoverCam c; std::memset(&c, 0, sizeof c);
+        std::memcpy(c.cam, frames[i].cam, 12); c.focal = frames[i].focal; std::memcpy(c.quat, frames[i].quat, 16); c.aspect = frames[i].aspect;
+        bool seen = false;
+        for (size_t k = cams.size(); k-- > 0 && !seen;) seen = std::memcmp(&cams[k], &c, sizeof c) == 0;
+        if (!seen) cams.push_back(c);
+    }
+    PtContext::Cover* found = nullptr; PtContext::Cover* victim = &ctx->covers[0];
+    for (PtContext::Cover& c : ctx->covers) {
+        if (c.valid && c.tree_version == ctx->tree_version && c.width == width && c.height == height && c.cams.size() == cams.size() &&
+            std::memcmp(c.cams.data(), cams.data(), cams.size() * sizeof(ptk::CoverCam)) == 0) { found = &c; break; }
+        if (!c.valid || (victim->valid && c.used < victim->used)) victim = &c;
+    }
+    PtContext::Cover& cv = found ? *found : *victim;
+    cv.used = ++ctx->cover_clock;
+    if (!found) {
+        cv.valid = true; cv.computed = false; cv.usable = false;
+        cv.cams = cams; cv.tree_version = ctx->tree_version; cv.width = width; cv.height = height;
+        if (!now) return PT_OK;
+    }
+    if (!cv.computed) {
+        if (int rc = sync_refit_meta(ctx)) return rc;
+        const uint32_t tiles = ((width + pt::kTile - 1) / pt::kTile) * ((height + pt::kTile - 1) / pt::kTile), words = (tiles + 31u) / 32u;
+        if (!ctx->cover_stream) {
+            int lo = 0, hi = 0;
+            (void)hipDeviceGetStreamPriorityRange(&lo, &hi);
+            PT_HIP(ctx, hipStreamCreateWithPriority(&ctx->cover_stream, hipStreamNonBlocking, hi));
+        }
+        PT_HIP(ctx, ctx->d_cover.ensure(words + 1u));
+        if (ctx->h_cover_cap < words + 1u) {
+            if (ctx->h_cover) (void)hipHostFree(ctx->h_cover);
+            ctx->h_cover = nullptr; ctx->h_cover_cap = 0;
+            PT_HIP(ctx, hipHostMalloc((void**)&ctx->h_cover, (size_t(words) + 1u) * sizeof(uint32_t), hipHostMallocDefault));
+            ctx->h_cover_cap = words + 1u;
+        }
+        cv.valid = false;
+        PT_HIP(ctx, hipMemsetAsync(ctx->d_cover.ptr, 0, (size_t(words) + 1u) * sizeof(uint32_t), ctx->cover_stream));
+        for (size_t first = 0; first < cams.size(); first += ptk::kCoverCams) {
+            ptk::CoverCams group; std::memset(&group, 0, sizeof group);
+            const uint32_t n = uint32_t(std::min<size_t>(ptk::kCoverCams, cams.size() - first));
+            std::memcpy(group.c, cams.data() + first, n * sizeof(ptk::CoverCam));
+            PT_HIP(ctx, ptk::launch_tile_cover(ctx->wide(), ctx->d_cut.ptr, ctx->cut_count, group, n, width, height, ctx->d_cover.ptr, words, ctx->cover_stream));
+        }
+        PT_HIP(ctx, hipMemcpyAsync(ctx->h_cover, ctx->d_cover.ptr, (size_t(words) + 1u) * sizeof(uint32_t), hipMemcpyDeviceToHost, ctx->cover_stream));
+        PT_HIP(ctx, hipStreamSynchronize(ctx->cover_stream));
+        cv.mask.assign(ctx->h_cover, ctx->h_cover + words);
+        cv.usable = ctx->h_cover[words] == 0u;
+        cv.id = ++ctx->cover_ids; if (cv.id == 0u) cv.id = ++ctx->cover_ids;
+        cv.valid = true; cv.computed = true;
+    }
+    if (cv.usable) { *mask = cv.mask.data(); *id = cv.id; }
+    return PT_OK;
 }
 
 int prepare_slots(PtContext* ctx, const LaunchPlan& P, const ptk::RenderArgs& A, uint32_t nf, bool stats) {
@@ -373,18 +471,21 @@
     return PT_OK;
 }
 
-int stage_traced_tiles(PtContext* ctx, PtContext::FrameSlot& sl, const uint32_t key[8], const std::vector<uint32_t>& traced) {
-    if (sl.cull_valid && std::memcmp(key, sl.cull_key, 8 * sizeof(uint32_t)) == 0) return PT_OK;
+int stage_traced_tiles(PtContext* ctx, PtContext::FrameSlot& sl, const uint32_t key[9], const std::vector<uint32_t>& traced, const uint32_t* cover, uint32_t words) {
+    if (sl.cull_valid && std::memcmp(key, sl.cull_key, 9 * sizeof(uint32_t)) == 0) return PT_OK;
     if (!sl.trace_copied) PT_HIP(ctx, hipEventCreateWithFlags(&sl.trace_copied, hipEventDisableTiming));
     else PT_HIP(ctx, hipEventSynchronize(sl.trace_copied));
-    if (sl.h_trace_cap < traced.size()) {
+    const size_t need = traced.size() + words;
+    if (sl.h_trace_cap < need) {
         if (sl.h_trace) (void)hipHostFree(sl.h_trace);
         sl.h_trace = nullptr; sl.h_trace_cap = 0;
-        PT_HIP(ctx, hipHostMalloc((void**)&sl.h_trace, std::max<size_t>(traced.size(), 1024) * sizeof(uint32_t), hipHostMallocDefault));
-        sl.h_trace_cap = std::max<size_t>(traced.size(), 1024);
-    }
-    PT_HIP(ctx, sl.trace_slots.ensure(std::max<size_t>(traced.size(), 1)));
+        PT_HIP(ctx, hipHostMalloc((void**)&sl.h_trace, std::max<size_t>(need, 1024) * sizeof(uint32_t), hipHostMallocDefault));
+        sl.h_trace_cap = std::max<size_t>(need, 1024);
+    }
+    PT_HIP(ctx, sl.trace_slots.ensure(std::max<size_t>(need, 1)));
     if (!traced.empty()) std::memcpy(sl.h_trace, traced.data(), traced.size() * sizeof(uint32_t));
+    if (cover) std::memcpy(sl.h_trace + traced.size(), cover, size_t(words) * sizeof(uint32_t));
+    else std::memset(sl.h_trace + traced.size(), 0xff, size_t(words) * sizeof(uint32_t));
     sl.cull_valid = false;
     return PT_OK;
 }
@@ -404,7 +505,12 @@
 
     std::vector<uint32_t> traced;
     TileRect rect;
-    const bool cull = traced_tiles(ctx, A, nf, sharded, rect, traced);
+    const bool cover_now = uint64_t(A.num_tiles) * 64u * A.spp * nf * (uint64_t(A.max_bounces) + 1u) >= (1ull << 24);
+    const uint32_t* cover = nullptr; uint32_t cover_id = 0u;
+    if (!stats && PtTune::pick(ctx->tune.timeline, 0u) == 0u && PtTune::pick(ctx->tune.cull, 2u) >= 2u) {
+        if (int rc = tile_cover(ctx, ctx->pending_frames.data(), nf, A.width, A.height, A.num_tris, cover_now, &cover, &cover_id)) return rc;
+    }
+    const bool cull = traced_tiles(ctx, A, nf, sharded, cover, rect, traced);
     A.num_trace_tiles = cull ? uint32_t(traced.size()) : A.num_tiles;
     ctx->stats_culled = 0;
     if (stats && cull) {
@@ -439,8 +545,9 @@
     A.prime = stats ? 1u : 0u;
     A.samples = sl.samples.ptr; A.queue = sl.queue.ptr; A.spill = sl.spill.ptr; A.raybuf = sl.rays.ptr;
     A.trace_slots = nullptr;
-    const uint32_t cull_key[8] = {rect.tx0, rect.ty0, rect.tx1, rect.ty1, A.width, A.height, ctx->pending_rank | (ctx->pending_count << 16), A.num_trace_tiles};
-    if (cull) { if (int rc = stage_traced_tiles(ctx, sl, cull_key, traced)) return rc; }
+    const uint32_t cull_key[9] = {rect.tx0, rect.ty0, rect.tx1, rect.ty1, A.width, A.height, ctx->pending_rank | (ctx->pending_count << 16), A.num_trace_tiles, cover_id};
+    const uint32_t cover_words = (A.tiles_x * ((A.height + pt::kTile - 1) / pt::kTile) + 31u) / 32u;
+    if (cull) { if (int rc = stage_traced_tiles(ctx, sl, cull_key, traced, cover, cover_words)) return rc; }
     const bool timeline = !stats && PtTune::pick(ctx->tune.timeline, 0u) != 0u;
     if (stats || timeline) {
         const uint32_t stat_waves = P.grid * ptk::megakernel_block() / 64u;
@@ -452,7 +559,7 @@
     if (sl.used) PT_HIP(ctx, hipStreamWaitEvent(sl.side, sl.resolved, 0));
     if (cull) {
         if (!sl.cull_valid) {
-            if (!traced.empty()) PT_HIP(ctx, hipMemcpyAsync(sl.trace_slots.ptr, sl.h_trace, traced.size() * sizeof(uint32_t), hipMemcpyHostToDevice, sl.side));
+            PT_HIP(ctx, hipMemcpyAsync(sl.trace_slots.ptr, sl.h_trace, (traced.size() + cover_words) * sizeof(uint32_t), hipMemcpyHostToDevice, sl.side));
             PT_HIP(ctx, hipEventRecord(sl.trace_copied, sl.side));
             std::memcpy(sl.cull_key, cull_key, sizeof cull_key); sl.cull_valid = true; sl.num_trace_tiles = A.num_trace_tiles;
         }
@@ -552,6 +659,9 @@
     ctx->d_refit_parent2.release(); ctx->d_refit_arrive2.release(); ctx->d_cost.release();
     if (ctx->h_refit) (void)hipHostFree(ctx->h_refit);
     if (ctx->ev_refit) (void)hipEventDestroy(ctx->ev_refit);
+    if (ctx->cover_stream) { (void)hipStreamSynchronize(ctx->cover_stream); (void)hipStreamDestroy(ctx->cover_stream); }
+    ctx->d_cut.release(); ctx->d_cover.release();
+    if (ctx->h_cover) (void)hipHostFree(ctx->h_cover);
     for (auto& sl : ctx->slots) {
         sl.queue.release(); sl.samples.release(); sl.spill.release(); sl.rays.release(); sl.trace_slots.release();
         if (sl.h_trace) (void)hipHostFree(sl.h_trace);
@@ -794,6 +904,7 @@
     if (tree) {
         PT_HIP(ctx, ptk::launch_refit4(ctx->d_tris9.ptr, num_tris, ctx->d_bvh4.ptr, ctx->num_nodes4, refit_buffers(ctx), ctx->wide(), ctx->stream));
         PT_HIP(ctx, hipMemcpyAsync(ctx->h_refit, ctx->d_bvh4.ptr + 1, 12, hipMemcpyDeviceToHost, ctx->stream));
+        ++ctx->tree_version;
     }
     PT_HIP(ctx, hipMemcpyAsync(ctx->h_refit + 3, ctx->d_edge_max.ptr, 4, hipMemcpyDeviceToHost, ctx->stream));
     PT_HIP(ctx, hipEventRecord(ctx->ev_refit, ctx->stream));
@@ -966,7 +1077,7 @@
     ctx->num_wide = internal; ctx->tree_built = true;
     ctx->have_bvh = true;
     ctx->accum_count = 0;
-    return PT_OK;
+    return install_cut(ctx);
 }
 
 int pt_read_bvh4(PtContext* ctx, uint32_t* dst, uint64_t bytes) {
@@ -1530,6 +1641,42 @@
     return PT_OK;
 }
 
+int pt_debug_traced_tiles(PtContext* ctx, const PtRenderParams* p, uint32_t* bitmask_out, uint32_t words, uint32_t* rect_tiles, uint32_t* traced_tiles_out) {
+    if (int rc = bind(ctx)) return rc;
+    if (!p) return fail(ctx, PT_ERR_INVALID_ARG, "pt_debug_traced_tiles: null params");
+    if (p->width == 0 || p->height == 0 || p->width > 32768 || p->height > 32768) return fail(ctx, PT_ERR_INVALID_ARG, "pt_debug_traced_tiles: bad resolution");
+    const uint32_t count = p->tile_count ? p->tile_count : 1u;
+    if (p->tile_rank >= count) return fail(ctx, PT_ERR_INVALID_ARG, "pt_debug_traced_tiles: tile_rank >= tile_count");
+    const uint32_t tiles_x = (p->width + pt::kTile - 1) / pt::kTile, tiles_y = (p->height + pt::kTile - 1) / pt::kTile, need = (tiles_x * tiles_y + 31u) / 32u;
+    if (bitmask_out && words < need) return fail(ctx, PT_ERR_INVALID_ARG, "pt_debug_traced_tiles: the bitmask needs one bit per tile of the frame");
+    if (int rc = sync_refit_meta(ctx)) return rc;
+    ptk::FrameParams f; std::memset(&f, 0, sizeof(f));
+    std::memcpy(f.cam, p->cam_pos, 12); std::memcpy(f.quat, p->cam_quat, 16); f.focal = p->focal; f.aspect = p->aspect;
+    const bool brute = (p->flags & PT_FLAG_BRUTE_FORCE) != 0, stats = (p->flags & PT_FLAG_STATS) != 0;
+    TileRect rect = {0, 0, tiles_x, tiles_y};
+    const uint32_t* cover = nullptr; uint32_t cover_id = 0u;
+    if (!brute && launch_rect(ctx, &f, 1u, p->width, p->height, p->num_tris, rect)) {
+        if (!stats && PtTune::pick(ctx->tune.timeline, 0u) == 0u && PtTune::pick(ctx->tune.cull, 2u) >= 2u) {
+            if (int rc = tile_cover(ctx, &f, 1u, p->width, p->height, p->num_tris, true, &cover, &cover_id)) return rc;
+        }
+    } else rect = {0, 0, tiles_x, tiles_y};
+    std::vector<uint32_t> owned;
+    pt::tile_list(p->width, p->height, p->tile_rank, count, owned);
+    if (bitmask_out) std::memset(bitmask_out, 0, size_t(words) * sizeof(uint32_t));
+    uint32_t in_rect = 0, traced = 0;
+    for (uint32_t tile : owned) {
+        const uint32_t tx = tile % tiles_x, ty = tile / tiles_x;
+        if (!(tx >= rect.tx0 && tx < rect.tx1 && ty >= rect.ty0 && ty < rect.ty1)) continue;
+        ++in_rect;
+        if (cover && !((cover[tile >> 5] >> (tile & 31u)) & 1u)) continue;
+        ++traced;
+        if (bitmask_out) bitmask_out[tile >> 5] |= 1u << (tile & 31u);
+    }
+    if (rect_tiles) *rect_tiles = in_rect;
+    if (traced_tiles_out) *traced_tiles_out = traced;
+    return PT_OK;
+}
+
 int pt_read_radiance(PtContext* ctx, float* dst, uint64_t dst_floats) {
     if (int rc = bind(ctx)) return rc;
     if (int rc = flush_pending(ctx)) return rc;
diff --git a/raytracer-public_amd/csrc/pt_cover.hip b/raytracer-public_amd/csrc/pt_cover.hip
--- /dev/null
+++ b/raytracer-public_amd/csrc/pt_cover.hip
@@ -0,0 +1,125 @@
+#include "pt_kernels.h"
+#include "pt_bounds.h"
+
+namespace ptk {
+
+namespace {
+
+constexpr uint32_t kCutBlock = 1024;
+constexpr uint32_t kCoverBlock = 64;
+constexpr uint32_t kCutLeafBit = 0x80000000u;
+constexpr uint32_t kCutEmpty = 0xFFFFFFFFu;
+
+__device__ __forceinline__ uint32_t cut_node_of(uint32_t ref, uint32_t node_base16, uint32_t num_wide) {
+    if ((ref & kCutLeafBit) || ref < node_base16 || ((ref - node_base16) & 3u)) return kCutEmpty;
+    const uint32_t idx = (ref - node_base16) >> 2;
+    return idx < num_wide ? idx : kCutEmpty;
+}
+
+__global__ __launch_bounds__(kCutBlock) void tile_cut_kernel(const uint4* __restrict__ wide, uint32_t num_wide, uint32_t node_base16, uint32_t root_index,
+                                                             uint32_t* __restrict__ cut) {
+    __shared__ uint32_t frontier[2][kCutMax];
+    __shared__ uint32_t n_cur, n_next, expands;
+    const uint32_t tid = threadIdx.x;
+    if (tid == 0u) {
+        uint32_t n = 0;
+        if (root_index < num_wide)
+            for (uint32_t s = 0; s < 4u; ++s) if (wide[(size_t)root_index * 4u + s].w != kCutEmpty) frontier[0][n++] = (root_index << 2) | s;
+        n_cur = n; n_next = 0u; expands = 0u;
+    }
+    __syncthreads();
+    uint32_t cur = 0u;
+    for (uint32_t level = 0; level < 64u; ++level) {
+        const uint32_t n = n_cur;
+        uint32_t grows = 0u, internal = 0u;
+        for (uint32_t i = tid; i < n; i += kCutBlock) {
+            const uint32_t e = frontier[cur][i];
+            const uint32_t node = cut_node_of(wide[(size_t)(e >> 2) * 4u + (e & 3u)].w, node_base16, num_wide);
+            if (node == kCutEmpty) { grows += 1u; continue; }
+            internal = 1u;
+            for (uint32_t s = 0; s < 4u; ++s) grows += wide[(size_t)node * 4u + s].w != kCutEmpty ? 1u : 0u;
+        }
+        if (grows) atomicAdd(&n_next, grows);
+        if (internal) atomicOr(&expands, 1u);
+        __syncthreads();
+        const uint32_t total = n_next, any = expands;
+        __syncthreads();
+        if (total > kCutMax || any == 0u) break;
+        if (tid == 0u) { n_next = 0u; expands = 0u; }
+        __syncthreads();
+        for (uint32_t i = tid; i < n; i += kCutBlock) {
+            const uint32_t e = frontier[cur][i];
+            const uint32_t node = cut_node_of(wide[(size_t)(e >> 2) * 4u + (e & 3u)].w, node_base16, num_wide);
+            if (node == kCutEmpty) { frontier[cur ^ 1u][atomicAdd(&n_next, 1u)] = e; continue; }
+            for (uint32_t s = 0; s < 4u; ++s)
+                if (wide[(size_t)node * 4u + s].w != kCutEmpty) frontier[cur ^ 1u][atomicAdd(&n_next, 1u)] = (node << 2) | s;
+        }
+        __syncthreads();
+        if (tid == 0u) { n_cur = n_next; n_next = 0u; expands = 0u; }
+        cur ^= 1u;
+        __syncthreads();
+    }
+    const uint32_t n = n_cur;
+    for (uint32_t i = tid; i < n; i += kCutBlock) cut[i] = frontier[cur][i];
+    if (tid == 0u) cut[kCutMax] = n;
+}
+
+__global__ __launch_bounds__(kCoverBlock) void tile_cover_kernel(const uint4* __restrict__ wide, const uint32_t* __restrict__ cut, uint32_t count, const CoverCams cams,
+                                                         uint32_t width, uint32_t height, uint32_t tiles_x, uint32_t tiles_y, uint32_t* mask, uint32_t words) {
+    const uint32_t i = blockIdx.x * blockDim.x + threadIdx.x;
+    if (i >= count) return;
+    const uint32_t e = cut[i];
+    const uint4 piece = wide[(size_t)(e >> 2) * 4u + (e & 3u)];
+    if (piece.w == kCutEmpty || box_degenerate(piece.x, piece.y, piece.z)) return;
+    const CoverCam& c = cams.c[blockIdx.y];
+    const double mn[3] = {half_exact(piece.x & 0xffffu), half_exact(piece.x >> 16), half_exact(piece.y & 0xffffu)};
+    const double mx[3] = {half_exact(piece.y >> 16), half_exact(piece.z & 0xffffu), half_exact(piece.z >> 16)};
+    const double qx = c.quat[0], qy = c.quat[1], qz = c.quat[2], qw = c.quat[3];
+    double x0 = 1e300, x1 = -1e300, y0 = 1e300, y1 = -1e300;
+    bool ok = true;
+    for (int k = 0; k < 8; ++k) {
+        const double p[3] = {((k & 1) ? mx[0] : mn[0]) - c.cam[0], ((k & 2) ? mx[1] : mn[1]) - c.cam[1], ((k & 4) ? mx[2] : mn[2]) - c.cam[2]};
+        const double ux = -qx, uy = -qy, uz = -qz;
+        const double cx = uy * p[2] - uz * p[1], cy = uz * p[0] - ux * p[2], cz = ux * p[1] - uy * p[0];
+        const double dx = uy * cz - uz * cy, dy = uz * cx - ux * cz, dz = ux * cy - uy * cx;
+        const double vx = p[0] + 2.0 * (qw * cx + dx), vy = p[1] + 2.0 * (qw * cy + dy), vz = p[2] + 2.0 * (qw * cz + dz);
+        if (!(vz < -1e-4)) ok = false;
+        const double sx = vx / -vz * c.focal / c.aspect, sy = vy / -vz * c.focal;
+        const double fx = (sx + 1.0) * 0.5 * width, fy = (sy + 1.0) * 0.5 * height;
+        if (!(fx > -1e300 && fx < 1e300 && fy > -1e300 && fy < 1e300)) ok = false;
+        x0 = fx < x0 ? fx : x0; x1 = fx > x1 ? fx : x1; y0 = fy < y0 ? fy : y0; y1 = fy > y1 ? fy : y1;
+    }
+    if (!ok) { atomicOr(&mask[words], 1u); return; }
+    const double margin = 2.0;
+    auto lo = [&](double v, uint32_t n) { v = (v - margin) / 8.0; return v <= 0.0 ? 0u : (v >= n ? n : uint32_t(v)); };
+    auto hi = [&](double v, uint32_t n) { v = (v + margin) / 8.0 + 1.0; return v <= 0.0 ? 0u : (v >= n ? n : uint32_t(v)); };
+    const uint32_t tx0 = lo(x0, tiles_x), tx1 = hi(x1, tiles_x), ty0 = lo(y0, tiles_y), ty1 = hi(y1, tiles_y);
+    if (tx0 >= tx1) return;
+    for (uint32_t ty = ty0; ty < ty1; ++ty) {
+        const uint32_t a = ty * tiles_x + tx0, b = ty * tiles_x + tx1;
+        for (uint32_t w = a >> 5; w <= ((b - 1u) >> 5); ++w) {
+            const uint32_t first = w == (a >> 5) ? (a & 31u) : 0u, last = w == ((b - 1u) >> 5) ? ((b - 1u) & 31u) : 31u;
+            const uint32_t bits = (0xFFFFFFFFu << first) & (0xFFFFFFFFu >> (31u - last));
+            if ((__hip_atomic_load(&mask[w], __ATOMIC_RELAXED, __HIP_MEMORY_SCOPE_AGENT) & bits) != bits) atomicOr(&mask[w], bits);
+        }
+    }
+}
+
+}
+
+hipError_t launch_tile_cut(const uint4* wide, uint32_t num_wide, uint32_t node_base16, uint32_t root_index, uint32_t* cut, hipStream_t stream) {
+    hipLaunchKernelGGL(tile_cut_kernel, dim3(1), dim3(kCutBlock), 0, stream, wide, num_wide, node_base16, root_index, cut);
+    return hipGetLastError();
+}
+
+hipError_t launch_tile_cover(const uint4* wide, const uint32_t* cut, uint32_t count, const CoverCams& cams, uint32_t num_cams, uint32_t width, uint32_t height,
+                             uint32_t* mask, uint32_t words, hipStream_t stream) {
+    if (count == 0u || num_cams == 0u) return hipSuccess;
+    if (count > kCutMax || num_cams > kCoverCams) return hipErrorInvalidValue;
+    const uint32_t tiles_x = (width + 7u) / 8u, tiles_y = (height + 7u) / 8u;
+    if ((uint64_t)tiles_x * tiles_y > (uint64_t)words * 32u) return hipErrorInvalidValue;
+    hipLaunchKernelGGL(tile_cover_kernel, dim3((count + kCoverBlock - 1u) / kCoverBlock, num_cams), dim3(kCoverBlock), 0, stream, wide, cut, count, cams, width, height, tiles_x, tiles_y, mask, words);
+    return hipGetLastError();
+}
+
+}
diff --git a/raytracer-public_amd/csrc/pt_kernels.h b/raytracer-public_amd/csrc/pt_kernels.h
--- a/raytracer-public_amd/csrc/pt_kernels.h
+++ b/raytracer-public_amd/csrc/pt_kernels.h
@@ -188,6 +188,13 @@
 hipError_t launch_refit_prepare2(const uint32_t* bvh2, uint32_t nn2, uint32_t* parent2, hipStream_t stream);
 hipError_t launch_refit2(const float* tris9, uint32_t num_tris, uint32_t* bvh2, uint32_t nn2, const uint32_t* parent2, uint32_t* arrive, hipStream_t stream);
 hipError_t launch_bvh_cost(const uint32_t* bvh4, uint32_t num_nodes4, const uint2* self, double* out, hipStream_t stream);
+constexpr uint32_t kCutMax = 4096;
+hipError_t launch_tile_cut(const uint4* wide, uint32_t num_wide, uint32_t node_base16, uint32_t root_index, uint32_t* cut, hipStream_t stream);
+constexpr uint32_t kCoverCams = 16;
+struct CoverCam { float cam[3]; float focal; float quat[4]; float aspect; };
+struct CoverCams { CoverCam c[kCoverCams]; };
+hipError_t launch_tile_cover(const uint4* wide, const uint32_t* cut, uint32_t count, const CoverCams& cams, uint32_t num_cams, uint32_t width, uint32_t height,
+                             uint32_t* mask, uint32_t words, hipStream_t stream);
 hipError_t launch_rgba8(const float4* src, uint32_t* dst, uint32_t n, hipStream_t stream);
 hipError_t launch_tonemap(const float4* src, uint32_t* dst, uint32_t width, uint32_t height, int from_rgba8, hipStream_t stream);
 
diff --git a/raytracer-public_amd/csrc/pt_megakernel.hip b/raytracer-public_amd/csrc/pt_megakernel.hip
--- a/raytracer-public_amd/csrc/pt_megakernel.hip
+++ b/raytracer-public_amd/csrc/pt_megakernel.hip
@@ -274,7 +274,11 @@
     const FrameParams* const frames = A.frames;
     float4* const* const outs = A.outs;
     const uint32_t f_begin = ACCUM ? 0u : blockIdx.y, f_end = ACCUM ? A.num_frames : blockIdx.y + 1u;
-    const bool untraced = A.trace_slots != nullptr && !(tx >= A.trace_rect[0] && tx < A.trace_rect[1] && ty >= A.trace_rect[2] && ty < A.trace_rect[3]);
+    bool untraced = false;
+    if (A.trace_slots != nullptr) {
+        untraced = !(tx >= A.trace_rect[0] && tx < A.trace_rect[1] && ty >= A.trace_rect[2] && ty < A.trace_rect[3]);
+        if (!untraced) untraced = ((A.trace_slots[A.num_trace_tiles + (tile >> 5)] >> (tile & 31u)) & 1u) == 0u;
+    }
     for (uint32_t fid = f_begin; fid < f_end; ++fid) {
         F3 sum = f3(0.0f, 0.0f, 0.0f);
         float4* const sp = A.samples + (((size_t)fid * A.batches_per_frame + (size_t)slot * A.spp) * 64u + p);
```

New measurement: 12850 Msamples/s, median of 6. +6.1%, better.
